# RediSearch/RediSearch

Hardware: NVIDIA H100
Metric: KNN QPS @k=10 on 10M x 768 fp32 (cosine, batch=256) (higher is better)
Workload: dtype f32

## Files before the change

### redisearch_b200/csrc/coarse_tc.cu

```cuda
#include "coarse_tc.h"
#include "distance_core.cuh"
#include "topk_common.cuh"

#include <cuda.h>
#include <cuda_fp16.h>
#include <algorithm>
#include <cstdio>
#include <cstdlib>
#include <type_traits>

namespace rsb200 {

constexpr int kTileM = 128;
constexpr int kMaxStages = 8;
constexpr int kCoarseThreads = 256;
constexpr int kListCap = 64;
constexpr uint32_t kStageBytes = kTileM * 128;
constexpr int kTF32StageStride = 33;

struct CfgTF32 {
    static constexpr int kTileN = 32;
    static constexpr int kBlockK = 32;
    static constexpr int kElem = 4;
};
// ... 320 lines not shown
        const int ew = warp - 4;
        const int et = threadIdx.x - 128;
        mbar_wait(qbar, 0);
        uint32_t s = 0, ph = 0;
        const uint64_t bdesc_first = make_smem_desc(smem_u32(sQ));
        constexpr uint64_t kQStep = kQBlockBytes >> 4, kHalfTile = (kStageBytes / 2) >> 4;
        for (uint32_t i = 0; i < my_tiles; i++) {
            const uint32_t tile = blockIdx.x + i * gridDim.x;
            float acc[2][16];
            uint32_t prev = 0;
            for (uint32_t kb = 0; kb < num_kb; kb++) {
                mbar_wait_spin(&full[s], ph);
                wg_fence();
                const uint64_t ad = make_smem_desc(smem_u32(sA + (size_t)s * kStageBytes));
                const uint64_t bd = bdesc_first + (uint64_t)kb * kQStep;
#pragma unroll
                for (int kk = 0; kk < 4; kk++) {
                    const uint32_t acc_on = (kb | (uint32_t)kk) != 0;
                    wgmma_tf32_n32(acc[0], ad + 2 * kk, bd + 2 * kk, acc_on);
                    wgmma_tf32_n32(acc[1], ad + kHalfTile + 2 * kk, bd + 2 * kk, acc_on);
                }
                wg_commit();
                wg_wait<1>();
                if (kb != 0 && et == 0) mbar_arrive(&empty[prev]);
                prev = s;
                if (++s == nstages) s = 0, ph ^= 1;
            }
            wg_wait<0>();
            if (et == 0) mbar_arrive(&empty[prev]);
            wg_fence_operands(acc[0]);
            wg_fence_operands(acc[1]);
            asm volatile("bar.sync 1, 128;" ::: "memory");
#pragma unroll
            for (int mb = 0; mb < 2; mb++)
#pragma unroll
                for (int j = 0; j < 4; j++)
#pragma unroll
                    for (int x = 0; x < 4; x++) {
                        const int r = 64 * mb + 16 * ew + (lane >> 2) + 8 * (x >> 1), c = 8 * j + 2 * (lane & 3) + (x & 1);
                        sacc[r * kTF32StageStride + c] = __float_as_uint(acc[mb][4 * j + x]);
                    }
            asm volatile("bar.sync 1, 128;" ::: "memory");
            uint32_t v[kHalves][32];
#pragma unroll
            for (int h = 0; h < kHalves; h++)
#pragma unroll
                for (int j = 0; j < 32; j++) v[h][j] = sacc[et * kTF32StageStride + h * 32 + j];
            const uint32_t row = tile * kTileM + et;
            uint32_t pend[kHalves];
#pragma unroll
            for (int h = 0; h < kHalves; h++) {
                pend[h] = 0;
                if (row < n_rows) {
#pragma unroll
                    for (int j = 0; j < 32; j++) {
                        const float d = 1.0f - __uint_as_float(v[h][j]);
                        v[h][j] = orderable_key(d);
                        if (v[h][j] < thresh[h * 32 + j]) pend[h] |= 1u << j;
                    }
                }
            }
            for (;;) {
                uint32_t any_left = 0;
#pragma unroll
                for (int h = 0; h < kHalves; h++) {
                    uint32_t still = 0;
                    uint32_t p = pend[h];
                    while (p) {
                        const int jj = __ffs(p) - 1;
                        p &= p - 1;
                        uint32_t key = 0;
#pragma unroll
                        for (int x = 0; x < 32; x++)
                            if (x == jj) key = v[h][x];
                        const int j = h * 32 + jj;
                        if (key >= thresh[j]) continue;
                        const uint32_t slot = atomicAdd(&counts[j], 1u);
                        if (slot < (uint32_t)kListCap)
                            lists[j * kListCap + slot] = ((uint64_t)key << 32) | row;
                        else
                            still |= 1u << jj;
                    }
                    pend[h] = still;
                    any_left |= still;
                }
                if (any_left) *pending_flag = 1;
                asm volatile("bar.sync 1, 128;" ::: "memory");
                const uint32_t any_pending = *pending_flag;
                for (int j = ew; j < kTileN; j += 4) {
                    const uint32_t c = min(counts[j], (uint32_t)kListCap);
                    if (c < (uint32_t)(kListCap / 2) && !any_pending) continue;
                    if (c <= keep) {
                        if (lane == 0) counts[j] = c;
                        continue;
                    }
                    uint64_t e0 = (lane < (int)c) ? lists[j * kListCap + lane] : kEmptySlot;
                    uint64_t e1 = (lane + 32 < (int)c) ? lists[j * kListCap + lane + 32] : kEmptySlot;
                    __syncwarp();
                    uint64_t last = 0;
                    for (uint32_t r = 0; r < keep; r++) {
                        uint64_t m = e0 < e1 ? e0 : e1;
#pragma unroll
                        for (int sft = 16; sft > 0; sft >>= 1) {
                            const uint64_t o = shfl_xor_u64(m, sft);
                            m = o < m ? o : m;
                        }
                        if (e0 == m) e0 = kEmptySlot; else if (e1 == m) e1 = kEmptySlot;
                        if (lane == 0) lists[j * kListCap + r] = m;
                        last = m;
                    }
                    if (lane == 0) {
                        counts[j] = keep;
                        thresh[j] = (uint32_t)(last >> 32);
                    }
                }
                asm volatile("bar.sync 1, 128;" ::: "memory");
                if (!any_pending) break;
                if (et == 0) *pending_flag = 0;
                asm volatile("bar.sync 1, 128;" ::: "memory");
            }
        }
        asm volatile("bar.sync 1, 128;" ::: "memory");
        for (int j = ew; j < kTileN; j += 4) {
            const uint32_t c = min(counts[j], (uint32_t)kListCap);
            uint64_t e0 = (lane < (int)c) ? lists[j * kListCap + lane] : kEmptySlot;
            uint64_t e1 = (lane + 32 < (int)c) ? lists[j * kListCap + lane + 32] : kEmptySlot;
            const uint32_t q = q_base + j;
            for (uint32_t r = 0; r < keep; r++) {
                uint64_t m = e0 < e1 ? e0 : e1;
#pragma unroll
                for (int sft = 16; sft > 0; sft >>= 1) {
                    const uint64_t o = shfl_xor_u64(m, sft);
                    m = o < m ? o : m;
                }
                if (e0 == m) e0 = kEmptySlot; else if (e1 == m) e1 = kEmptySlot;
                if (lane == 0 && q < nq) cand_out[((size_t)q * gridDim.x + blockIdx.x) * keep + r] = m;
            }
        }
    }
}

constexpr int kQM = 64;
constexpr int kQN = 128;
constexpr int kQMaxStages = 16;
constexpr int kQKbPerStage = 2;
constexpr int kQListStride = 129;
constexpr uint32_t kQBlockBytes = kQN * 128;
constexpr uint32_t kQStageBytes = kQKbPerStage * kQBlockBytes;
__host__ __device__ constexpr uint32_t coarse_kb(uint32_t bytes_per_row) {
    return ((bytes_per_row + 127) / 128 + kQKbPerStage - 1) / kQKbPerStage * kQKbPerStage;
}
constexpr int kQAccStride = kQN + 4;
constexpr uint32_t kQAccBytes = kQM * kQAccStride * 4;
__host__ __device__ constexpr int coarse_consumers(int mode) { return mode == 1 ? 2 : 1; }
__host__ __device__ constexpr int coarse_cta_queries(bool q8, int mode) { return q8 && mode == 1 ? 2 * kQM : kQM; }
__host__ __device__ constexpr int coarse_threads(int mode) { return 128 * (1 + coarse_consumers(mode)); }

template <int kId, int kCount>
__device__ __forceinline__ void named_sync() {
    asm volatile("bar.sync %0, %1;" ::"n"(kId), "n"(kCount) : "memory");
}
template <int kId, int kCount>
__device__ __forceinline__ void named_arrive() {
    asm volatile("bar.arrive %0, %1;" ::"n"(kId), "n"(kCount) : "memory");
}

enum : int { kCaPass, kCaWait, kCaIssue, kCaWait1, kCaEpilogue, kCaHandoff, kCaTiles, kCaSlots };
#ifdef COARSE_CYCLE_ACCOUNT
constexpr int kCaMaxCtas = 1024;
__device__ unsigned long long g_coarse_cycles[kCaMaxCtas][3][kCaSlots];
struct CycleAccount {
    unsigned long long v[kCaSlots] = {};
    __device__ __forceinline__ long long now() const { return clock64(); }
    __device__ __forceinline__ void add(int slot, long long t0) { v[slot] += (unsigned long long)(clock64() - t0); }
    __device__ __forceinline__ void count(int slot) { v[slot]++; }
    __device__ __forceinline__ void flush(uint32_t cta, int role) {
        if (cta < (uint32_t)kCaMaxCtas)
            for (int i = 0; i < kCaSlots; i++) g_coarse_cycles[cta][role][i] = v[i];
    }
};
#else
struct CycleAccount {
    __device__ __forceinline__ long long now() const { return 0; }
    __device__ __forceinline__ void add(int, long long) {}
    __device__ __forceinline__ void count(int) {}
    __device__ __forceinline__ void flush(uint32_t, int) {}
};
#endif

template <int kEpl>
__device__ __forceinline__ uint32_t select_keep(uint64_t *lists, int q, uint32_t c, uint32_t keep, int lane) {
    __syncwarp();
    uint64_t e[kEpl];
    uint32_t k[kEpl];
    bool v[kEpl];
#pragma unroll
    for (int t = 0; t < kEpl; t++) {
        const uint32_t idx = lane + 32 * t;
        v[t] = idx < c;
        e[t] = v[t] ? lists[idx * kQListStride + q] : kEmptySlot;
        k[t] = (uint32_t)(e[t] >> 32);
    }
    __syncwarp();
    uint32_t prefix = 0, remaining = keep;
#pragma unroll 1
    for (int bit = 31; bit >= 0; bit--) {
        const uint32_t hi_mask = bit == 31 ? 0u : ~((2u << bit) - 1u);
        uint32_t zeros = 0;
#pragma unroll
        for (int t = 0; t < kEpl; t++) {
            const bool z = v[t] && ((k[t] ^ prefix) & hi_mask) == 0 && !((k[t] >> bit) & 1u);
            zeros += __popc(__ballot_sync(0xFFFFFFFFu, z));
        }
        if (zeros < remaining) {
            remaining -= zeros;
            prefix |= 1u << bit;
        }
    }
    const uint32_t lt = (1u << lane) - 1u;
    uint32_t base = 0;
#pragma unroll
    for (int t = 0; t < kEpl; t++) {
        const bool less = v[t] && k[t] < prefix;
        const uint32_t m = __ballot_sync(0xFFFFFFFFu, less);
        if (less) lists[(base + __popc(m & lt)) * kQListStride + q] = e[t];
        base += __popc(m);
    }
    uint32_t n_eq = 0;
#pragma unroll
    for (int t = 0; t < kEpl; t++) n_eq += __popc(__ballot_sync(0xFFFFFFFFu, v[t] && k[t] == prefix));
    uint32_t row_cut = 0xFFFFFFFFu;
    if (n_eq > remaining) {
        uint32_t rp = 0, rem = remaining;
#pragma unroll 1
        for (int bit = 31; bit >= 0; bit--) {
            const uint32_t hi_mask = bit == 31 ? 0u : ~((2u << bit) - 1u);
            uint32_t zeros = 0;
#pragma unroll
            for (int t = 0; t < kEpl; t++) {
                const uint32_t row = (uint32_t)e[t];
                const bool z = v[t] && k[t] == prefix && ((row ^ rp) & hi_mask) == 0 && !((row >> bit) & 1u);
                zeros += __popc(__ballot_sync(0xFFFFFFFFu, z));
            }
            if (zeros < rem) {
                rem -= zeros;
                rp |= 1u << bit;
            }
        }
        row_cut = rp;
    }
#pragma unroll
    for (int t = 0; t < kEpl; t++) {
        const bool eq = v[t] && k[t] == prefix && (uint32_t)e[t] <= row_cut;
        const uint32_t m = __ballot_sync(0xFFFFFFFFu, eq);
        if (eq) lists[(base + __popc(m & lt)) * kQListStride + q] = e[t];
        base += __popc(m);
    }
    __syncwarp();
    return prefix;
}

__device__ __forceinline__ int range_int_bound(float r) {
    if (!(r == r) || r < -1073741824.0f) return INT_MIN;
    if (r >= 1073741824.0f) return INT_MAX;
    int x = (int)floorf(r);
    while (__int2float_rn(x + 1) <= r) x++;
    return x;
}

__device__ __forceinline__ int q8_dot_bound(float tdot, float rq, float rt) {
    const float r = __fmul_rn(rq, rt);
    const float f = __fmul_rn(tdot, r);
    if (!(f == f) || !(r >= 0x1p-125f && r <= 0x1p125f)) return INT_MIN;
    const float c = fminf(fmaxf(f, -33554432.0f), 33554432.0f);
    return (int)floorf(c - fabsf(c) * 1e-5f) - 1;
}

template <bool kDirect, int kEpl, int kOp, int kMode, int kVar = 0, bool kFilt = false, int kRegKb = 0>
__global__ void __launch_bounds__(coarse_threads(kMode), 1)
coarse_wgmma_kernel(const __grid_constant__ CUtensorMap map_rows, const uint8_t *__restrict__ shadow, size_t row_pitch,
                    const uint8_t *__restrict__ q16, size_t q16_pitch, const float *__restrict__ row_norm2,
                    const float *__restrict__ q_norm2, uint32_t n_rows, uint32_t nq, uint32_t dim, uint32_t row_bytes,
                    uint32_t num_kb, uint32_t tiles_total, uint32_t keep, uint32_t nstages, uint32_t csize,
                    uint64_t *__restrict__ list_scratch, uint64_t *__restrict__ cand_out, const uint32_t *__restrict__ nq_dev,
                    uint32_t tile_stride, const float *__restrict__ thr_fixed, uint32_t *__restrict__ overflow,
                    const uint32_t *__restrict__ filt, uint32_t filt_words, const uint32_t *__restrict__ filt_q) {
    constexpr bool kFixed = kMode == 1, kSample = kMode == 2;
    constexpr bool kQ8 = kOp == 5;
    constexpr bool kInt = kOp == 1 || kOp == 2 || kOp == 4 || kQ8;
    constexpr int kOpE = kQ8 ? 0 : kOp;
    constexpr int kCons = coarse_consumers(kMode), kConsThreads = 128 * kCons;
    constexpr int kCtaQ = coarse_cta_queries(kQ8, kMode);
    constexpr bool kWide = kCtaQ > kQM;
    static_assert(!kWide || (kCons == 2 && kCtaQ == kCons * kQM), "a wide CTA: one consumer warpgroup per 64 queries");
    constexpr uint32_t kQKbBytes = kCtaQ * 128;
    using Acc = typename std::conditional<kInt, uint32_t, float>::type;
    const uint32_t bx = blockIdx.x, by = blockIdx.y, gx = gridDim.x;
    static_assert(kMode == 0 || (!kDirect && (kOp == 0 || kOp == 3 || kQ8)) || (kDirect && kOp == 0) || (kDirect && kFixed && kInt && kEpl == 8),
                  "fixed bound / sample pass: the fp32 route and 16-bit corpora (inner product / cosine); fixed radius: 8-bit corpora");
    static_assert(!kQ8 || (!kDirect && !kFilt && kRegKb == 0 && kVar == 1), "int8 shadow: signed operands, no filters");
    static_assert(!kFilt || (!kDirect && (kOp == 0 || kOp == 3)) || (kDirect && kFixed && kInt && kEpl == 8),
                  "row filters: the fp32 route and the 8-bit fixed-radius pass");
    static_assert(kRegKb == 0 || (!kDirect && kFixed && kRegKb % kQKbPerStage == 0),
                  "register-held queries: the fixed-bound pass over the fp16 shadow, whole stages");
    auto filt_row = [&](uint32_t pos) { return filt + (size_t)filt_words * (filt_q ? filt_q[pos] : pos); };
    constexpr int kSliceSets = (int)kCoarseSampleSlices / (kQN / 32);
    constexpr int kQListCap = kEpl * 32;
    if (nq_dev) {
        nq = min(nq, *nq_dev);
        if (nq == 0) return;
    }
    constexpr uint32_t kQTrigger = kQListCap - 32;
    extern __shared__ uint8_t smem_raw[];
    uint8_t *smem = smem_raw + ((1024u - (smem_u32(smem_raw) & 1023u)) & 1023u);
    uint8_t *sB = smem;
    uint8_t *sQ = sB + (size_t)nstages * kQStageBytes;
    uint32_t *sacc = reinterpret_cast<uint32_t *>(sQ + (size_t)(num_kb - kRegKb) * kQKbBytes);
    uint64_t *bars = reinterpret_cast<uint64_t *>(sacc + (kFixed ? 0 : kQM * kQAccStride));
    uint64_t *full = bars, *empty = bars + kQMaxStages;
    uint32_t *qcount = reinterpret_cast<uint32_t *>(bars + 2 * kQMaxStages);
    uint64_t *lists = list_scratch + (size_t)(by * gx + bx) * (kQListCap * kQListStride);

    const int warp = threadIdx.x >> 5, lane = threadIdx.x & 31;
    const uint32_t q_base = by * kCtaQ;
    const uint32_t my_tiles = (tiles_total > bx) ? (tiles_total - bx + gx - 1) / gx : 0;

    if (threadIdx.x == 0) {
        for (uint32_t s = 0; s < nstages; s++) {
            mbar_init(&full[s], 1);
            mbar_init(&empty[s], kWide ? kCons * csize : csize);
        }
        asm volatile("fence.mbarrier_init.release.cluster;" ::: "memory");
        asm volatile("fence.proxy.async.shared::cta;" ::: "memory");
    }
    __syncthreads();
    const uint32_t crank = (csize > 1) ? cluster_ctarank() : 0;
    const uint16_t cmask = (uint16_t)((1u << csize) - 1u);
    if (csize > 1) cluster_sync_all();

    CycleAccount ca;
    const uint32_t cta = by * gx + bx;
    if (warp == 0) {
        uint32_t s = 0, ph = 0;
        const uint32_t slice = kQStageBytes / csize;
        const long long t_pass = ca.now();
        for (uint32_t i = 0; i < my_tiles; i++) {
            const uint32_t tile = (bx + i * gx) * tile_stride;
            ca.count(kCaTiles);
            for (uint32_t kb0 = 0; kb0 < num_kb; kb0 += kQKbPerStage) {
                const uint32_t kbn = min((uint32_t)kQKbPerStage, num_kb - kb0);
                const long long t_wait = ca.now();
                mbar_wait_spin(&empty[s], ph ^ 1);
                ca.add(kCaWait, t_wait);
                if (elect_one_sync()) {
                    const uint32_t bytes = kbn * kQBlockBytes;
                    mbar_expect_tx(&full[s], bytes);
                    if constexpr (kDirect) {
                        const uint32_t slice_rows = kQN / csize;
                        for (uint32_t j = 0; j < kbn; j++) {
                            uint8_t *dst = sB + (size_t)s * kQStageBytes + j * kQBlockBytes + crank * slice_rows * 128;
                            const int c0 = (int)((kb0 + j) * ((kOp == 0 || kOp == 3) ? 64 : 128)), c1 = (int)(tile * kQN + crank * slice_rows);
                            if (csize > 1)
                                tma_load_2d_mc(dst, &map_rows, &full[s], c0, c1, cmask);
                            else
                                tma_load_2d(dst, &map_rows, &full[s], c0, c1);
                        }
                    } else {
                        const uint8_t *src = shadow + ((size_t)tile * num_kb + kb0) * kQBlockBytes;
                        if constexpr (kFixed) {
                            if (i + 1 < my_tiles) bulk_prefetch_l2(src + (size_t)gx * num_kb * kQBlockBytes + crank * slice, slice);
                        }
                        if (csize > 1) {
                            bulk_load_1d_mc(sB + (size_t)s * kQStageBytes + crank * slice, src + crank * slice, slice, &full[s], cmask);
                        } else {
                            bulk_load_1d(sB + (size_t)s * kQStageBytes, src, bytes, &full[s]);
                        }
                    }
                }
                __syncwarp();
                if (++s == nstages) s = 0, ph ^= 1;
            }
        }
        ca.add(kCaPass, t_pass);
        if (kFixed && lane == 0) ca.flush(cta, 2);
    } else if (warp >= 4) {
        const int cw = kCons > 1 ? (warp - 4) >> 2 : 0;
        const int ew = kCons > 1 ? (warp - 4) & 3 : warp - 4;
        const int et = kCons > 1 ? (threadIdx.x - 128) & 127 : threadIdx.x - 128;
        const int wq = kWide ? kQM * cw : 0;
        const uint32_t qw = q_base + wq;
        const uint32_t q = qw + et;
        const bool live = et < kQM && q < nq;
        if ((kWide || cw == 0) && et < kQM) {
            const uint4 *src = reinterpret_cast<const uint4 *>(q16 + (size_t)q * q16_pitch);
            for (uint32_t kb = kRegKb; kb < num_kb; kb++) {
                uint8_t *row = sQ + (size_t)(kb - kRegKb) * kQKbBytes + wq * 128 + et * 128;
#pragma unroll
                for (int u = 0; u < 8; u++) {
                    uint4 x = make_uint4(0, 0, 0, 0);
                    if (live && kb * 128 + u * 16 < row_bytes) x = src[kb * 8 + u];
                    *reinterpret_cast<uint4 *>(row + ((u ^ (et & 7)) * 16)) = x;
                }
            }
            if constexpr (kFixed) qcount[wq + et] = 0;
        }
        uint32_t qa[kRegKb ? 4 * kRegKb : 1][4];
        if constexpr (kRegKb > 0) {
#pragma unroll
            for (int i2 = 0; i2 < 2; i2++) {
                const uint32_t fq = qw + 16 * ew + (lane >> 2) + 8 * i2;
                const uint8_t *src = q16 + (size_t)fq * q16_pitch;
#pragma unroll
                for (int t = 0; t < 4 * kRegKb; t++)
#pragma unroll
                    for (int h = 0; h < 2; h++) {
                        const uint32_t off = 32 * t + 4 * (lane & 3) + 16 * h;
                        qa[t][i2 + 2 * h] = (fq < nq && off < row_bytes) ? __ldg(reinterpret_cast<const uint32_t *>(src + off)) : 0u;
                    }
            }
        }
        asm volatile("fence.proxy.async.shared::cta;" ::: "memory");
        named_sync<1, kConsThreads>();
        auto release = [&](uint32_t st) {
            if (csize == 1) {
                if (et == 0) mbar_arrive(&empty[st]);
            } else if (et < (int)csize) {
                mbar_arrive_remote(mapa_u32(smem_u32(&empty[st]), (uint32_t)et));
            }
        };
        uint32_t thr = 0xFFFFFFFFu, cnt = 0;
        float thr_dot = -__int_as_float(0x7f800000);
        float nq_norm = 1.0f;
        if constexpr (kOp == 2) nq_norm = live ? *reinterpret_cast<const float *>(q16 + (size_t)q * q16_pitch + dim) : 1.0f;
        if constexpr (kOp == 3) nq_norm = live ? q_norm2[q] : 0.0f;
        const int *irn2 = reinterpret_cast<const int *>(row_norm2);
        int nq_int = 0, thr_e = live ? INT_MAX : INT_MIN;
        if constexpr (kOp == 4) nq_int = live ? reinterpret_cast<const int *>(q_norm2)[q] : 0;
        float smax[kSample ? kSliceSets : 1][kQN / 32];
#pragma unroll
        for (int x = 0; x < (kSample ? kSliceSets : 1); x++)
#pragma unroll
            for (int h = 0; h < kQN / 32; h++) smax[x][h] = -__int_as_float(0x7f800000);
        if (!live) thr_dot = __int_as_float(0x7f800000);
        uint32_t fthr[2];
        float fthr_dot[2], fnq[2];
        float frad[2];
        int fix[2], fnqi[2];
        float fsq[2] = {1.0f, 1.0f};
        float frq[2] = {1.0f, 1.0f};
        if constexpr (kQ8) {
#pragma unroll
            for (int i2 = 0; i2 < 2; i2++) {
                const uint32_t fq = qw + 16 * ew + (lane >> 2) + 8 * i2;
                if (fq < nq) fsq[i2] = *reinterpret_cast<const float *>(q16 + (size_t)fq * q16_pitch + row_bytes);
                if constexpr (kFixed) frq[i2] = __frcp_rn(fsq[i2]);
            }
        }
        if constexpr (kFixed && kInt && !kQ8) {
#pragma unroll
            for (int i2 = 0; i2 < 2; i2++) {
                const uint32_t fq = qw + 16 * ew + (lane >> 2) + 8 * i2;
                const bool flive = fq < nq;
                frad[i2] = flive ? thr_fixed[fq] : __int_as_float(0x7fffffff);
                fix[i2] = range_int_bound(frad[i2]);
                fnqi[i2] = (kOp == 4 && flive) ? reinterpret_cast<const int *>(q_norm2)[fq] : 0;
                fnq[i2] = (kOp == 2 && flive) ? *reinterpret_cast<const float *>(q16 + (size_t)fq * q16_pitch + dim) : 0.0f;
                fthr_dot[i2] = fnq[i2] * ((1.0f - frad[i2]) - 1e-6f * (1.0f + fabsf(frad[i2])));
            }
        }
        if constexpr (kFixed && (!kInt || kQ8)) {
#pragma unroll
            for (int i2 = 0; i2 < 2; i2++) {
                const uint32_t fq = qw + 16 * ew + (lane >> 2) + 8 * i2;
                const bool flive = fq < nq;
                fnq[i2] = (kOp == 3 && flive) ? q_norm2[fq] : 0.0f;
                const float T = flive ? thr_fixed[fq] : -__int_as_float(0x7f800000);
                fthr[i2] = orderable_key(T);
                if constexpr (kOpE == 0) {
                    const float t = 1.0f - T;
                    fthr_dot[i2] = t - (4e-7f + 2.4e-7f * fabsf(t));
                } else {
                    fthr_dot[i2] = 0.5f * (fnq[i2] - T) - 2e-6f * (fabsf(fnq[i2]) + fabsf(T));
                }
                if (!(T == T)) fthr_dot[i2] = -__int_as_float(0x7f800000), fthr[i2] = 0xFFFFFFFFu;
                if (!flive) fthr_dot[i2] = __int_as_float(0x7f800000);
            }
        }
        uint32_t s = 0, ph = 0;
        const uint64_t bdesc_first = make_smem_desc(smem_u32(sB)), adesc_first = make_smem_desc(smem_u32(sQ + wq * 128));
        constexpr uint64_t kStageStep = kQStageBytes >> 4, kBlockStep = kQBlockBytes >> 4, kAKbStep = kQKbBytes >> 4;
        const uint32_t stages_per_tile = num_kb / kQKbPerStage;
        auto skip = [&](uint32_t n) {
            for (s += n; s >= nstages; s -= nstages) ph ^= 1;
        };
        if (kCons > 1 && !kWide) skip(stages_per_tile * cw);
        const long long t_pass = ca.now();
        for (uint32_t i = kWide ? 0 : cw; i < my_tiles; i += kWide ? 1 : kCons) {
            const uint32_t tile = (bx + i * gx) * tile_stride;
            if (kCons > 1 && !kWide && i >= (uint32_t)kCons) skip(stages_per_tile * (kCons - 1));
            ca.count(kCaTiles);
            float nrm[kQN / 32];
            int inrm[kQN / 32];
            if constexpr (kOp == 4) {
#pragma unroll
                for (int h = 0; h < kQN / 32; h++) {
                    const uint32_t r = tile * kQN + h * 32 + lane;
                    inrm[h] = r < n_rows ? __ldg(irn2 + r) : 0;
                }
            }
            if constexpr (kOp == 3 && !kFixed) {
#pragma unroll
                for (int h = 0; h < kQN / 32; h++) {
                    const uint32_t r = tile * kQN + h * 32 + lane;
                    nrm[h] = r < n_rows ? __ldg(row_norm2 + r) : 0.0f;
                }
            }
            if constexpr (kOp == 2) {
#pragma unroll
                for (int h = 0; h < kQN / 32; h++) {
                    const uint32_t r = tile * kQN + h * 32 + lane;
                    nrm[h] = r < n_rows ? __ldg(reinterpret_cast<const float *>(shadow + (size_t)r * row_pitch + dim)) : 1.0f;
                }
            }
            const uint32_t rbase = tile * kQN + 2 * (lane & 3);
            float q8_st = 0.0f;
            if constexpr (kFixed && kQ8) q8_st = __ldg(row_norm2 + tile);
            float2 rn[(kFixed && kOp == 3) ? kQN / 8 : 1];
            if constexpr (kFixed && kOp == 3) {
#pragma unroll
                for (int j = 0; j < kQN / 8; j++) {
                    const uint32_t r = rbase + 8 * j;
                    if (r + 1 < n_rows)
                        rn[j] = __ldg(reinterpret_cast<const float2 *>(row_norm2 + r));
                    else
                        rn[j] = make_float2(r < n_rows ? __ldg(row_norm2 + r) : 0.0f, 0.0f);
                }
            }
            if constexpr (kCons > 1 && !kWide) {
                static_assert(kCons == 2, "the hand-off pairs two warpgroups");
                const long long t_handoff = ca.now();
                if (i != 0) {
                    if (cw == 0)
                        named_sync<2, 2 * 128>();
                    else
                        named_sync<3, 2 * 128>();
                }
                ca.add(kCaHandoff, t_handoff);
            }
            Acc acc[64];
            uint32_t prev = 0;
            auto stage = [&](uint32_t kb0, auto issue) {
                const long long t_wait = ca.now();
                mbar_wait_spin(&full[s], ph);
                const long long t_issue = ca.now();
                ca.add(kCaWait, t_wait);
                wg_fence();
                issue(bdesc_first + (uint64_t)s * kStageStep);
                wg_commit();
                if constexpr (kCons > 1 && !kWide) {
                    if (kb0 + kQKbPerStage >= num_kb && i + 1 < my_tiles) {
                        if (cw == 0)
                            named_arrive<3, 2 * 128>();
                        else
                            named_arrive<2, 2 * 128>();
                    }
                }
                ca.add(kCaIssue, t_issue);
                const long long t_wait1 = ca.now();
                wg_wait<1>();
                ca.add(kCaWait1, t_wait1);
                if (kb0 != 0) release(prev);
                prev = s;
                if (++s == nstages) s = 0, ph ^= 1;
            };
            if constexpr (kRegKb > 0) {
#pragma unroll
                for (int rs = 0; rs < kRegKb / kQKbPerStage; rs++)
                    stage(rs * kQKbPerStage, [&](uint64_t bd) {
#pragma unroll
                        for (int x = 0; x < 4 * kQKbPerStage; x++)
                            wgmma_f16_n128_ra(acc, qa[4 * kQKbPerStage * rs + x], bd + (x >> 2) * kBlockStep + 2 * (x & 3), (rs | x) != 0);
                    });
            }
            for (uint32_t kb0 = kRegKb; kb0 < num_kb; kb0 += kQKbPerStage)
                stage(kb0, [&](uint64_t bd) {
                    const uint64_t ad = adesc_first + (uint64_t)(kb0 - kRegKb) * kAKbStep;
#pragma unroll
                    for (int x = 0; x < 4 * kQKbPerStage; x++)
                        wgmma_n128<kInt, kVar>(acc, ad + (x >> 2) * kAKbStep + 2 * (x & 3), bd + (x >> 2) * kBlockStep + 2 * (x & 3),
                                               (kb0 | (uint32_t)x) != 0);
                });
            const long long t_epilogue = ca.now();
            wg_wait<0>();
            release(prev);
            wg_fence_operands(acc);
            if constexpr (kFixed && kQ8) {
                const float st = q8_st, rst = __frcp_rn(st);
#pragma unroll
                for (int i2 = 0; i2 < 2; i2++) {
                    const float sqt = __fmul_rn(fsq[i2], st);
                    const int ti = q8_dot_bound(fthr_dot[i2], frq[i2], rst);
                    int m3[11];
#pragma unroll
                    for (int g = 0; g < 10; g++)
                        m3[g] = __vimax3_s32((int)acc[4 * ((3 * g) >> 1) + 2 * i2 + ((3 * g) & 1)],
                                             (int)acc[4 * ((3 * g + 1) >> 1) + 2 * i2 + ((3 * g + 1) & 1)],
                                             (int)acc[4 * ((3 * g + 2) >> 1) + 2 * i2 + ((3 * g + 2) & 1)]);
                    m3[10] = max((int)acc[4 * 15 + 2 * i2], (int)acc[4 * 15 + 2 * i2 + 1]);
                    const int mx = __vimax3_s32(__vimax3_s32(m3[0], m3[1], m3[2]), __vimax3_s32(m3[3], m3[4], m3[5]),
                                                __vimax3_s32(__vimax3_s32(m3[6], m3[7], m3[8]), m3[9], m3[10]));
                    uint32_t pass = 0;
                    if (mx > ti) {
#pragma unroll
                        for (int j = 0; j < kQN / 8; j++)
#pragma unroll
                            for (int c = 0; c < 2; c++)
                                if ((int)acc[4 * j + 2 * i2 + c] > ti) pass |= 1u << (2 * j + c);
                    }
                    if (pass && tile * kQN + kQN > n_rows) {
#pragma unroll
                        for (int j = 0; j < kQN / 8; j++)
#pragma unroll
                            for (int c = 0; c < 2; c++)
                                if (rbase + 8 * j + c >= n_rows) pass &= ~(1u << (2 * j + c));
                    }
                    while (pass) {
                        const int b = __ffs(pass) - 1;
                        pass &= pass - 1;
                        uint32_t raw = 0;
#pragma unroll
                        for (int x = 0; x < 32; x++)
                            if (x == b) raw = acc[4 * (x >> 1) + 2 * i2 + (x & 1)];
                        const uint32_t row = rbase + 8 * (b >> 1) + (b & 1);
                        const uint32_t key = orderable_key(__fsub_rn(1.0f, __fmul_rn(sqt, __int2float_rn((int)raw))));
                        if (key < fthr[i2]) {
                            const int qs = wq + 16 * ew + (lane >> 2) + 8 * i2;
                            const uint32_t slot = atomicAdd(&qcount[qs], 1u);
                            if (slot < (uint32_t)kQListCap) lists[slot * kQListStride + qs] = ((uint64_t)key << 32) | row;
                        }
                    }
                }
                ca.add(kCaEpilogue, t_epilogue);
                continue;
            }
            if constexpr (kFixed && kInt) {
                uint32_t pass2[2] = {0u, 0u};
                if constexpr (kOp == 1) {
#pragma unroll
                    for (int i2 = 0; i2 < 2; i2++) {
                        int mx = (int)acc[2 * i2];
#pragma unroll
                        for (int x = 1; x < 32; x++) mx = max(mx, (int)acc[4 * (x >> 1) + 2 * i2 + (x & 1)]);
                        if (1 - mx <= fix[i2]) {
#pragma unroll
                            for (int x = 0; x < 32; x++)
                                if (1 - (int)acc[4 * (x >> 1) + 2 * i2 + (x & 1)] <= fix[i2]) pass2[i2] |= 1u << x;
                        }
                    }
                } else {
#pragma unroll
                    for (int j = 0; j < kQN / 8; j++)
#pragma unroll
                        for (int c = 0; c < 2; c++) {
                            const int src = 8 * (j & 3) + 2 * (lane & 3) + c;
                            if constexpr (kOp == 4) {
                                const int rn = __shfl_sync(0xFFFFFFFFu, inrm[j >> 2], src);
#pragma unroll
                                for (int i2 = 0; i2 < 2; i2++)
                                    if (rn + fnqi[i2] - 2 * (int)acc[4 * j + 2 * i2 + c] <= fix[i2]) pass2[i2] |= 1u << (2 * j + c);
                            } else {
                                const float nr = __shfl_sync(0xFFFFFFFFu, nrm[j >> 2], src);
#pragma unroll
                                for (int i2 = 0; i2 < 2; i2++)
                                    if (__int2float_rn((int)acc[4 * j + 2 * i2 + c]) >= nr * fthr_dot[i2]) pass2[i2] |= 1u << (2 * j + c);
                            }
                        }
                }
#pragma unroll
                for (int i2 = 0; i2 < 2; i2++) {
                    uint32_t pass = pass2[i2];
                    if (pass && tile * kQN + kQN > n_rows) {
#pragma unroll
                        for (int x = 0; x < 32; x++)
                            if (rbase + 8 * (x >> 1) + (x & 1) >= n_rows) pass &= ~(1u << x);
                    }
                    while (pass) {
                        const int b = __ffs(pass) - 1;
                        pass &= pass - 1;
                        uint32_t raw = 0;
#pragma unroll
                        for (int x = 0; x < 32; x++)
                            if (x == b) raw = acc[4 * (x >> 1) + 2 * i2 + (x & 1)];
                        const uint32_t row = rbase + 8 * (b >> 1) + (b & 1);
                        float d;
                        if constexpr (kOp == 1) {
                            d = (float)(1 - (int)raw);
                        } else if constexpr (kOp == 2) {
                            const float nr = __ldg(reinterpret_cast<const float *>(shadow + (size_t)row * row_pitch + dim));
                            d = __fsub_rn(1.0f, __fdiv_rn((float)(int)raw, __fmul_rn(nr, fnq[i2])));
                        } else {
                            d = __int2float_rn(__ldg(irn2 + row) + fnqi[i2] - 2 * (int)raw);
                        }
                        bool hit = d <= frad[i2];
                        if constexpr (kFilt) {
                            if (hit) hit = (__ldg(filt_row(q_base + 16 * ew + (lane >> 2) + 8 * i2) + (row >> 5)) >> (row & 31)) & 1u;
                        }
                        if (hit) {
                            const int qs = wq + 16 * ew + (lane >> 2) + 8 * i2;
                            const uint32_t slot = atomicAdd(&qcount[qs], 1u);
                            if (slot < (uint32_t)kQListCap) lists[slot * kQListStride + qs] = ((uint64_t)orderable_key(d) << 32) | row;
                        }
                    }
                }
                ca.add(kCaEpilogue, t_epilogue);
                continue;
            }
            if constexpr (kFixed && !kInt) {
#pragma unroll
                for (int i2 = 0; i2 < 2; i2++) {
                    uint32_t pass = 0;
                    if constexpr (kOp == 0) {
                        float m8[8];
#pragma unroll
                        for (int g = 0; g < 8; g++)
                            m8[g] = fmaxf(fmaxf(acc[8 * g + 2 * i2], acc[8 * g + 2 * i2 + 1]), fmaxf(acc[8 * g + 4 + 2 * i2], acc[8 * g + 5 + 2 * i2]));
                        const float mx = fmaxf(fmaxf(fmaxf(m8[0], m8[1]), fmaxf(m8[2], m8[3])), fmaxf(fmaxf(m8[4], m8[5]), fmaxf(m8[6], m8[7])));
                        if (mx > fthr_dot[i2]) {
#pragma unroll
                            for (int j = 0; j < kQN / 8; j++)
#pragma unroll
                                for (int c = 0; c < 2; c++)
                                    if (acc[4 * j + 2 * i2 + c] > fthr_dot[i2]) pass |= 1u << (2 * j + c);
                        }
                    } else {
#pragma unroll
                        for (int j = 0; j < kQN / 8; j++)
#pragma unroll
                            for (int c = 0; c < 2; c++)
                                if (acc[4 * j + 2 * i2 + c] > fmaf(c ? rn[j].y : rn[j].x, 0.499999f, fthr_dot[i2])) pass |= 1u << (2 * j + c);
                    }
                    if (pass && tile * kQN + kQN > n_rows) {
#pragma unroll
                        for (int j = 0; j < kQN / 8; j++)
#pragma unroll
                            for (int c = 0; c < 2; c++)
                                if (rbase + 8 * j + c >= n_rows) pass &= ~(1u << (2 * j + c));
                    }
                    while (pass) {
// ... 32 lines not shown
            }
#pragma unroll
            for (int j = 0; j < kQN / 8; j++) {
                const int m = 16 * ew + (lane >> 2), n = 8 * j + 2 * (lane & 3);
                uint32_t b[4];
#pragma unroll
                for (int x = 0; x < 4; x++) {
                    if constexpr (kQ8)
                        b[x] = __float_as_uint(__fmul_rn(tsqt[x >> 1], __int2float_rn((int)acc[4 * j + x])));
                    else if constexpr (kInt)
                        b[x] = acc[4 * j + x];
                    else
                        b[x] = __float_as_uint(acc[4 * j + x]);
                }
                *reinterpret_cast<uint2 *>(sacc + m * kQAccStride + n) = make_uint2(b[0], b[1]);
                *reinterpret_cast<uint2 *>(sacc + (m + 8) * kQAccStride + n) = make_uint2(b[2], b[3]);
            }
            asm volatile("bar.sync 1, 128;" ::: "memory");
            uint32_t v[kQN / 32][32];
            {
                const uint32_t *mine = sacc + (et & (kQM - 1)) * kQAccStride;
#pragma unroll
                for (int h = 0; h < kQN / 32; h++)
#pragma unroll
                    for (int u = 0; u < 8; u++) {
                        const uint4 w = *reinterpret_cast<const uint4 *>(mine + h * 32 + 4 * u);
                        v[h][4 * u] = w.x, v[h][4 * u + 1] = w.y, v[h][4 * u + 2] = w.z, v[h][4 * u + 3] = w.w;
                    }
            }
#pragma unroll
            for (int h = 0; h < kQN / 32; h++) {
                const uint32_t row0 = tile * kQN + h * 32;
                uint32_t fw = 0xFFFFFFFFu;
                if constexpr (kFilt) fw = (live && row0 < n_rows) ? __ldg(filt_row(q) + (row0 >> 5)) : 0u;
                if constexpr (kSample) {
                    float mx = -__int_as_float(0x7f800000);
                    const bool tail = row0 + 32 > n_rows;
                    if constexpr (kFilt) {
#pragma unroll
                        for (int j = 0; j < 32; j++) {
                            float u = __uint_as_float(v[h][j]);
                            if constexpr (kOpE != 0) u = fmaf(__shfl_sync(0xFFFFFFFFu, nrm[h], j), -0.5f, u);
                            if ((fw >> j) & 1u) mx = fmaxf(mx, u);
                        }
                    } else if constexpr (kOpE == 0) {
                        if (!tail) {
                            float m8[8];
#pragma unroll
                            for (int g = 0; g < 8; g++)
                                m8[g] = fmaxf(fmaxf(__uint_as_float(v[h][4 * g]), __uint_as_float(v[h][4 * g + 1])),
                                              fmaxf(__uint_as_float(v[h][4 * g + 2]), __uint_as_float(v[h][4 * g + 3])));
                            mx = fmaxf(fmaxf(fmaxf(m8[0], m8[1]), fmaxf(m8[2], m8[3])), fmaxf(fmaxf(m8[4], m8[5]), fmaxf(m8[6], m8[7])));
                        } else {
#pragma unroll
                            for (int j = 0; j < 32; j++)
                                if (row0 + j < n_rows) mx = fmaxf(mx, __uint_as_float(v[h][j]));
                        }
                    } else {
#pragma unroll
                        for (int j = 0; j < 32; j++) {
                            const float u = fmaf(__shfl_sync(0xFFFFFFFFu, nrm[h], j), -0.5f, __uint_as_float(v[h][j]));
                            if (!tail || row0 + j < n_rows) mx = fmaxf(mx, u);
                        }
                    }
#pragma unroll
                    for (int x = 0; x < kSliceSets; x++)
                        if ((int)(i % (uint32_t)kSliceSets) == x) smax[kSample ? x : 0][h] = fmaxf(smax[kSample ? x : 0][h], mx);
                    continue;
                }
                uint32_t pass = 0;
#pragma unroll
                for (int j = 0; j < 32; j++) {
                    bool p;
                    if constexpr (kOpE == 0)
                        p = __uint_as_float(v[h][j]) > thr_dot;
                    else if constexpr (kOp == 1)
                        p = (float)(int)v[h][j] > thr_dot;
                    else if constexpr (kOp == 2)
                        p = (float)(int)v[h][j] > __shfl_sync(0xFFFFFFFFu, nrm[h], j) * thr_dot - 0.01f;
                    else if constexpr (kOp == 4)
                        p = __shfl_sync(0xFFFFFFFFu, inrm[h], j) + nq_int - 2 * (int)v[h][j] < thr_e;
                    else
                        p = __uint_as_float(v[h][j]) > fmaf(__shfl_sync(0xFFFFFFFFu, nrm[h], j), 0.499999f, thr_dot);
                    if (p) pass |= 1u << j;
                }
                if (row0 + 32 > n_rows) pass &= (n_rows > row0) ? ((1u << (n_rows - row0)) - 1u) : 0u;
                if constexpr (kFilt) pass &= fw;
                while (pass) {
                    const int j = __ffs(pass) - 1;
                    pass &= pass - 1;
                    uint32_t raw = 0;
#pragma unroll
                    for (int x = 0; x < 32; x++)
                        if (x == j) raw = v[h][x];
                    float d;
                    if constexpr (kOpE == 0)
                        d = 1.0f - __uint_as_float(raw);
                    else if constexpr (kOp == 1)
                        d = (float)(1 - (int)raw);
                    else if constexpr (kOp == 2) {
                        const uint32_t r = row0 + j;
                        const float nr = __ldg(reinterpret_cast<const float *>(shadow + (size_t)r * row_pitch + dim));
                        d = __fsub_rn(1.0f, __fdiv_rn((float)(int)raw, __fmul_rn(nr, nq_norm)));
                    } else if constexpr (kOp == 4) {
                        d = __int2float_rn(__ldg(irn2 + row0 + j) + nq_int - 2 * (int)raw);
                    } else {
                        d = __fsub_rn(__fadd_rn(nq_norm, __ldg(row_norm2 + row0 + j)), __fmul_rn(2.0f, __uint_as_float(raw)));
                    }
                    const uint32_t key = orderable_key(d);
                    if (key < thr) {
                        lists[cnt * kQListStride + et] = ((uint64_t)key << 32) | (row0 + j);
                        cnt++;
                    }
                }
                uint32_t m = __ballot_sync(0xFFFFFFFFu, cnt > kQTrigger);
                while (m) {
                    const int src = __ffs(m) - 1;
                    m &= m - 1;
                    const uint32_t c = __shfl_sync(0xFFFFFFFFu, cnt, src);
                    const uint32_t worst = select_keep<kEpl>(lists, ew * 32 + src, c, keep, lane);
                    if (lane == src) {
                        cnt = keep;
                        thr = worst;
                        const float t = 1.0f - key_to_float(thr);
                        if constexpr (kOpE == 0)
                            thr_dot = t - 4e-7f;
                        else if constexpr (kOp == 1)
                            thr_dot = t - (fabsf(t) * 1e-6f + 2.0f);
                        else if constexpr (kOp == 2) {
                            const float tq = t * nq_norm;
                            thr_dot = tq - fabsf(tq) * 4e-6f;
                        } else if constexpr (kOp == 4) {
                            thr_e = __float2int_ru(key_to_float(thr));
                        } else {
                            const float dthr = key_to_float(thr);
                            thr_dot = 0.5f * (nq_norm - dthr) - 2e-6f * (fabsf(nq_norm) + fabsf(dthr));
                        }
                    }
                }
            }
        }
        ca.add(kCaPass, t_pass);
        if (kFixed && et == 0) ca.flush(cta, cw);
        __syncwarp();
        if constexpr (kFixed) {
            named_sync<1, kConsThreads>();
            constexpr int per = kCtaQ / (4 * kCons);
            const int pw = 4 * cw + ew;
            for (int qs = per * pw; qs < per * pw + per; qs++) {
                const uint32_t qq = q_base + qs;
                if (qq >= nq) break;
                const uint32_t n = qcount[qs], c = min(n, (uint32_t)kQListCap);
                uint64_t *dst = cand_out + ((size_t)qq * gx + bx) * keep;
                for (uint32_t r = lane; r < keep; r += 32) dst[r] = r < c ? lists[r * kQListStride + qs] : kEmptySlot;
                if (lane == 0 && n > (uint32_t)kQListCap) overflow[qq] = 1u;
            }
        }
        if constexpr (kSample) {
            if (live) {
                uint64_t *dst = cand_out + ((size_t)q * gx + bx) * keep;
#pragma unroll
                for (int x = 0; x < kSliceSets; x++)
#pragma unroll
                    for (int h = 0; h < kQN / 32; h++) {
                        const float m = smax[kSample ? x : 0][h];
                        uint64_t c = kEmptySlot;
                        if (m > -__int_as_float(0x7f800000)) {
                            const float d = kOpE == 0 ? 1.0f - m : __fsub_rn(nq_norm, __fmul_rn(2.0f, m));
                            c = (uint64_t)orderable_key(d) << 32;
                        }
                        if ((uint32_t)(x * (kQN / 32) + h) < keep) dst[x * (kQN / 32) + h] = c;
                    }
            }
        }
        for (int src = 0; src < ((kSample || kFixed) ? 0 : 32); src++) {
            uint32_t c = __shfl_sync(0xFFFFFFFFu, cnt, src);
            const uint32_t qq = q_base + ew * 32 + src;
            if (c > keep) {
                select_keep<kEpl>(lists, ew * 32 + src, c, keep, lane);
                c = keep;
            }
            if (ew * 32 + src < kQM && qq < nq) {
                uint64_t *dst = cand_out + ((size_t)qq * gx + bx) * keep;
                __syncwarp();
                for (uint32_t r = lane; r < keep; r += 32) dst[r] = r < c ? lists[r * kQListStride + ew * 32 + src] : kEmptySlot;
            }
        }
    }
    __syncthreads();
    if (csize > 1) cluster_sync_all();
}

__global__ void __launch_bounds__(256) to_f16_kernel(const uint8_t *__restrict__ src, size_t spitch, uint32_t dim, uint32_t first,
                                                     uint32_t n, uint8_t *__restrict__ dst, size_t dpitch) {
    const uint32_t per_row = dim / 8;
    const size_t total = (size_t)n * per_row;
    for (size_t i = (size_t)blockIdx.x * blockDim.x + threadIdx.x; i < total; i += (size_t)gridDim.x * blockDim.x) {
        const uint32_t r = first + (uint32_t)(i / per_row), c = (uint32_t)(i % per_row);
        const float4 *p = reinterpret_cast<const float4 *>(src + (size_t)r * spitch) + 2 * c;
        const float4 x = p[0], y = p[1];
        __half2 h0 = __floats2half2_rn(x.x, x.y), h1 = __floats2half2_rn(x.z, x.w);
        __half2 h2 = __floats2half2_rn(y.x, y.y), h3 = __floats2half2_rn(y.z, y.w);
        uint4 o;
        o.x = *reinterpret_cast<uint32_t *>(&h0);
        o.y = *reinterpret_cast<uint32_t *>(&h1);
        o.z = *reinterpret_cast<uint32_t *>(&h2);
        o.w = *reinterpret_cast<uint32_t *>(&h3);
        reinterpret_cast<uint4 *>(dst + (size_t)r * dpitch)[c] = o;
    }
}

constexpr uint32_t kRefineMaxSurv = 2048;
constexpr uint32_t kRefineMaxSurvWide = 4096;

__device__ __forceinline__ float query_eps(float eps, const float *q_norm2, uint32_t pos, float max_norm, uint32_t dim, bool l2,
                                           const float *q_eps = nullptr) {
    if (q_eps) return q_eps[pos];
    if (!q_norm2) return eps;
    const float qn2 = q_norm2[pos], qn = sqrtf(qn2);
    float e = eps * max_norm * qn + 5.97e-8f * sqrtf((float)dim) * (max_norm + qn);
    if (l2) e = 2.0f * e + (float)(dim + 4) * 1.2e-7f * (max_norm * max_norm + qn2);
    return e * 1.0001f;
}
__device__ __forceinline__ uint32_t block_kth_key(const uint64_t *mine, uint32_t total, uint32_t k, uint32_t *hist, uint32_t *ctl) {
    const int lane = threadIdx.x & 31;
    if (threadIdx.x == 0) ctl[0] = 0, ctl[1] = k, ctl[2] = 0;
    __syncthreads();
    uint32_t cnt = 0;
    for (uint32_t i = threadIdx.x; i < total; i += blockDim.x) cnt += mine[i] != kEmptySlot;
    cnt = __reduce_add_sync(0xFFFFFFFFu, cnt);
    if (lane == 0 && cnt) atomicAdd(&ctl[2], cnt);
    __syncthreads();
    if (ctl[2] < k) return 0xFFFFFFFFu;
    for (int shift = 24; shift >= 0; shift -= 8) {
        hist[threadIdx.x] = 0;
        __syncthreads();
        const uint32_t prefix = ctl[0];
        const uint32_t hi_mask = shift == 24 ? 0u : ~((1u << (shift + 8)) - 1u);
        for (uint32_t i = threadIdx.x; i < total; i += blockDim.x) {
            const uint64_t c = mine[i];
            if (c == kEmptySlot) continue;
            const uint32_t key = (uint32_t)(c >> 32);
            if (((key ^ prefix) & hi_mask) == 0) atomicAdd(&hist[(key >> shift) & 255u], 1u);
        }
        __syncthreads();
        if (threadIdx.x == 0) {
            uint32_t rem = ctl[1], b = 0;
            for (; b < 255; b++) {
                if (hist[b] >= rem) break;
                rem -= hist[b];
            }
            ctl[0] = prefix | (b << shift);
            ctl[1] = rem;
        }
        __syncthreads();
    }
    return ctl[0];
}

__global__ void __launch_bounds__(256) threshold_kernel(const uint64_t *__restrict__ cand, uint32_t nq, uint32_t lists_per_query,
                                                        uint32_t keep, uint32_t k, float eps, const float *__restrict__ q_norm2,
                                                        float max_norm, uint32_t dim, int l2, float *__restrict__ thr_out,
                                                        uint32_t *__restrict__ overflow, const float *__restrict__ q_eps) {
    __shared__ uint32_t hist[256];
    __shared__ uint32_t ctl[4];
    const uint32_t q = blockIdx.x;
    if (q >= nq) return;
    const uint32_t ak = block_kth_key(cand + (size_t)q * lists_per_query * keep, lists_per_query * keep, k, hist, ctl);
    if (threadIdx.x == 0) {
        const float e = query_eps(eps, q_norm2, q, max_norm, dim, l2 != 0, q_eps);
        float T;
        if (ak == 0xFFFFFFFFu)
            T = __int_as_float(0x7f800000);
        else if (e == 0.0f)
            T = key_to_float(ak + 1u);
        else
            T = key_to_float(ak) + (2.0f * e) * 1.001f + 1e-30f;
        thr_out[q] = T;
        overflow[q] = 0;
    }
}

template <int MT, uint32_t kSurv, bool kLab = false>
__global__ void __launch_bounds__(256) refine_kernel(const uint8_t *rows, size_t pitch, uint32_t dim, const uint8_t *queries,
                                                     size_t qpitch, uint32_t nq, uint32_t lists_per_query, uint32_t keep, uint32_t k,
                                                     const uint64_t *__restrict__ cand, float eps, const float *__restrict__ q_norm2,
                                                     float max_norm, uint32_t *__restrict__ ok, uint32_t ok_value, uint64_t *__restrict__ out,
                                                     const uint32_t *__restrict__ q_index, const uint32_t *__restrict__ nq_dev,
                                                     const float *__restrict__ thr_T, const uint32_t *__restrict__ overflow,
                                                     uint32_t smem_cap, const uint64_t *__restrict__ row_label, const float *__restrict__ q_eps) {
    using Tile = DistTile<DT_F32, MT, 1, 1>;
    __shared__ uint64_t surv[kSurv];
    __shared__ uint32_t hist[256];
    __shared__ uint32_t ctl[4];
    __shared__ uint32_t s_nsurv, s_bad, s_ncomp;
    if (nq_dev) nq = min(nq, *nq_dev);
    if (blockIdx.x >= nq) return;
    const uint32_t q = q_index ? q_index[blockIdx.x] : blockIdx.x;
    const int warp = threadIdx.x >> 5, lane = threadIdx.x & 31;
    const uint64_t *mine = cand + (size_t)blockIdx.x * lists_per_query * keep;
    uint32_t total = lists_per_query * keep;
    eps = query_eps(eps, q_norm2, blockIdx.x, max_norm, dim, MT == MT_L2, q_eps);
    if (threadIdx.x == 0) s_nsurv = 0, s_bad = 0, s_ncomp = 0;
    __syncthreads();
    extern __shared__ uint64_t s_cand[];
    for (uint32_t i0 = 0; i0 < total; i0 += blockDim.x) {
        const uint32_t i = i0 + threadIdx.x;
        const uint64_t c = i < total ? mine[i] : kEmptySlot;
        const uint32_t m = __ballot_sync(0xFFFFFFFFu, c != kEmptySlot);
        uint32_t base = 0;
        if (lane == 0 && m) base = atomicAdd(&s_ncomp, (uint32_t)__popc(m));
        base = __shfl_sync(0xFFFFFFFFu, base, 0);
        if (c != kEmptySlot) {
            const uint32_t pos = base + __popc(m & ((1u << lane) - 1u));
            if (pos < smem_cap) s_cand[pos] = c;
        }
    }
    __syncthreads();
    const bool packed = s_ncomp <= smem_cap;
    const uint64_t *mine_all = mine;
    const uint32_t total_all = total;
    if (packed) {
        mine = s_cand;
        total = s_ncomp;
    }
    const uint32_t ak_key = block_kth_key(mine, total, k, hist, ctl);
    const float cut = ak_key == 0xFFFFFFFFu ? __int_as_float(0x7f800000) : key_to_float(ak_key) + (2.0f * eps) * 1.001f + 1e-30f;
    for (uint32_t i0 = 0; i0 < total; i0 += blockDim.x) {
        const uint32_t i = i0 + threadIdx.x;
        const uint64_t c = i < total ? mine[i] : kEmptySlot;
        const bool take = c != kEmptySlot && (ak_key == 0xFFFFFFFFu || key_to_float((uint32_t)(c >> 32)) <= cut);
        const uint32_t m = __ballot_sync(0xFFFFFFFFu, take);
        uint32_t base = 0;
        if (lane == 0 && m) base = atomicAdd(&s_nsurv, (uint32_t)__popc(m));
        base = __shfl_sync(0xFFFFFFFFu, base, 0);
        if (take) {
            const uint32_t pos = base + __popc(m & ((1u << lane) - 1u));
            if (pos < kSurv) surv[pos] = c;
        }
    }
    __syncthreads();
    const uint32_t n_all = s_nsurv, n_surv = min(n_all, kSurv);
    const uint8_t *qb[1] = {queries + (size_t)q * qpitch};
    for (uint32_t i = warp; i < n_surv; i += 8) {
        const uint32_t row = (uint32_t)surv[i];
        const uint8_t *rowb[1] = {rows + (size_t)row * pitch};
        float d[1];
        Tile::run(rowb, qb, dim, lane, d);
        __syncwarp();
        if (lane == 0) surv[i] = make_composite(d[0], kLab ? (uint32_t)row_label[row] : row);
    }
    const uint32_t n_sort = max(32u, next_pow2(n_surv));
    __syncthreads();
    for (uint32_t i = n_surv + threadIdx.x; i < n_sort; i += blockDim.x) surv[i] = kEmptySlot;
    bitonic_sort_smem(surv, n_sort);
    for (uint32_t i = threadIdx.x; i < k; i += blockDim.x) out[(size_t)q * k + i] = i < n_surv ? surv[i] : kEmptySlot;
    bool bad = n_all > kSurv;
    if (q_norm2 && !(q_norm2[blockIdx.x] == q_norm2[blockIdx.x])) bad = true;
    if (!isfinite(cut) || (thr_T && !isfinite(thr_T[blockIdx.x]))) bad = true;
    const bool have_k = n_surv >= k;
    const float ek = have_k ? key_to_float((uint32_t)(surv[k - 1] >> 32)) : 0.0f;
    if (thr_T) {
        if (threadIdx.x == 0 && (overflow[blockIdx.x] != 0 || !have_k || !(thr_T[blockIdx.x] - eps > ek))) bad = true;
    } else {
        (void)total_all;
        for (uint32_t l = threadIdx.x; l < lists_per_query; l += blockDim.x) {
            const uint64_t *lst = mine_all + (size_t)l * keep;
            uint32_t worst = 0;
            bool full = true;
            for (uint32_t j = 0; j < keep; j++) {
                const uint64_t c = lst[j];
                if (c == kEmptySlot)
                    full = false;
                else
                    worst = max(worst, (uint32_t)(c >> 32));
            }
            if (!full) continue;
            if (!have_k)
                bad = true;
            else if (!(key_to_float(worst) - eps > ek))
                bad = true;
        }
    }
    if (bad) atomicOr(&s_bad, 1u);
    __syncthreads();
    if (threadIdx.x == 0) ok[q] = s_bad ? 0u : ok_value;
}

constexpr uint32_t kRangeWindow = 2048;

__global__ void range_bound_kernel(const float *__restrict__ radius, uint32_t nq, float eps, const float *__restrict__ q_norm2,
                                   float max_norm, uint32_t dim, int l2, float *__restrict__ thr, uint32_t *__restrict__ overflow,
                                   uint32_t *__restrict__ total) {
    const uint32_t q = blockIdx.x * blockDim.x + threadIdx.x;
    if (q == 0) *total = 0;
    if (q >= nq) return;
    const float e = query_eps(eps, q_norm2, q, max_norm, dim, l2 != 0);
    thr[q] = radius[q] + e * 1.001f + 1e-30f;
    overflow[q] = 0;
}

constexpr double kR16U = 0x1p-24;
constexpr double kR16TcStep = 0x1p-22;
constexpr double kR16Underflow = 0x1p-149;
constexpr double kR16Flush = 0x1p-126;
constexpr double kR16Margin = 2.0;
constexpr double kR16MaxMag = 0x1p120;

template <int DT>
__global__ void __launch_bounds__(256) range_bound16_kernel(const uint8_t *__restrict__ queries, size_t qpitch, uint32_t nq, uint32_t dim,
                                                            const float *__restrict__ radius, float max_norm, float *__restrict__ thr,
                                                            uint32_t *__restrict__ overflow) {
    const uint32_t q = blockIdx.x * 8 + (threadIdx.x >> 5);
    const int lane = threadIdx.x & 31;
    if (q >= nq) return;
    const uint8_t *qb = queries + (size_t)q * qpitch;
    double s = 0.0;
    for (uint32_t i = lane; i < dim; i += 32) {
        const double v = (double)load16<DT>(qb, i);
        s = __fma_ru(v, v, s);
    }
#pragma unroll
    for (int o = 16; o > 0; o >>= 1) s = __dadd_ru(s, __shfl_xor_sync(0xFFFFFFFFu, s, o));
    if (lane != 0) return;
    const double d = (double)dim;
    const double qn = __dsqrt_ru(s);
    const double x = __dadd_ru(__dmul_ru(__dmul_ru((double)max_norm, 1.0 + 0x1p-23), __dsqrt_ru(__fma_ru(d, 0x1p-20, 1.0))),
                               __dsqrt_ru(__dmul_ru(d, 0x1p-149)));
    const double mag = __dmul_ru(x, qn);
    const double chain = 8.0 * ((dim / 8 + 31) / 32) + (double)((dim % 8 + 31) / 32) + 7.0;
    const double gamma = __ddiv_ru(chain * kR16U, __dsub_rd(1.0, chain * kR16U));
    const double ue = __dmul_ru(kR16U, __dadd_ru(1.0, mag));
    const double b_tc = __dadd_ru(__dmul_ru(__dmul_ru(d, kR16TcStep), mag), ue);
    const double b_cc = __dadd_ru(__dadd_ru(__dmul_ru(gamma, mag), ue), __dmul_ru(d, kR16Underflow));
    const double eps = __dmul_ru(kR16Margin, __dadd_ru(__dadd_ru(b_tc, b_cc), __dmul_ru(d, kR16Flush)));
    const float t = __double2float_ru(__dadd_ru((double)radius[q], eps));
    const bool ok = isfinite(qn) && isfinite(x) && mag < kR16MaxMag && isfinite(t);
    thr[q] = ok ? t : -__int_as_float(0x7f800000);
    overflow[q] = 0;
}

template <int DT, int MT>
__global__ void __launch_bounds__(256) range_refine_kernel(const uint8_t *rows, size_t pitch, uint32_t dim, const uint8_t *queries,
                                                           size_t qpitch, uint32_t slots, uint64_t *cand, const float *__restrict__ radius,
                                                           const float *__restrict__ q_norm2, const float *__restrict__ thr,
                                                           const uint32_t *__restrict__ overflow, uint64_t *__restrict__ out,
                                                           uint32_t *__restrict__ total, uint32_t *__restrict__ ok, uint32_t *__restrict__ cnt,
                                                           uint32_t *__restrict__ off, uint32_t cap) {
    using Tile = DistTile<DT, MT, 1, 1>;
    __shared__ uint64_t s_cand[kRangeWindow];
    __shared__ uint32_t s_n, s_kept, s_base;
    const uint32_t q = blockIdx.x;
    const int warp = threadIdx.x >> 5, lane = threadIdx.x & 31;
    bool proven = overflow[q] == 0 && isfinite(thr[q]);
    if (q_norm2 && !(q_norm2[q] == q_norm2[q])) proven = false;
    if (!proven) {
        if (threadIdx.x == 0) ok[q] = 0, cnt[q] = 0;
        if (threadIdx.x == 0 && !cap) off[q] = 0;
        return;
    }
    const float r = radius[q];
    uint64_t *mine = cand + (size_t)q * slots;
    const uint8_t *qb[1] = {queries + (size_t)q * qpitch};
    if (threadIdx.x == 0) s_kept = 0;
    for (uint32_t w0 = 0; w0 < slots; w0 += kRangeWindow) {
        const uint32_t wend = min(slots, w0 + kRangeWindow);
        if (threadIdx.x == 0) s_n = 0;
        __syncthreads();
        for (uint32_t i0 = w0; i0 < wend; i0 += blockDim.x) {
            const uint32_t i = i0 + threadIdx.x;
            const uint64_t c = i < wend ? mine[i] : kEmptySlot;
            const uint32_t m = __ballot_sync(0xFFFFFFFFu, c != kEmptySlot);
            uint32_t base = 0;
            if (lane == 0 && m) base = atomicAdd(&s_n, (uint32_t)__popc(m));
            base = __shfl_sync(0xFFFFFFFFu, base, 0);
            if (c != kEmptySlot) s_cand[base + __popc(m & ((1u << lane) - 1u))] = c;
        }
        __syncthreads();
        const uint32_t n = s_n;
        for (uint32_t i = warp; i < n; i += blockDim.x / 32) {
            const uint32_t row = (uint32_t)s_cand[i];
            const uint8_t *rowb[1] = {rows + (size_t)row * pitch};
            float d[1];
            Tile::run(rowb, qb, dim, lane, d);
            if (lane == 0 && d[0] <= r) mine[atomicAdd(&s_kept, 1u)] = make_composite(d[0], row);
        }
        __syncthreads();
    }
    const uint32_t kept = s_kept;
    if (cap) {
        if (threadIdx.x == 0) ok[q] = 1, cnt[q] = kept;
        for (uint32_t i = threadIdx.x; i < min(kept, cap); i += blockDim.x) out[(size_t)q * cap + i] = mine[i];
        return;
    }
    if (threadIdx.x == 0) {
        s_base = atomicAdd(total, kept);
        ok[q] = 1;
        cnt[q] = kept;
        off[q] = s_base;
    }
    __syncthreads();
    for (uint32_t i = threadIdx.x; i < kept; i += blockDim.x) out[s_base + i] = mine[i];
}

__global__ void __launch_bounds__(256) range_pack_kernel(const uint64_t *__restrict__ cand, uint32_t slots, const uint32_t *__restrict__ overflow,
                                                         uint32_t cap, uint64_t *__restrict__ out, uint32_t *__restrict__ cnt,
                                                         uint32_t *__restrict__ ok) {
    __shared__ uint32_t s_n;
    const uint32_t q = blockIdx.x;
    if (overflow[q]) {
        if (threadIdx.x == 0) ok[q] = 0, cnt[q] = 0;
        return;
    }
    if (threadIdx.x == 0) s_n = 0;
    __syncthreads();
    const uint64_t *mine = cand + (size_t)q * slots;
    for (uint32_t i = threadIdx.x; i < slots; i += blockDim.x) {
        const uint64_t c = mine[i];
        if (c == kEmptySlot) continue;
        const uint32_t pos = atomicAdd(&s_n, 1u);
        if (pos < cap) out[(size_t)q * cap + pos] = c;
    }
    __syncthreads();
    if (threadIdx.x == 0) ok[q] = 1, cnt[q] = s_n;
}

__global__ void __launch_bounds__(512) range_label_fold_kernel(const uint64_t *__restrict__ cand, uint32_t slots, const uint32_t *__restrict__ front,
                                                               const uint32_t *__restrict__ overflow, const uint64_t *__restrict__ id_to_label,
                                                               uint32_t cap, uint64_t *__restrict__ out, uint32_t *__restrict__ cnt,
                                                               uint32_t *__restrict__ ok, uint32_t *__restrict__ flags) {
    extern __shared__ uint64_t s_hi[];
    uint32_t *s_row = reinterpret_cast<uint32_t *>(s_hi + kRangeFoldMaxHits);
    __shared__ uint32_t s_n, s_labels;
    const uint32_t q = blockIdx.x;
    const bool proven = front ? ok[q] != 0 : overflow[q] == 0;
    if (!proven) {
        if (threadIdx.x == 0) ok[q] = 0, flags[q] = 0;
        return;
    }
// ... 16 lines not shown
        if (threadIdx.x == 0) ok[q] = 0, flags[q] = 3;
        return;
    }
    uint32_t n2 = 1;
    while (n2 < n) n2 <<= 1;
    for (uint32_t i = n + threadIdx.x; i < n2; i += blockDim.x) s_hi[i] = ~0ull, s_row[i] = ~0u;
    __syncthreads();
    for (uint32_t k = 2; k <= n2; k <<= 1)
        for (uint32_t j = k >> 1; j > 0; j >>= 1) {
            for (uint32_t i = threadIdx.x; i < n2; i += blockDim.x) {
                const uint32_t p = i ^ j;
                if (p <= i) continue;
                const uint64_t ha = s_hi[i], hb = s_hi[p];
                const uint32_t ra = s_row[i], rb = s_row[p];
                const bool b_first = hb < ha || (hb == ha && rb < ra);
                if (b_first == ((i & k) == 0)) {
                    s_hi[i] = hb, s_hi[p] = ha;
                    s_row[i] = rb, s_row[p] = ra;
                }
            }
            __syncthreads();
        }
    for (uint32_t i = threadIdx.x; i < n; i += blockDim.x) {
        if (i > 0 && (s_hi[i] >> 32) == (s_hi[i - 1] >> 32)) continue;
        const uint32_t pos = atomicAdd(&s_labels, 1u);
        if (pos < cap) out[(size_t)q * cap + pos] = (s_hi[i] << 32) | s_row[i];
    }
    __syncthreads();
    if (threadIdx.x == 0) ok[q] = 1, flags[q] = 1, cnt[q] = s_labels;
}

__global__ void compact_unproven_kernel(const uint32_t *__restrict__ ok, uint32_t nq, uint32_t *__restrict__ idx,
                                        uint32_t *__restrict__ count) {
    __shared__ uint32_t n;
    if (threadIdx.x == 0) n = 0;
    __syncthreads();
    for (uint32_t q0 = 0; q0 < nq; q0 += blockDim.x) {
        const uint32_t q = q0 + threadIdx.x;
        const bool un = q < nq && ok[q] == 0;
        const uint32_t m = __ballot_sync(0xFFFFFFFFu, un);
        __shared__ uint32_t wbase[32];
        const int warp = threadIdx.x >> 5, lane = threadIdx.x & 31;
        if (lane == 0) wbase[warp] = __popc(m);
        __syncthreads();
        uint32_t before = 0;
        for (int w = 0; w < warp; w++) before += wbase[w];
        uint32_t all = 0;
        for (uint32_t w = 0; w < blockDim.x / 32; w++) all += wbase[w];
        if (un) idx[n + before + __popc(m & ((1u << lane) - 1u))] = q;
        __syncthreads();
        if (threadIdx.x == 0) n += all;
        __syncthreads();
    }
    if (threadIdx.x == 0) *count = n;
}
__global__ void gather_queries_kernel(const uint8_t *__restrict__ src, size_t pitch, const float *__restrict__ src_n2,
                                      const uint32_t *__restrict__ idx, const uint32_t *__restrict__ count,
                                      uint8_t *__restrict__ dst, float *__restrict__ dst_n2) {
    const uint32_t n = *count;
    for (uint32_t i = blockIdx.x; i < n; i += gridDim.x) {
        const uint4 *s4 = reinterpret_cast<const uint4 *>(src + (size_t)idx[i] * pitch);
        uint4 *d4 = reinterpret_cast<uint4 *>(dst + (size_t)i * pitch);
        for (uint32_t c = threadIdx.x; c < pitch / 16; c += blockDim.x) d4[c] = s4[c];
        if (src_n2 && threadIdx.x == 0) dst_n2[i] = src_n2[idx[i]];
    }
}

typedef CUresult (*EncodeTiledFn)(CUtensorMap *, CUtensorMapDataType, cuuint32_t, void *, const cuuint64_t *,
                                  const cuuint64_t *, const cuuint32_t *, const cuuint32_t *, CUtensorMapInterleave,
                                  CUtensorMapSwizzle, CUtensorMapL2promotion, CUtensorMapFloatOOBfill);

static EncodeTiledFn encode_fn() {
    static EncodeTiledFn fn = nullptr;
    static bool tried = false;
    if (!tried) {
        tried = true;
        void *p = nullptr;
        cudaDriverEntryPointQueryResult qres;
        if (cudaGetDriverEntryPoint("cuTensorMapEncodeTiled", &p, cudaEnableDefault, &qres) == cudaSuccess &&
            qres == cudaDriverEntryPointSuccess)
            fn = reinterpret_cast<EncodeTiledFn>(p);
    }
    return fn;
}

static bool make_map(CUtensorMap *m, CUtensorMapDataType dt, const void *base, uint64_t inner, uint64_t outer, uint64_t pitch_bytes,
                     uint32_t box_inner, uint32_t box_outer) {
    EncodeTiledFn fn = encode_fn();
    if (!fn) return false;
    cuuint64_t dims[2] = {inner, outer};
    cuuint64_t strides[1] = {pitch_bytes};
    cuuint32_t box[2] = {box_inner, box_outer};
    cuuint32_t estr[2] = {1, 1};
    return fn(m, dt, 2, const_cast<void *>(base), dims, strides, box, estr, CU_TENSOR_MAP_INTERLEAVE_NONE,
              CU_TENSOR_MAP_SWIZZLE_128B, CU_TENSOR_MAP_L2_PROMOTION_L2_256B, CU_TENSOR_MAP_FLOAT_OOB_FILL_NONE) == CUDA_SUCCESS;
}


static constexpr size_t kSmemLimit = 232448;

template <int V>
static const void *wgmma_kernel_fn_v(CoarseKind kind, uint32_t epl, int epi, int mode, bool filt) {
    if (filt) {
        if (kind != CoarseDirect8 || mode != 1) return nullptr;
        if (epi == 2) return (const void *)coarse_wgmma_kernel<true, 8, 4, 1, V, true>;
        return epi == 1 ? (const void *)coarse_wgmma_kernel<true, 8, 2, 1, V, true> : (const void *)coarse_wgmma_kernel<true, 8, 1, 1, V, true>;
    }
    if (kind == CoarseDirect16) {
        if (mode == 1) return (const void *)coarse_wgmma_kernel<true, 8, 0, 1, V>;
        if (mode == 2) return (const void *)coarse_wgmma_kernel<true, 3, 0, 2, V>;
        return epl == 3 ? (const void *)coarse_wgmma_kernel<true, 3, 0, 0, V> : (const void *)coarse_wgmma_kernel<true, 8, 0, 0, V>;
    }
    if (kind == CoarseDirect8) {
        if (mode == 1) {
            if (epi == 2) return (const void *)coarse_wgmma_kernel<true, 8, 4, 1, V>;
            return epi == 1 ? (const void *)coarse_wgmma_kernel<true, 8, 2, 1, V> : (const void *)coarse_wgmma_kernel<true, 8, 1, 1, V>;
        }
        if (epi == 2) return epl == 3 ? (const void *)coarse_wgmma_kernel<true, 3, 4, 0, V> : (const void *)coarse_wgmma_kernel<true, 8, 4, 0, V>;
        if (epi == 1) return epl == 3 ? (const void *)coarse_wgmma_kernel<true, 3, 2, 0, V> : (const void *)coarse_wgmma_kernel<true, 8, 2, 0, V>;
        return epl == 3 ? (const void *)coarse_wgmma_kernel<true, 3, 1, 0, V> : (const void *)coarse_wgmma_kernel<true, 8, 1, 0, V>;
    }
    return nullptr;
}
static constexpr uint32_t kFixedRegKb = 4;
static uint32_t fixed_reg_kb(uint32_t epl, bool l2, bool filt) { return (epl == 3 && !l2 && !filt) ? kFixedRegKb : 0u; }
static const void *wgmma_kernel_fn(CoarseKind kind, uint32_t epl, int epi, int mode = 0, uint32_t variant = 0, bool filt = false,
                                   uint32_t reg_kb = 0) {
    const bool l2 = epi != 0;
    if (kind == CoarseDirect16 || kind == CoarseDirect8)
        return variant ? wgmma_kernel_fn_v<1>(kind, epl, epi, mode, filt) : wgmma_kernel_fn_v<0>(kind, epl, epi, mode, filt);
    if (kind == CoarseQ8) {
        if (filt || reg_kb || epi) return nullptr;
        if (mode == 1) return (const void *)coarse_wgmma_kernel<false, 8, 5, 1, 1>;
        if (mode == 2) return (const void *)coarse_wgmma_kernel<false, 3, 5, 2, 1>;
        return epl == 8 ? (const void *)coarse_wgmma_kernel<false, 8, 5, 0, 1> : nullptr;
    }
    if (reg_kb) {
        if (mode != 1 || reg_kb != fixed_reg_kb(epl, l2, filt)) return nullptr;
        return (const void *)coarse_wgmma_kernel<false, 3, 0, 1, 0, false, kFixedRegKb>;
    }
    if (filt) {
        if (mode == 1 && epl == 8) return l2 ? (const void *)coarse_wgmma_kernel<false, 8, 3, 1, 0, true> : (const void *)coarse_wgmma_kernel<false, 8, 0, 1, 0, true>;
        if (mode == 1) return l2 ? (const void *)coarse_wgmma_kernel<false, 3, 3, 1, 0, true> : (const void *)coarse_wgmma_kernel<false, 3, 0, 1, 0, true>;
        if (mode == 2) return l2 ? (const void *)coarse_wgmma_kernel<false, 3, 3, 2, 0, true> : (const void *)coarse_wgmma_kernel<false, 3, 0, 2, 0, true>;
        if (epl != 8) return nullptr;
        return l2 ? (const void *)coarse_wgmma_kernel<false, 8, 3, 0, 0, true> : (const void *)coarse_wgmma_kernel<false, 8, 0, 0, 0, true>;
    }
    if (mode == 1 && epl == 8) return l2 ? (const void *)coarse_wgmma_kernel<false, 8, 3, 1> : (const void *)coarse_wgmma_kernel<false, 8, 0, 1>;
    if (mode == 1) return l2 ? (const void *)coarse_wgmma_kernel<false, 3, 3, 1> : (const void *)coarse_wgmma_kernel<false, 3, 0, 1>;
    if (mode == 2) return l2 ? (const void *)coarse_wgmma_kernel<false, 3, 3, 2> : (const void *)coarse_wgmma_kernel<false, 3, 0, 2>;
    if (l2) return epl == 3 ? (const void *)coarse_wgmma_kernel<false, 3, 3, 0> : (const void *)coarse_wgmma_kernel<false, 8, 3, 0>;
    return epl == 3 ? (const void *)coarse_wgmma_kernel<false, 3, 0, 0> : (const void *)coarse_wgmma_kernel<false, 8, 0, 0>;
}
static size_t wgmma_fixed_smem(uint32_t num_kb, int mode = 0, uint32_t reg_kb = 0, uint32_t cta_q = kQM) {
    return 1024 + (size_t)(num_kb - reg_kb) * cta_q * 128 + (mode == 1 ? cta_q * 4 : kQAccBytes) + 2 * kQMaxStages * 8 + 64;
}
static uint32_t wgmma_stages(uint32_t num_kb, int mode, uint32_t reg_kb, uint32_t cta_q = kQM) {
    return (uint32_t)std::min<size_t>(kQMaxStages, (kSmemLimit - wgmma_fixed_smem(num_kb, mode, reg_kb, cta_q)) / kQStageBytes);
}
static bool wgmma_fits_bytes(uint32_t row_bytes, uint32_t cta_q = kQM) {
    return wgmma_fixed_smem(coarse_kb(row_bytes), 0, 0, cta_q) + 2 * (size_t)kQStageBytes <= kSmemLimit;
}
static bool wgmma_fits(uint32_t dim) { return wgmma_fits_bytes(dim * 2); }

static size_t fixed_smem(uint32_t num_kb) {
    const uint32_t tn = CfgTF32::kTileN;
    return 1024 + (size_t)num_kb * tn * 128 + (size_t)kTileM * kTF32StageStride * 4 + (size_t)tn * kListCap * 8 + (2 * kMaxStages + 1) * 8 +
           tn * 8 + 64;
}

bool coarse_supported(const CorpusView &c, uint32_t nq, uint32_t k, CoarseKind kind) {
    if (kind == CoarseDirect16) {
        if ((c.dtype != DT_F16 && c.dtype != DT_BF16) || c.metric != MT_IP) return false;
        if (c.dim % 8 != 0 || c.dim < 32 || c.pitch % 16 != 0 || !wgmma_fits(c.dim)) return false;
        if (k > 128 || nq < 1 || c.n_rows < 65536) return false;
        return encode_fn() != nullptr;
    }
    if (kind == CoarseDirect8) {
        if (c.dtype != DT_I8 && c.dtype != DT_U8) return false;
        if (c.dim % 16 != 0 || c.dim < 32 || c.pitch % 16 != 0 || !wgmma_fits_bytes(c.dim)) return false;
        if (k > 128 || nq < 1 || c.n_rows < 65536) return false;
        return encode_fn() != nullptr;
    }
    if (kind == CoarseQ8) {
        if (c.dtype != DT_F32 || c.metric != MT_IP || c.dim % 8 != 0 || c.dim < 32 || c.dim > 1024 || c.pitch % 16 != 0) return false;
        if (k > kCoarseMaxK || nq < 1 || c.n_rows < 65536 || !wgmma_fits_bytes(c.dim, coarse_cta_queries(true, 1))) return false;
        if (coarse_kb(c.dim) >= coarse_kb(c.dim * 2)) return false;
        return encode_fn() != nullptr;
    }
    if (c.dtype != DT_F32 || (c.metric != MT_IP && c.metric != MT_L2)) return false;
    if (kind == CoarseTF32 && c.metric != MT_IP) return false;
    if (c.dim % 8 != 0 || c.dim < 32 || c.dim > 1024) return false;
    if (c.pitch % 16 != 0) return false;
    if (k > (kind == CoarseF16 ? kCoarseMaxKWide : kCoarseMaxK) || nq < 1) return false;
    if (c.n_rows < 65536) return false;
    if (kind == CoarseF16 && !wgmma_fits(c.dim)) return false;
    if (kind == CoarseTF32 && fixed_smem((c.dim + CfgTF32::kBlockK - 1) / CfgTF32::kBlockK) + 3 * kStageBytes > kSmemLimit) return false;
    return encode_fn() != nullptr;
}

CoarsePlan plan_coarse(const CorpusView &c, uint32_t nq, CoarseKind kind, uint32_t k, uint32_t keep_override, uint32_t tile_stride,
                       int mode, bool filt) {
    CoarsePlan p{};
    p.kind = kind;
    p.tile_stride = std::max(1u, tile_stride);
    p.mode = (kind == CoarseF16 || kind == CoarseQ8 || (kind == CoarseDirect16 && c.metric == MT_IP)) ? mode : (kind == CoarseDirect8 && mode == 1) ? 1 : 0;
    if (kind == CoarseF16 || kind == CoarseQ8 || kind == CoarseDirect16 || kind == CoarseDirect8) {
        p.num_kb = coarse_kb(kind == CoarseDirect8 || kind == CoarseQ8 ? c.dim : c.dim * 2);
        p.tiles = ((c.n_rows + kQN - 1) / kQN + p.tile_stride - 1) / p.tile_stride;
        const uint32_t cta_q = (uint32_t)coarse_cta_queries(kind == CoarseQ8, p.mode);
        p.grid_y = (nq + cta_q - 1) / cta_q;
        const uint32_t sms = (uint32_t)device_sm_count();
        p.grid_x = std::max(1u, std::min(p.tiles, sms / p.grid_y));
        p.keep = (kind == CoarseF16 || kind == CoarseQ8) ? (keep_override ? keep_override : (k <= kCoarseTier1MaxK ? kCoarseKeep : kCoarseKeepWide))
                                   : (k <= 32 ? 32u : 128u);
        p.epl = p.keep <= 32 ? 3 : 8;
        if (p.mode == 1 && kind == CoarseF16)
            p.keep = k > kCoarseMaxK ? kCoarseFixedCapWide : kCoarseFixedCap, p.epl = k > kCoarseMaxK ? 8 : 3;
        if (p.mode == 1 && (kind == CoarseDirect16 || kind == CoarseDirect8)) p.keep = kCoarseFixedCapDirect, p.epl = 8;
        if (p.mode == 1 && kind == CoarseQ8) p.keep = kCoarseFixedCapQ8, p.epl = 8;
        if (p.mode == 2) p.keep = kCoarseSampleSlices, p.epl = 3;
        p.threads = (uint32_t)coarse_threads(p.mode);
        const int epi = kind == CoarseQ8 ? 0 : kind == CoarseF16 ? (c.metric == MT_L2 ? 1 : 0) : c.metric == MT_COS ? 1 : (kind == CoarseDirect8 && c.metric == MT_L2) ? 2 : 0;
        static int rcap = -1;
        if (rcap < 0) {
            const char *e = getenv("VECSIM_B200_REGKB");
            rcap = e ? std::max(0, atoi(e)) : (int)kFixedRegKb;
        }
        p.reg_kb = 0;
        if (kind == CoarseF16 && p.mode == 1) {
            const uint32_t rk = fixed_reg_kb(p.epl, epi != 0, filt);
            if (rk && (int)rk <= rcap && p.num_kb >= rk + kQKbPerStage && wgmma_stages(p.num_kb, p.mode, rk) > wgmma_stages(p.num_kb, p.mode, 0))
                p.reg_kb = rk;
        }
        p.stages = wgmma_stages(p.num_kb, p.mode, p.reg_kb, cta_q);
        p.smem_bytes = wgmma_fixed_smem(p.num_kb, p.mode, p.reg_kb, cta_q) + (size_t)p.stages * kQStageBytes;
        p.csize = 1;
        static int ccap = -1;
        if (ccap < 0) {
            const char *e = getenv("VECSIM_B200_CLUSTER");
            ccap = e ? std::max(1, atoi(e)) : 4;
        }
        for (uint32_t cs = cta_q > kQM ? 2 : 4; cs > 1; cs >>= 1)
            if ((int)cs <= ccap && p.grid_y % cs == 0 && (kQStageBytes / kQKbPerStage) % (16 * cs) == 0) {
                p.csize = cs;
                break;
            }
        const void *kfn = wgmma_kernel_fn(kind, p.epl, epi, p.mode, (c.dtype == DT_BF16 || c.dtype == DT_I8 || kind == CoarseQ8) ? 1u : 0u, filt,
                                          p.reg_kb);
        if (p.csize > 1) {
            cudaFuncSetAttribute(kfn, cudaFuncAttributeMaxDynamicSharedMemorySize, (int)p.smem_bytes);
            cudaLaunchConfig_t cfg{};
            cudaLaunchAttribute at[1];
            cfg.gridDim = dim3(1, p.grid_y, 1);
            cfg.blockDim = dim3(p.threads);
            cfg.dynamicSmemBytes = p.smem_bytes;
            at[0].id = cudaLaunchAttributeClusterDimension;
            at[0].val.clusterDim.x = 1, at[0].val.clusterDim.y = p.csize, at[0].val.clusterDim.z = 1;
            cfg.attrs = at, cfg.numAttrs = 1;
            int nclusters = 0;
            if (cudaOccupancyMaxActiveClusters(&nclusters, kfn, &cfg) != cudaSuccess || nclusters < 1) {
                cudaGetLastError();
                p.csize = 1;
            } else {
                p.grid_x = std::max(1u, std::min(p.grid_x, (uint32_t)nclusters / (p.grid_y / p.csize)));
            }
        }
        p.cand_elems = (size_t)nq * p.grid_x * p.keep;
        p.scratch_elems = (size_t)p.grid_x * p.grid_y * (p.epl * 32) * kQListStride;
        return p;
    }
    const uint32_t bk = CfgTF32::kBlockK, tn = CfgTF32::kTileN;
    p.num_kb = (c.dim + bk - 1) / bk;
    p.tiles = (c.n_rows + kTileM - 1) / kTileM;
    p.grid_y = (nq + tn - 1) / tn;
    const uint32_t sms = (uint32_t)device_sm_count();
    p.grid_x = std::max(1u, std::min(p.tiles, sms / p.grid_y));
    p.keep = kCoarseKeep;
    const size_t fixed_bytes = fixed_smem(p.num_kb);
    p.threads = kCoarseThreads;
    p.stages = (uint32_t)std::min<size_t>(kMaxStages, (kSmemLimit - fixed_bytes) / kStageBytes);
    p.cand_elems = (size_t)nq * p.grid_x * p.keep;
    p.smem_bytes = fixed_bytes + (size_t)p.stages * kStageBytes;
    return p;
}

template <class Cfg>
static cudaError_t launch_coarse_t(const void *rows, size_t pitch, uint32_t n_rows, uint32_t dim, const void *d_queries, size_t qpitch,
                                   uint32_t nq, const CoarsePlan &p, uint64_t *d_cand, cudaStream_t s) {
    const CUtensorMapDataType dt = Cfg::kElem == 4 ? CU_TENSOR_MAP_DATA_TYPE_FLOAT32 : CU_TENSOR_MAP_DATA_TYPE_FLOAT16;
    CUtensorMap ma, mq;
    if (!make_map(&ma, dt, rows, dim, n_rows, pitch, Cfg::kBlockK, kTileM)) return cudaErrorInvalidValue;
    if (!make_map(&mq, dt, d_queries, dim, nq, qpitch, Cfg::kBlockK, Cfg::kTileN)) return cudaErrorInvalidValue;
    cudaError_t e = cudaFuncSetAttribute(coarse_kernel<Cfg>, cudaFuncAttributeMaxDynamicSharedMemorySize, (int)p.smem_bytes);
    if (e != cudaSuccess) return e;
    coarse_kernel<Cfg><<<dim3(p.grid_x, p.grid_y), p.threads, p.smem_bytes, s>>>(ma, mq, n_rows, nq, p.num_kb, p.tiles, p.keep, p.stages,
                                                                                d_cand);
    return cudaGetLastError();
}

cudaError_t launch_coarse(const CoarseOperands &o, uint32_t n_rows, uint32_t dim, uint32_t nq, const CoarsePlan &p, uint64_t *d_cand,
                          uint64_t *d_scratch, cudaStream_t s, const uint32_t *d_nq_dev, const float *d_thr_fixed, uint32_t *d_overflow,
                          const uint32_t *d_filt, uint32_t filt_words, const uint32_t *d_filt_q) {
    if (d_filt && p.kind != CoarseF16 && !(p.kind == CoarseDirect8 && p.mode == 1)) return cudaErrorInvalidValue;
    if (p.kind == CoarseF16 || p.kind == CoarseQ8 || p.kind == CoarseDirect16 || p.kind == CoarseDirect8) {
        if (p.mode == 1 && (!d_thr_fixed || !d_overflow)) return cudaErrorInvalidValue;
        const uint32_t ev = (p.kind == CoarseDirect16 || p.kind == CoarseDirect8) && o.elem_variant ? 1u : 0u;
        const void *kfn = wgmma_kernel_fn(p.kind, p.epl, o.epilogue, p.mode, ev, d_filt != nullptr, p.reg_kb);
        if (!kfn) return cudaErrorInvalidValue;
        cudaError_t e = cudaFuncSetAttribute(kfn, cudaFuncAttributeMaxDynamicSharedMemorySize, (int)p.smem_bytes);
        if (e != cudaSuccess) {
            fprintf(stderr, "vecsim_b200: coarse pass: %zu bytes of shared memory refused: %s\n", p.smem_bytes, cudaGetErrorString(e));
            return e;
        }
        CUtensorMap mr{};
        uint32_t row_bytes = dim * 2;
        if (p.kind == CoarseDirect16) {
            if (!make_map(&mr, ev ? CU_TENSOR_MAP_DATA_TYPE_BFLOAT16 : CU_TENSOR_MAP_DATA_TYPE_FLOAT16, o.rows, dim, n_rows, o.pitch, 64,
                          kQN / p.csize))
                return cudaErrorInvalidValue;
        } else if (p.kind == CoarseQ8) {
            row_bytes = (uint32_t)coarse_q8_payload(dim);
        } else if (p.kind == CoarseDirect8) {
            row_bytes = dim;
            if (!make_map(&mr, CU_TENSOR_MAP_DATA_TYPE_UINT8, o.rows, dim, n_rows, o.pitch, 128, kQN / p.csize)) return cudaErrorInvalidValue;
        }
        cudaLaunchConfig_t cfg{};
        cudaLaunchAttribute at[1];
        cfg.gridDim = dim3(p.grid_x, p.grid_y, 1);
        cfg.blockDim = dim3(p.threads);
        cfg.dynamicSmemBytes = p.smem_bytes;
        cfg.stream = s;
        at[0].id = cudaLaunchAttributeClusterDimension;
        at[0].val.clusterDim.x = 1, at[0].val.clusterDim.y = p.csize, at[0].val.clusterDim.z = 1;
        cfg.attrs = at, cfg.numAttrs = 1;
        const uint8_t *rows = static_cast<const uint8_t *>(o.rows), *qs = static_cast<const uint8_t *>(o.queries);
        size_t rp = o.pitch, qp = o.qpitch;
        const float *rn2 = o.row_norm2, *qn2 = o.q_norm2;
        uint32_t a_nrows = n_rows, a_nq = nq, a_dim = dim, a_rb = row_bytes, a_kb = p.num_kb, a_tiles = p.tiles, a_keep = p.keep,
                 a_st = p.stages, a_cs = p.csize, a_stride = p.tile_stride;
        void *args[] = {&mr,   &rows,    &rp,     &qs,   &qp,   &rn2,  &qn2,      &a_nrows, &a_nq,     &a_dim,       &a_rb, &a_kb,
                        &a_tiles, &a_keep, &a_st, &a_cs, &d_scratch, &d_cand, &d_nq_dev, &a_stride, &d_thr_fixed, &d_overflow,
                        &d_filt, &filt_words, &d_filt_q};
        const cudaError_t le = cudaLaunchKernelExC(&cfg, kfn, args);
        if (le != cudaSuccess)
            fprintf(stderr, "vecsim_b200: coarse pass launch failed (kind %d mode %d csize %u grid %u x %u smem %zu): %s\n", (int)p.kind,
                    p.mode, p.csize, p.grid_x, p.grid_y, p.smem_bytes, cudaGetErrorString(le));
        return le;
    }
    return launch_coarse_t<CfgTF32>(o.rows, o.pitch, n_rows, dim, o.queries, o.qpitch, nq, p, d_cand, s);
}

#ifdef COARSE_CYCLE_ACCOUNT
extern "C" int VecSimB200_CoarseCycles(unsigned long long *host, int max_ctas) {
    const size_t bytes = (size_t)std::min(max_ctas, kCaMaxCtas) * 3 * kCaSlots * sizeof(unsigned long long);
    if (cudaMemcpyFromSymbol(host, g_coarse_cycles, bytes) != cudaSuccess) return -1;
    return kCaSlots;
}
#endif

__global__ void __launch_bounds__(256) to_f16_tiled_kernel(const uint8_t *__restrict__ src, size_t spitch, uint32_t dim, uint32_t first,
                                                           uint32_t n, uint8_t *__restrict__ dst, uint32_t num_kb) {
    const uint32_t per_row = num_kb * 8;
    const size_t total = (size_t)n * per_row;
    for (size_t i = (size_t)blockIdx.x * blockDim.x + threadIdx.x; i < total; i += (size_t)gridDim.x * blockDim.x) {
        const uint32_t r = first + (uint32_t)(i / per_row), ci = (uint32_t)(i % per_row);
        uint4 o = make_uint4(0, 0, 0, 0);
        if (ci * 8 < dim) {
            const float4 *p = reinterpret_cast<const float4 *>(src + (size_t)r * spitch) + 2 * ci;
            const float4 x = p[0], y = p[1];
            __half2 h0 = __floats2half2_rn(x.x, x.y), h1 = __floats2half2_rn(x.z, x.w);
            __half2 h2 = __floats2half2_rn(y.x, y.y), h3 = __floats2half2_rn(y.z, y.w);
            o.x = *reinterpret_cast<uint32_t *>(&h0);
            o.y = *reinterpret_cast<uint32_t *>(&h1);
            o.z = *reinterpret_cast<uint32_t *>(&h2);
            o.w = *reinterpret_cast<uint32_t *>(&h3);
        }
        const uint32_t tile = r / kQN, rr = r % kQN, kb = ci / 8, c = ci % 8;
        uint8_t *blk = dst + ((size_t)tile * num_kb + kb) * kQBlockBytes;
        *reinterpret_cast<uint4 *>(blk + rr * 128 + ((c ^ (rr & 7)) * 16)) = o;
    }
}

size_t coarse_shadow_bytes(uint32_t rows, uint32_t dim) {
    return (size_t)((rows + kQN - 1) / kQN) * coarse_kb(dim * 2) * kQBlockBytes;
}

cudaError_t launch_to_f16_tiled(const void *src, size_t spitch, uint32_t dim, uint32_t first, uint32_t n, void *dst, cudaStream_t s) {
    if (n == 0) return cudaSuccess;
    const uint32_t num_kb = coarse_kb(dim * 2);
    const size_t total = (size_t)n * num_kb * 8;
    const uint32_t grid = (uint32_t)std::max<size_t>(1, std::min<size_t>((total + 255) / 256, (size_t)device_sm_count() * 16));
    to_f16_tiled_kernel<<<grid, 256, 0, s>>>(static_cast<const uint8_t *>(src), spitch, dim, first, n, static_cast<uint8_t *>(dst), num_kb);
    return cudaGetLastError();
}

__global__ void __launch_bounds__(256) to_i8_tiled_kernel(const uint8_t *__restrict__ src, size_t spitch, uint32_t dim, uint32_t n_rows,
                                                          uint32_t tile0, uint32_t ntiles, uint8_t *__restrict__ dst, uint32_t num_kb,
                                                          float *__restrict__ tscale, uint32_t *__restrict__ stats) {
    __shared__ float s_max[8];
    const int warp = threadIdx.x >> 5, lane = threadIdx.x & 31;
    float w_res = 0.0f, w_nrm = 0.0f;
    for (uint32_t t = tile0 + blockIdx.x; t < tile0 + ntiles; t += gridDim.x) {
        float m = 0.0f;
        for (uint32_t rr = warp; rr < (uint32_t)kQN; rr += 8) {
            const uint32_t r = t * kQN + rr;
            if (r >= n_rows) break;
            const float *x = reinterpret_cast<const float *>(src + (size_t)r * spitch);
            for (uint32_t e = lane * 4; e < dim; e += 128) {
                const float4 v = *reinterpret_cast<const float4 *>(x + e);
                m = fmaxf(m, fmaxf(fmaxf(fabsf(v.x), fabsf(v.y)), fmaxf(fabsf(v.z), fabsf(v.w))));
                if (!(v.x == v.x && v.y == v.y && v.z == v.z && v.w == v.w)) m = __int_as_float(0x7f800000);
            }
        }
#pragma unroll
        for (int o = 16; o > 0; o >>= 1) m = fmaxf(m, __shfl_xor_sync(0xFFFFFFFFu, m, o));
        if (lane == 0) s_max[warp] = m;
        __syncthreads();
        m = s_max[0];
        for (int w = 1; w < 8; w++) m = fmaxf(m, s_max[w]);
        __syncthreads();
        const float sc = m > 0.0f ? __fdiv_rn(m, 127.0f) : 1.0f;
        if (threadIdx.x == 0) tscale[t] = sc;
        for (uint32_t rr = warp; rr < (uint32_t)kQN; rr += 8) {
            const uint32_t r = t * kQN + rr;
            const bool real = r < n_rows;
            const float *x = reinterpret_cast<const float *>(src + (size_t)(real ? r : 0) * spitch);
            double res2 = 0.0, nrm2 = 0.0;
            for (uint32_t ci = lane; ci < num_kb * 8; ci += 32) {
                uint32_t w[4] = {0u, 0u, 0u, 0u};
#pragma unroll
                for (int g = 0; g < 4; g++) {
                    const uint32_t e = ci * 16 + g * 4;
                    if (!real || e >= dim) continue;
                    const float4 v = *reinterpret_cast<const float4 *>(x + e);
                    const float f[4] = {v.x, v.y, v.z, v.w};
#pragma unroll
                    for (int h = 0; h < 4; h++) {
                        const float qv = fminf(fmaxf(rintf(__fdiv_rn(f[h], sc)), -127.0f), 127.0f);
                        const double d = (double)f[h] - (double)sc * (double)qv;
                        res2 = fma(d, d, res2);
                        nrm2 = fma((double)f[h], (double)f[h], nrm2);
                        w[g] |= ((uint32_t)(int)qv & 0xFFu) << (8 * h);
                    }
                }
                const uint32_t kb = ci / 8, c = ci % 8;
                uint8_t *blk = dst + ((size_t)t * num_kb + kb) * kQBlockBytes;
                *reinterpret_cast<uint4 *>(blk + rr * 128 + ((c ^ (rr & 7)) * 16)) = make_uint4(w[0], w[1], w[2], w[3]);
            }
#pragma unroll
            for (int o = 16; o > 0; o >>= 1) {
                res2 += __shfl_xor_sync(0xFFFFFFFFu, res2, o);
                nrm2 += __shfl_xor_sync(0xFFFFFFFFu, nrm2, o);
            }
            const float rn = __double2float_ru(sqrt(res2));
            w_res = (rn == rn && w_res == w_res) ? fmaxf(w_res, rn) : __int_as_float(0x7fc00000);
            w_nrm = fmaxf(w_nrm, __double2float_ru(sqrt(nrm2)));
        }
    }
    if (lane == 0) {
        atomicMax(&stats[0], __float_as_uint(w_res));
        atomicMax(&stats[1], __float_as_uint(w_nrm));
    }
}

size_t coarse_shadow8_bytes(uint32_t rows, uint32_t dim) {
    return (size_t)((rows + kQN - 1) / kQN) * coarse_kb(dim) * kQBlockBytes;
}

cudaError_t launch_to_i8_tiled(const void *src, size_t spitch, uint32_t dim, uint32_t n_rows, uint32_t first, uint32_t n, void *dst,
                               float *d_tscale, uint32_t *d_stats, cudaStream_t s) {
    if (n == 0) return cudaSuccess;
    if (dim % 8 != 0 || spitch % 16 != 0) return cudaErrorInvalidValue;
    const uint32_t tile0 = first / kQN, ntiles = (first + n - 1) / kQN - tile0 + 1;
    const uint32_t grid = std::max(1u, std::min(ntiles, (uint32_t)device_sm_count() * 8));
    to_i8_tiled_kernel<<<grid, 256, 0, s>>>(static_cast<const uint8_t *>(src), spitch, dim, n_rows, tile0, ntiles, static_cast<uint8_t *>(dst),
                                            coarse_kb(dim), d_tscale, d_stats);
    return cudaGetLastError();
}

__global__ void __launch_bounds__(256) quantize_queries_kernel(const uint8_t *__restrict__ q, size_t qpitch, uint32_t dim, uint32_t nq,
                                                               uint8_t *__restrict__ q8, size_t pitch8, uint32_t payload,
                                                               float *__restrict__ eps, float delta_max, float x_max) {
    const int warp = threadIdx.x >> 5, lane = threadIdx.x & 31;
    const uint32_t i = blockIdx.x * 8 + warp;
    if (i >= nq) return;
    const float *x = reinterpret_cast<const float *>(q + (size_t)i * qpitch);
    float m = 0.0f;
    bool finite = true;
    for (uint32_t e = lane; e < dim; e += 32) {
        const float v = x[e];
        m = fmaxf(m, fabsf(v));
        finite = finite && fabsf(v) <= 3.4e38f;
    }
#pragma unroll
    for (int o = 16; o > 0; o >>= 1) m = fmaxf(m, __shfl_xor_sync(0xFFFFFFFFu, m, o));
    finite = __all_sync(0xFFFFFFFFu, finite);
    const float sc = (finite && m > 0.0f) ? __fdiv_rn(m, 127.0f) : 1.0f;
    double qn2 = 0.0, en2 = 0.0;
    uint8_t *dst = q8 + (size_t)i * pitch8;
    for (uint32_t e = lane; e < payload; e += 32) {
        int8_t b = 0;
        if (e < dim && finite) {
            const float v = x[e];
            const float qv = fminf(fmaxf(rintf(__fdiv_rn(v, sc)), -127.0f), 127.0f);
            const double d = (double)v - (double)sc * (double)qv;
            en2 = fma(d, d, en2);
            qn2 = fma((double)v, (double)v, qn2);
            b = (int8_t)(int)qv;
        }
        dst[e] = (uint8_t)b;
    }
#pragma unroll
    for (int o = 16; o > 0; o >>= 1) {
        qn2 += __shfl_xor_sync(0xFFFFFFFFu, qn2, o);
        en2 += __shfl_xor_sync(0xFFFFFFFFu, en2, o);
    }
    if (lane == 0) {
        *reinterpret_cast<float *>(dst + payload) = sc;
        const double qn = sqrt(qn2), en = sqrt(en2), X = (double)x_max, D = (double)delta_max;
        double e = qn * D + en * X + en * D + (double)(dim + 8) * 0x1p-23 * (qn + en) * (X + D) + 0x1p-21;
        e *= 1.0001;
        const float ef = __double2float_ru(e);
        eps[i] = (finite && isfinite(ef)) ? ef : __int_as_float(0x7fc00000);
    }
}

cudaError_t launch_quantize_queries(const void *d_q, size_t qpitch, uint32_t dim, uint32_t nq, void *d_q8, float *d_eps, float delta_max,
                                    float x_max, cudaStream_t s) {
    if (nq == 0) return cudaSuccess;
    quantize_queries_kernel<<<(nq + 7) / 8, 256, 0, s>>>(static_cast<const uint8_t *>(d_q), qpitch, dim, nq, static_cast<uint8_t *>(d_q8),
                                                         coarse_q8_pitch(dim), (uint32_t)coarse_q8_payload(dim), d_eps, delta_max, x_max);
    return cudaGetLastError();
}

template <int DT>
__global__ void __launch_bounds__(256) row_stats_kernel(const uint8_t *__restrict__ rows, size_t pitch, uint32_t dim, uint32_t first,
                                                        uint32_t n, float *__restrict__ norm2, uint32_t *__restrict__ stats) {
    const int warp = threadIdx.x >> 5, lane = threadIdx.x & 31;
    for (uint32_t r = blockIdx.x * 8 + warp; r < n; r += gridDim.x * 8) {
        const uint8_t *x = rows + (size_t)(first + r) * pitch;
        float s = 0.0f, m = 0.0f;
        for (uint32_t i = lane; i < dim; i += 32) {
            const float v = DT == DT_F32 ? reinterpret_cast<const float *>(x)[i] : load16<DT>(x, i);
            s = fmaf(v, v, s);
            m = fmaxf(m, fabsf(v));
            if (v != v) m = __int_as_float(0x7f800000);
        }
#pragma unroll
        for (int o = 16; o > 0; o >>= 1) {
            s += __shfl_xor_sync(0xFFFFFFFFu, s, o);
            m = fmaxf(m, __shfl_xor_sync(0xFFFFFFFFu, m, o));
        }
        if (lane == 0) {
            norm2[first + r] = m < 65520.0f ? s : __int_as_float(0x7fc00000);
            if (stats) {
                atomicMax(&stats[0], __float_as_uint(s));
                atomicMax(&stats[1], __float_as_uint(m));
            }
        }
    }
}
cudaError_t launch_row_stats(const void *rows, size_t pitch, uint32_t dim, uint32_t first, uint32_t n, float *d_norm2, uint32_t *d_stats,
                             cudaStream_t s, int dtype) {
    if (n == 0) return cudaSuccess;
    const uint32_t grid = std::max(1u, std::min((n + 7) / 8, (uint32_t)device_sm_count() * 8));
    const uint8_t *r = static_cast<const uint8_t *>(rows);
    if (dtype == DT_F32)
        row_stats_kernel<DT_F32><<<grid, 256, 0, s>>>(r, pitch, dim, first, n, d_norm2, d_stats);
    else if (dtype == DT_F16)
        row_stats_kernel<DT_F16><<<grid, 256, 0, s>>>(r, pitch, dim, first, n, d_norm2, d_stats);
    else if (dtype == DT_BF16)
        row_stats_kernel<DT_BF16><<<grid, 256, 0, s>>>(r, pitch, dim, first, n, d_norm2, d_stats);
    else
        return cudaErrorInvalidValue;
    return cudaGetLastError();
}

template <bool kSigned>
__global__ void __launch_bounds__(256) int_norm2_kernel(const uint8_t *__restrict__ rows, size_t pitch, uint32_t dim, uint32_t first,
                                                        uint32_t n, int32_t *__restrict__ norm2) {
    const int warp = threadIdx.x >> 5, lane = threadIdx.x & 31;
    for (uint32_t r = blockIdx.x * 8 + warp; r < n; r += gridDim.x * 8) {
        const uint8_t *x = rows + (size_t)(first + r) * pitch;
        int s = 0;
        for (uint32_t i = lane * 16; i < dim; i += 32 * 16) {
            const uint4 w = *reinterpret_cast<const uint4 *>(x + i);
            const uint32_t u[4] = {w.x, w.y, w.z, w.w};
#pragma unroll
            for (int t = 0; t < 4; t++) s = kSigned ? __dp4a((int)u[t], (int)u[t], s) : (int)__dp4a(u[t], u[t], (uint32_t)s);
        }
#pragma unroll
        for (int o = 16; o > 0; o >>= 1) s += __shfl_xor_sync(0xFFFFFFFFu, s, o);
        if (lane == 0) norm2[first + r] = s;
    }
}
cudaError_t launch_int_norm2(const void *rows, size_t pitch, uint32_t dim, uint32_t first, uint32_t n, bool is_signed, int32_t *d_norm2,
                             cudaStream_t s) {
    if (n == 0) return cudaSuccess;
    if (dim % 16 != 0 || pitch % 16 != 0 || dim > 2048) return cudaErrorInvalidValue;
    const uint32_t grid = std::max(1u, std::min((n + 7) / 8, (uint32_t)device_sm_count() * 8));
    const uint8_t *r = static_cast<const uint8_t *>(rows);
    if (is_signed)
        int_norm2_kernel<true><<<grid, 256, 0, s>>>(r, pitch, dim, first, n, d_norm2);
    else
        int_norm2_kernel<false><<<grid, 256, 0, s>>>(r, pitch, dim, first, n, d_norm2);
    return cudaGetLastError();
}

cudaError_t launch_to_f16(const void *src, size_t spitch, uint32_t dim, uint32_t first, uint32_t n, void *dst, size_t dpitch,
                          cudaStream_t s) {
    if (n == 0) return cudaSuccess;
    const size_t total = (size_t)n * (dim / 8);
    const uint32_t grid = (uint32_t)std::max<size_t>(1, std::min<size_t>((total + 255) / 256, (size_t)device_sm_count() * 16));
    to_f16_kernel<<<grid, 256, 0, s>>>(static_cast<const uint8_t *>(src), spitch, dim, first, n, static_cast<uint8_t *>(dst), dpitch);
    return cudaGetLastError();
}

cudaError_t launch_refine(const CorpusView &c, const void *d_queries, size_t qpitch, uint32_t nq, uint32_t lists_per_query, uint32_t keep,
                          uint32_t k, const uint64_t *d_cand, float eps, const float *d_q_norm2, float max_norm, uint32_t *d_ok,
                          uint64_t *d_out, const uint32_t *d_q_index, const uint32_t *d_nq_dev, cudaStream_t s, const float *d_thr_T,
                          const uint32_t *d_overflow, const uint64_t *d_row_label, const float *d_q_eps) {
    if (nq == 0) return cudaSuccess;
    const uint32_t okv = d_q_index ? 2u : 1u;
    const uint8_t *rows = static_cast<const uint8_t *>(c.rows), *qs = static_cast<const uint8_t *>(d_queries);
    const bool wide = k > kCoarseMaxK;
    if (k > kCoarseMaxKWide) return cudaErrorInvalidValue;
    const uint32_t max_cap = wide ? 8192 : 2560;
    const uint32_t smem_cap = std::min<uint32_t>(lists_per_query * keep, max_cap);
    const size_t smem = (size_t)smem_cap * 8;
    const auto kern = d_row_label ? (c.metric == MT_L2 ? (wide ? refine_kernel<MT_L2, kRefineMaxSurvWide, true> : refine_kernel<MT_L2, kRefineMaxSurv, true>)
                                                      : (wide ? refine_kernel<MT_IP, kRefineMaxSurvWide, true> : refine_kernel<MT_IP, kRefineMaxSurv, true>))
                    : c.metric == MT_L2 ? (wide ? refine_kernel<MT_L2, kRefineMaxSurvWide> : refine_kernel<MT_L2, kRefineMaxSurv>)
                                        : (wide ? refine_kernel<MT_IP, kRefineMaxSurvWide> : refine_kernel<MT_IP, kRefineMaxSurv>);
    cudaFuncAttributes fa{};
    cudaError_t e = cudaFuncGetAttributes(&fa, kern);
    if (e != cudaSuccess) return e;
    if (fa.sharedSizeBytes + (size_t)max_cap * 8 > 48 * 1024) {
        e = cudaFuncSetAttribute(kern, cudaFuncAttributeMaxDynamicSharedMemorySize, (int)(max_cap * 8));
        if (e != cudaSuccess) return e;
    }
    kern<<<nq, 256, smem, s>>>(rows, c.pitch, c.dim, qs, qpitch, nq, lists_per_query, keep, k, d_cand, eps, d_q_norm2, max_norm, d_ok, okv,
                               d_out, d_q_index, d_nq_dev, d_thr_T, d_overflow, smem_cap, d_row_label, d_q_eps);
    return cudaGetLastError();
}

cudaError_t launch_threshold(const uint64_t *d_cand, uint32_t nq, uint32_t lists_per_query, uint32_t keep, uint32_t k, float eps,
                             const float *d_q_norm2, float max_norm, uint32_t dim, int l2, float *d_thr, uint32_t *d_overflow, cudaStream_t s,
                             const float *d_q_eps) {
    if (nq == 0) return cudaSuccess;
    threshold_kernel<<<nq, 256, 0, s>>>(d_cand, nq, lists_per_query, keep, k, eps, d_q_norm2, max_norm, dim, l2, d_thr, d_overflow, d_q_eps);
    return cudaGetLastError();
}

__global__ void flags_from_overflow_kernel(const uint32_t *__restrict__ ovf, uint32_t nq, uint32_t *__restrict__ ok) {
    const uint32_t q = blockIdx.x * blockDim.x + threadIdx.x;
    if (q < nq) ok[q] = ovf[q] ? 0u : 1u;
}
cudaError_t launch_flags_from_overflow(const uint32_t *d_overflow, uint32_t nq, uint32_t *d_ok, cudaStream_t s) {
    if (nq == 0) return cudaSuccess;
    flags_from_overflow_kernel<<<(nq + 255) / 256, 256, 0, s>>>(d_overflow, nq, d_ok);
    return cudaGetLastError();
}
__global__ void scatter_rows_kernel(const uint64_t *__restrict__ src, const uint32_t *__restrict__ idx, const uint32_t *__restrict__ count,
                                    uint32_t k, uint64_t *__restrict__ dst, uint32_t *__restrict__ ok) {
    const uint32_t n = *count;
    for (uint32_t i = blockIdx.x; i < n; i += gridDim.x) {
        const uint32_t q = idx[i];
        for (uint32_t t = threadIdx.x; t < k; t += blockDim.x) dst[(size_t)q * k + t] = src[(size_t)i * k + t];
        if (threadIdx.x == 0) ok[q] = 2u;
    }
}
cudaError_t launch_scatter_rows(const uint64_t *d_src, const uint32_t *d_idx, const uint32_t *d_count, uint32_t max_n, uint32_t k,
                                uint64_t *d_dst, uint32_t *d_ok, cudaStream_t s) {
    if (max_n == 0) return cudaSuccess;
    scatter_rows_kernel<<<std::min(max_n, 256u), 128, 0, s>>>(d_src, d_idx, d_count, k, d_dst, d_ok);
    return cudaGetLastError();
}

cudaError_t launch_compact_unproven(const uint32_t *d_ok, uint32_t nq, uint32_t *d_idx, uint32_t *d_count, cudaStream_t s) {
    compact_unproven_kernel<<<1, 256, 0, s>>>(d_ok, nq, d_idx, d_count);
    return cudaGetLastError();
}
cudaError_t launch_range_bound(const float *d_radius, uint32_t nq, float eps, const float *d_q_norm2, float max_norm, uint32_t dim, int l2,
                               float *d_thr, uint32_t *d_overflow, uint32_t *d_total, cudaStream_t s) {
    if (nq == 0) return cudaSuccess;
    range_bound_kernel<<<(nq + 255) / 256, 256, 0, s>>>(d_radius, nq, eps, d_q_norm2, max_norm, dim, l2, d_thr, d_overflow, d_total);
    return cudaGetLastError();
}
cudaError_t launch_range_bound16(const void *d_queries, size_t qpitch, uint32_t nq, uint32_t dim, int dtype, const float *d_radius,
                                 float max_norm, float *d_thr, uint32_t *d_overflow, cudaStream_t s) {
    if (nq == 0) return cudaSuccess;
    const uint8_t *qs = static_cast<const uint8_t *>(d_queries);
    if (dtype == DT_F16)
        range_bound16_kernel<DT_F16><<<(nq + 7) / 8, 256, 0, s>>>(qs, qpitch, nq, dim, d_radius, max_norm, d_thr, d_overflow);
    else if (dtype == DT_BF16)
        range_bound16_kernel<DT_BF16><<<(nq + 7) / 8, 256, 0, s>>>(qs, qpitch, nq, dim, d_radius, max_norm, d_thr, d_overflow);
    else
        return cudaErrorInvalidValue;
    return cudaGetLastError();
}
cudaError_t launch_range_refine(const CorpusView &c, const void *d_queries, size_t qpitch, uint32_t nq, uint32_t slots, uint64_t *d_cand,
                                const float *d_radius, const float *d_q_norm2, const float *d_thr, const uint32_t *d_overflow, uint64_t *d_out,
                                uint32_t *d_total, uint32_t *d_ok, uint32_t *d_cnt, uint32_t *d_off, cudaStream_t s, uint32_t cap) {
    if (nq == 0) return cudaSuccess;
    const uint8_t *rows = static_cast<const uint8_t *>(c.rows), *qs = static_cast<const uint8_t *>(d_queries);
    if (c.dtype == DT_F32 && c.metric == MT_L2)
        range_refine_kernel<DT_F32, MT_L2><<<nq, 256, 0, s>>>(rows, c.pitch, c.dim, qs, qpitch, slots, d_cand, d_radius, d_q_norm2, d_thr,
                                                              d_overflow, d_out, d_total, d_ok, d_cnt, d_off, cap);
    else if (c.dtype == DT_F32 && c.metric == MT_IP)
        range_refine_kernel<DT_F32, MT_IP><<<nq, 256, 0, s>>>(rows, c.pitch, c.dim, qs, qpitch, slots, d_cand, d_radius, d_q_norm2, d_thr,
                                                              d_overflow, d_out, d_total, d_ok, d_cnt, d_off, cap);
    else if (c.dtype == DT_F16 && c.metric == MT_IP)
        range_refine_kernel<DT_F16, MT_IP><<<nq, 256, 0, s>>>(rows, c.pitch, c.dim, qs, qpitch, slots, d_cand, d_radius, d_q_norm2, d_thr,
                                                              d_overflow, d_out, d_total, d_ok, d_cnt, d_off, cap);
    else if (c.dtype == DT_BF16 && c.metric == MT_IP)
        range_refine_kernel<DT_BF16, MT_IP><<<nq, 256, 0, s>>>(rows, c.pitch, c.dim, qs, qpitch, slots, d_cand, d_radius, d_q_norm2, d_thr,
                                                               d_overflow, d_out, d_total, d_ok, d_cnt, d_off, cap);
    else
        return cudaErrorInvalidValue;
    return cudaGetLastError();
}
cudaError_t launch_range_pack(const uint64_t *d_cand, uint32_t nq, uint32_t slots, const uint32_t *d_overflow, uint32_t cap, uint64_t *d_out,
                              uint32_t *d_cnt, uint32_t *d_ok, cudaStream_t s) {
    if (nq == 0) return cudaSuccess;
    range_pack_kernel<<<nq, 256, 0, s>>>(d_cand, slots, d_overflow, cap, d_out, d_cnt, d_ok);
    return cudaGetLastError();
}
cudaError_t launch_range_label_fold(const uint64_t *d_cand, uint32_t nq, uint32_t slots, const uint32_t *d_front, const uint32_t *d_overflow,
                                    const uint64_t *d_id_to_label, uint32_t cap, uint64_t *d_out, uint32_t *d_cnt, uint32_t *d_ok,
                                    uint32_t *d_flags, cudaStream_t s) {
    if (nq == 0) return cudaSuccess;
    constexpr size_t smem = (size_t)kRangeFoldMaxHits * 12;
    cudaError_t e = cudaFuncSetAttribute(range_label_fold_kernel, cudaFuncAttributeMaxDynamicSharedMemorySize, (int)smem);
    if (e != cudaSuccess) return e;
    range_label_fold_kernel<<<nq, 512, smem, s>>>(d_cand, slots, d_front, d_overflow, d_id_to_label, cap, d_out, d_cnt, d_ok, d_flags);
    return cudaGetLastError();
}
cudaError_t launch_gather_queries(const void *d_src, size_t pitch, const float *d_src_n2, const uint32_t *d_idx, const uint32_t *d_count,
                                  uint32_t max_n, void *d_dst, float *d_dst_n2, cudaStream_t s) {
    if (max_n == 0) return cudaSuccess;
    gather_queries_kernel<<<std::min(max_n, 256u), 128, 0, s>>>(static_cast<const uint8_t *>(d_src), pitch, d_src_n2, d_idx, d_count,
                                                               static_cast<uint8_t *>(d_dst), d_dst_n2);
    return cudaGetLastError();
}

}
```

### redisearch_b200/csrc/coarse_tc.h

```cpp
#pragma once
#include "vecsim_kernels.h"

namespace rsb200 {

constexpr uint32_t kCoarseKeep = 24;
constexpr uint32_t kCoarseKeepWide = 128;
constexpr uint32_t kCoarseTier1MaxK = 16;
constexpr uint32_t kCoarseMaxK = 128;
constexpr uint32_t kCoarseMaxKWide = 1024;
constexpr uint32_t kCoarseFixedCapWide = 256;
constexpr uint32_t kCoarseSampleSlices = 32;
constexpr uint32_t kCoarseFixedCapDirect = 256;
constexpr uint32_t kCoarseFixedCapQ8 = 256;
constexpr uint32_t kCoarseFixedCap = 96;
constexpr uint32_t kRangeFoldMaxHits = 4096;
constexpr float kCoarseEpsTF32 = 2.5e-3f;
constexpr float kCoarseEpsF16 = 1.2e-3f;

enum CoarseKind : int { CoarseTF32 = 0, CoarseF16 = 1, CoarseDirect16 = 2, CoarseDirect8 = 3, CoarseQ8 = 4 };
inline float coarse_eps(CoarseKind k) { return k == CoarseF16 ? kCoarseEpsF16 : kCoarseEpsTF32; }

struct CoarsePlan {
    CoarseKind kind;
    uint32_t grid_x, grid_y, num_kb, tiles, keep;
    uint32_t stages;
    uint32_t threads;
    uint32_t epl;
    uint32_t tile_stride;
    int mode;
    uint32_t csize;
    uint32_t reg_kb;
    size_t cand_elems;
    size_t scratch_elems;
    size_t smem_bytes;
};

struct CoarseOperands {
    const void *rows;
    size_t pitch;
    const void *queries;
    size_t qpitch;
    int elem_variant;
    int epilogue;
    const float *row_norm2;
    const float *q_norm2;
};
bool coarse_supported(const CorpusView &c, uint32_t nq, uint32_t k, CoarseKind kind);
CoarsePlan plan_coarse(const CorpusView &c, uint32_t nq, CoarseKind kind, uint32_t k, uint32_t keep_override = 0, uint32_t tile_stride = 1,
                       int mode = 0, bool filt = false);
cudaError_t launch_coarse(const CoarseOperands &o, uint32_t n_rows, uint32_t dim, uint32_t nq, const CoarsePlan &p, uint64_t *d_cand,
                          uint64_t *d_scratch, cudaStream_t s, const uint32_t *d_nq_dev = nullptr, const float *d_thr_fixed = nullptr,
                          uint32_t *d_overflow = nullptr, const uint32_t *d_filt = nullptr, uint32_t filt_words = 0,
                          const uint32_t *d_filt_q = nullptr);
cudaError_t launch_threshold(const uint64_t *d_cand, uint32_t nq, uint32_t lists_per_query, uint32_t keep, uint32_t k, float eps,
                             const float *d_q_norm2, float max_norm, uint32_t dim, int l2, float *d_thr, uint32_t *d_overflow, cudaStream_t s,
                             const float *d_q_eps = nullptr);
size_t coarse_shadow_bytes(uint32_t rows, uint32_t dim);
cudaError_t launch_to_f16_tiled(const void *src, size_t spitch, uint32_t dim, uint32_t first, uint32_t n, void *dst, cudaStream_t s);
size_t coarse_shadow8_bytes(uint32_t rows, uint32_t dim);
cudaError_t launch_to_i8_tiled(const void *src, size_t spitch, uint32_t dim, uint32_t n_rows, uint32_t first, uint32_t n, void *dst,
                               float *d_tscale, uint32_t *d_stats, cudaStream_t s);
inline size_t coarse_q8_payload(uint32_t dim) { return (dim + 15) & ~(size_t)15; }
inline size_t coarse_q8_pitch(uint32_t dim) { return coarse_q8_payload(dim) + 16; }
cudaError_t launch_quantize_queries(const void *d_q, size_t qpitch, uint32_t dim, uint32_t nq, void *d_q8, float *d_eps, float delta_max,
                                    float x_max, cudaStream_t s);
cudaError_t launch_to_f16(const void *src, size_t spitch, uint32_t dim, uint32_t first, uint32_t n, void *dst, size_t dpitch,
                          cudaStream_t s);
cudaError_t launch_refine(const CorpusView &c, const void *d_queries, size_t qpitch, uint32_t nq, uint32_t lists_per_query, uint32_t keep,
                          uint32_t k, const uint64_t *d_cand, float eps, const float *d_q_norm2, float max_norm, uint32_t *d_ok,
                          uint64_t *d_out, const uint32_t *d_q_index, const uint32_t *d_nq_dev, cudaStream_t s,
                          const float *d_thr_T = nullptr, const uint32_t *d_overflow = nullptr, const uint64_t *d_row_label = nullptr,
                          const float *d_q_eps = nullptr);
cudaError_t launch_flags_from_overflow(const uint32_t *d_overflow, uint32_t nq, uint32_t *d_ok, cudaStream_t s);
cudaError_t launch_scatter_rows(const uint64_t *d_src, const uint32_t *d_idx, const uint32_t *d_count, uint32_t max_n, uint32_t k,
                                uint64_t *d_dst, uint32_t *d_ok, cudaStream_t s);
cudaError_t launch_compact_unproven(const uint32_t *d_ok, uint32_t nq, uint32_t *d_idx, uint32_t *d_count, cudaStream_t s);
cudaError_t launch_gather_queries(const void *d_src, size_t pitch, const float *d_src_n2, const uint32_t *d_idx, const uint32_t *d_count,
                                  uint32_t max_n, void *d_dst, float *d_dst_n2, cudaStream_t s);
cudaError_t launch_range_bound(const float *d_radius, uint32_t nq, float eps, const float *d_q_norm2, float max_norm, uint32_t dim, int l2,
                               float *d_thr, uint32_t *d_overflow, uint32_t *d_total, cudaStream_t s);
cudaError_t launch_range_bound16(const void *d_queries, size_t qpitch, uint32_t nq, uint32_t dim, int dtype, const float *d_radius,
                                 float max_norm, float *d_thr, uint32_t *d_overflow, cudaStream_t s);
cudaError_t launch_range_refine(const CorpusView &c, const void *d_queries, size_t qpitch, uint32_t nq, uint32_t slots, uint64_t *d_cand,
                                const float *d_radius, const float *d_q_norm2, const float *d_thr, const uint32_t *d_overflow, uint64_t *d_out,
                                uint32_t *d_total, uint32_t *d_ok, uint32_t *d_cnt, uint32_t *d_off, cudaStream_t s, uint32_t cap = 0);
cudaError_t launch_range_pack(const uint64_t *d_cand, uint32_t nq, uint32_t slots, const uint32_t *d_overflow, uint32_t cap, uint64_t *d_out,
                              uint32_t *d_cnt, uint32_t *d_ok, cudaStream_t s);
cudaError_t launch_range_label_fold(const uint64_t *d_cand, uint32_t nq, uint32_t slots, const uint32_t *d_front, const uint32_t *d_overflow,
                                    const uint64_t *d_id_to_label, uint32_t cap, uint64_t *d_out, uint32_t *d_cnt, uint32_t *d_ok,
                                    uint32_t *d_flags, cudaStream_t s);
cudaError_t launch_row_stats(const void *rows, size_t pitch, uint32_t dim, uint32_t first, uint32_t n, float *d_norm2, uint32_t *d_stats,
                             cudaStream_t s, int dtype = DT_F32);
cudaError_t launch_int_norm2(const void *rows, size_t pitch, uint32_t dim, uint32_t first, uint32_t n, bool is_signed, int32_t *d_norm2,
                             cudaStream_t s);

}
```

### redisearch_b200/csrc/vecsim_index.cpp

```cpp
#include "vecsim_index.h"
#include "batch_scratch.h"
#include "host_numeric.h"
#include "topk_common.cuh"
#include "coarse_tc.h"
#include "micro_batcher.h"

#include <algorithm>
#include <cmath>
#include <cstdarg>
#include <cstdio>
#include <cstdlib>
#include <cstring>
#include <chrono>
#include <limits>
#include <thread>

namespace rsb200 {

Globals &globals() {
    static Globals g;
    return g;
}

#define CU_OK(expr)                                                                                 \
// ... 793 lines not shown
        uint32_t h[2] = {0, 0}, h8[2] = {0, 0};
        if (stats && cudaMemcpyAsync(h, d_stats_, 8, cudaMemcpyDeviceToHost, st) != cudaSuccess) return false;
        if (d_shadow8_ && cudaMemcpyAsync(h8, d_stats8_, 8, cudaMemcpyDeviceToHost, st) != cudaSuccess) return false;
        if (cudaStreamSynchronize(st) != cudaSuccess) return false;
        if (d_shadow8_) {
            memcpy(&shadow8_delta_, &h8[0], 4);
            memcpy(&shadow8_xmax_, &h8[1], 4);
        }
        if (stats) {
            float n2, ma;
            memcpy(&n2, &h[0], 4);
            memcpy(&ma, &h[1], 4);
            shadow_max_norm_ = std::sqrt(n2);
            shadow_max_abs_ = ma;
        }
    }
    return true;
}

void FlatIndex::disable_coarse() {
    std::lock_guard<std::mutex> g(mu_);
    coarse_disabled_ = true;
    cudaFree(d_shadow_);
    cudaFree(d_shadow8_);
    cudaFree(d_tscale_);
    cudaFree(d_norm2_);
    d_shadow_ = nullptr;
    d_shadow8_ = nullptr;
    d_tscale_ = nullptr;
    d_norm2_ = nullptr;
    shadow_cap_ = shadow_rows_ = 0;
    shadow_dirty_.clear();
}

bool FlatIndex::shadow_values_in_range() {
    if (unit_rows() || shadow_max_abs_ <= 60000.0f) return true;
    disable_coarse();
    return false;
}

bool FlatIndex::shadow_operands(const void *d_q, size_t qpitch, uint32_t nq, uint8_t *q16, float *d_qn2, cudaStream_t st, LaunchCounters &lc,
                                CoarseOperands &ops) {
    const size_t q16_pitch = f16_query_pitch();
    ops = CoarseOperands{d_shadow_, 0, q16, q16_pitch, 0, mkind_ == MT_L2 ? 1 : 0, d_norm2_, d_qn2};
    bool ok = launch_to_f16(d_q, qpitch, (uint32_t)dim_, 0, nq, q16, q16_pitch, st) == cudaSuccess;
    if (d_qn2) ok = ok && launch_row_stats(d_q, qpitch, (uint32_t)dim_, 0, nq, d_qn2, nullptr, st) == cudaSuccess;
    lc.launches += d_qn2 ? 2 : 1;
    return ok;
}

bool FlatIndex::direct8_operands(const void *d_q, size_t qpitch, uint32_t nq, int32_t *d_qn, cudaStream_t st, LaunchCounters &lc,
                                 CoarseOperands &ops) {
    ops = CoarseOperands{d_rows_, pitch_, d_q, qpitch, dtype_ == DT_I8 ? 1 : 0, mkind_ == MT_COS ? 1 : int_l2() ? 2 : 0, nullptr, nullptr};
    if (!int_l2()) return true;
    ops.row_norm2 = reinterpret_cast<const float *>(d_norm2_);
    ops.q_norm2 = reinterpret_cast<const float *>(d_qn);
    lc.launches++;
    return launch_int_norm2(d_q, qpitch, (uint32_t)dim_, 0, nq, dtype_ == DT_I8, d_qn, st) == cudaSuccess;
}

void FlatIndex::RangeScratch::take(BatchScratch &s, const FlatIndex &ix, CoarseKind kind, const CoarsePlan &cp, uint32_t nq, bool fold) {
    const bool shadow = kind == CoarseF16, refine = kind != CoarseDirect8;
    cand = s.take<uint64_t>((size_t)nq * cp.grid_x * cp.keep);
    list_scratch = s.take<uint64_t>(cp.scratch_elems);
    q16 = s.take<uint8_t>(shadow ? nq * ix.f16_query_pitch() : 0);
    qn2 = s.take<float>((shadow && !ix.unit_rows()) || (kind == CoarseDirect8 && ix.int_l2()) ? nq : 0);
    thr = s.take<float>(refine ? nq : 0);
    ovf = s.take<uint32_t>(nq);
    front = s.take<uint32_t>(fold && refine ? nq : 0);
}

bool FlatIndex::enqueue_range_route(QueryCtx &c, const CorpusView &v, CoarseKind kind, const CoarsePlan &cp, const RangeScratch &r,
                                    const void *d_q, size_t qpitch, uint32_t nq, const float *d_radii, const uint32_t *bm, uint32_t words,
                                    const RangeOut &out, cudaStream_t st, LaunchCounters &lc) {
    const uint32_t slots = cp.grid_x * cp.keep;
    CoarseOperands ops{};
    bool ok;
    if (kind == CoarseDirect8) {
        ok = cudaMemsetAsync(r.ovf, 0, nq * 4, st) == cudaSuccess;
        ok = ok && direct8_operands(d_q, qpitch, nq, reinterpret_cast<int32_t *>(r.qn2), st, lc, ops);
    } else if (kind == CoarseDirect16) {
        ok = launch_range_bound16(d_q, qpitch, nq, (uint32_t)dim_, dtype_, d_radii, shadow_max_norm_, r.thr, r.ovf, st) == cudaSuccess;
        ops = CoarseOperands{v.rows, v.pitch, d_q, qpitch, dtype_ == DT_BF16 ? 1 : 0, 0, nullptr, nullptr};
        lc.launches++;
    } else {
        ok = shadow_operands(d_q, qpitch, nq, r.q16, r.qn2, st, lc, ops);
        ok = ok && launch_range_bound(d_radii, nq, kCoarseEpsF16, r.qn2, shadow_max_norm_, (uint32_t)dim_, mkind_ == MT_L2 ? 1 : 0, r.thr, r.ovf,
                                      out.total, st) == cudaSuccess;
        lc.launches++;
    }
    cudaEventRecord(c.ev_start, st);
    ok = ok && launch_coarse(ops, v.n_rows, v.dim, nq, cp, r.cand, r.list_scratch, st, nullptr, kind == CoarseDirect8 ? d_radii : r.thr, r.ovf, bm,
                             words) == cudaSuccess;
    cudaEventRecord(c.ev_stop, st);
    lc.launches += 2;
    if (kind == CoarseDirect8)
        return ok && (out.flags ? launch_range_label_fold(r.cand, nq, slots, nullptr, r.ovf, d_id_to_label_, out.cap, out.hits, out.cnt, out.ok,
                                                          out.flags, st)
                                : launch_range_pack(r.cand, nq, slots, r.ovf, out.cap, out.hits, out.cnt, out.ok, st)) == cudaSuccess;
    if (!out.flags)
        return ok && launch_range_refine(v, d_q, qpitch, nq, slots, r.cand, d_radii, r.qn2, r.thr, r.ovf, out.hits, out.total, out.ok, out.cnt,
                                         out.off, st, out.cap) == cudaSuccess;
    ok = ok && launch_range_refine(v, d_q, qpitch, nq, slots, r.cand, d_radii, r.qn2, r.thr, r.ovf, r.cand, out.total, out.ok, r.front, nullptr, st,
                                   slots) == cudaSuccess;
    lc.launches++;
    return ok && launch_range_label_fold(r.cand, nq, slots, r.front, nullptr, d_id_to_label_, out.cap, out.hits, out.cnt, out.ok, out.flags, st) ==
                     cudaSuccess;
}

bool FlatIndex::batch_scan(QueryCtx &c, const void *d_q, size_t qpitch, uint32_t nq, uint32_t ke, cudaStream_t st,
                           LaunchCounters &lc, uint64_t **d_result) {
    return multi_ ? batch_scan_labels(c, d_q, qpitch, nq, ke, st, lc, d_result) : batch_scan_rows(c, d_q, qpitch, nq, ke, st, lc, d_result);
}

static uint32_t sample_stride(const CoarsePlan &probe, uint32_t ke, double aim, double tiles_per_k) {
    const double f = std::min(0.25, std::max(0.01, (double)ke / (aim * probe.grid_x)));
    return (uint32_t)std::max(1.0, std::min(std::floor(1.0 / f), std::floor(probe.tiles / (tiles_per_k * ke))));
}

FlatIndex::KnnTiers FlatIndex::plan_knn_tiers(const CorpusView &v, uint32_t nq, CoarseKind kind, uint32_t ke, double aim, double tiles_per_k,
                                              bool filt) {
    KnnTiers t;
    const bool shadow = kind == CoarseF16 || kind == CoarseQ8;
    t.two_pass = shadow && coarse_fixed_enabled();
    t.tier2 = shadow && coarse_tier2_enabled();
    if (!t.two_pass) {
        t.main = plan_coarse(v, nq, kind, ke);
    } else {
        t.main = plan_coarse(v, nq, kind, ke, 0, 1, 1, filt);
        t.sample = ke > kCoarseMaxK ? plan_coarse(v, nq, kind, ke, kCoarseKeepWide, sample_stride(t.main, ke, aim, tiles_per_k), 0)
                                    : plan_coarse(v, nq, kind, ke, 0, sample_stride(t.main, ke, aim, tiles_per_k), 2);
    }
    if (t.tier2) t.second = plan_coarse(v, nq, kind, ke, kCoarseKeepWide);
    return t;
}

void FlatIndex::KnnScratch::take(BatchScratch &s, const KnnTiers &t, uint32_t nq, size_t q_pitch, bool norms, bool q8) {
    cand = s.take<uint64_t>((size_t)nq * t.main.grid_x * t.main.keep);
    cand_s = s.take<uint64_t>(t.two_pass ? (size_t)nq * t.sample.grid_x * t.sample.keep : 0);
    cand_t2 = s.take<uint64_t>(t.tier2 ? (size_t)nq * t.second.grid_x * t.second.keep : 0);
    list_scratch = s.take<uint64_t>(std::max(std::max(t.main.scratch_elems, t.two_pass ? t.sample.scratch_elems : 0),
                                             t.tier2 ? t.second.scratch_elems : 0));
    q = s.take<uint8_t>(nq * q_pitch);
    q_t2 = s.take<uint8_t>(t.tier2 ? nq * q_pitch : 0);
    qn2 = s.take<float>(norms ? nq : 0);
    qn2_t2 = s.take<float>(norms && t.tier2 ? nq : 0);
    qeps = s.take<float>(q8 ? nq : 0);
    qeps_t2 = s.take<float>(q8 && t.tier2 ? nq : 0);
    ok = s.take<uint32_t>(nq);
    idx = s.take<uint32_t>(nq);
    n2 = s.take<uint32_t>(nq ? 1 : 0);
    thr = s.take<float>(nq);
    ovf = s.take<uint32_t>(nq);
}

bool FlatIndex::enqueue_knn_tiers(QueryCtx &c, const CorpusView &v, CoarseKind kind, const KnnTiers &t, const KnnScratch &s,
                                  const CoarseOperands &ops, const void *d_q32, size_t qpitch, uint32_t nq, uint32_t ke, uint64_t *out,
                                  const uint32_t *bm, uint32_t words, const uint64_t *row_label, cudaStream_t st, LaunchCounters &lc) {
    const float eps = coarse_eps(kind);
    bool ok = true;
    if (t.two_pass) {
        ok = launch_coarse(ops, v.n_rows, v.dim, nq, t.sample, s.cand_s, s.list_scratch, st, nullptr, nullptr, nullptr, bm, words) == cudaSuccess;
        ok = ok && launch_threshold(s.cand_s, nq, t.sample.grid_x, t.sample.keep, ke, eps, s.qn2, shadow_max_norm_, (uint32_t)dim_,
                                    mkind_ == MT_L2 ? 1 : 0, s.thr, s.ovf, st, s.qeps) == cudaSuccess;
        lc.launches += 2;
    }
    const float *thr = t.two_pass ? s.thr : nullptr;
    uint32_t *ovf = t.two_pass ? s.ovf : nullptr;
    cudaEventRecord(c.ev_start, st);
    ok = ok && launch_coarse(ops, v.n_rows, v.dim, nq, t.main, s.cand, s.list_scratch, st, nullptr, thr, ovf, bm, words) == cudaSuccess;
    cudaEventRecord(c.ev_stop, st);
    ok = ok && launch_refine(v, d_q32, qpitch, nq, t.main.grid_x, t.main.keep, ke, s.cand, eps, s.qn2, shadow_max_norm_, s.ok, out, nullptr,
                             nullptr, st, thr, ovf, row_label, s.qeps) == cudaSuccess;
    lc.launches += 2;
    if (!t.tier2) return ok;
    ok = ok && launch_compact_unproven(s.ok, nq, s.idx, s.n2, st) == cudaSuccess;
    ok = ok && launch_gather_queries(ops.queries, ops.qpitch, s.qeps ? s.qeps : s.qn2, s.idx, s.n2, nq, s.q_t2, s.qeps ? s.qeps_t2 : s.qn2_t2,
                                     st) == cudaSuccess;
    CoarseOperands ops2 = ops;
    ops2.queries = s.q_t2;
    if (ops.q_norm2) ops2.q_norm2 = s.qn2_t2;
    ok = ok && launch_coarse(ops2, v.n_rows, v.dim, nq, t.second, s.cand_t2, s.list_scratch, st, s.n2, nullptr, nullptr, bm, words,
                             bm ? s.idx : nullptr) == cudaSuccess;
    ok = ok && launch_refine(v, d_q32, qpitch, nq, t.second.grid_x, t.second.keep, ke, s.cand_t2, eps, s.qn2_t2, shadow_max_norm_, s.ok, out,
                             s.idx, s.n2, st, nullptr, nullptr, row_label, s.qeps_t2) == cudaSuccess;
    lc.launches += 4;
    return ok;
}

bool FlatIndex::batch_scan_rows(QueryCtx &c, const void *d_q, size_t qpitch, uint32_t nq, uint32_t ke, cudaStream_t st,
                                LaunchCounters &lc, uint64_t **d_result, bool tc_only) {
    const CorpusView v = view();
    const ScanPlan sp = plan_scan_topk(v, nq, ke);
    const int cmode = coarse_mode();
    const bool is16 = dtype_ == DT_F16 || dtype_ == DT_BF16, is8 = dtype_ == DT_I8 || dtype_ == DT_U8;
    const CoarseKind dkind = is16 ? CoarseDirect16 : CoarseDirect8;
    if (cmode != 0 && nq >= 16 && (is16 || is8) && coarse_supported(v, nq, ke, dkind) && (!int_l2() || ensure_shadow(st))) {
        const CoarseOperands ops16{v.rows, v.pitch, d_q, qpitch, dtype_ == DT_BF16 ? 1 : 0, mkind_ == MT_COS ? 1 : 0, nullptr, nullptr};
        last_batch_coarse_ = true;
        last_batch_path_ = 2;
        c.d_last_ok = nullptr;
        c.last_ok_n = 0;
        const CoarsePlan cp = plan_coarse(v, nq, dkind, ke);
        const CoarsePlan probe = plan_coarse(v, nq, dkind, ke, 0, 1, 1);
        if (is16 && probe.mode == 1 && coarse_fixed_enabled()) {
            const CoarsePlan cps = plan_coarse(v, nq, dkind, ke, 0, sample_stride(probe, ke, 64.0, 2.0), 2);
            const bool tier2 = coarse_tier2_enabled();
            const size_t nO = (size_t)nq * ke;
            const size_t scratch = std::max(std::max(probe.scratch_elems, cps.scratch_elems), tier2 ? cp.scratch_elems : 0);
            uint64_t *cand_m, *cand_s, *cand_t2, *out2, *list_scratch;
            uint8_t *q_t2;
            uint32_t *d_ok, *d_idx, *d_n2, *d_ovf;
            float *d_thr;
            const auto layout = [&](void *base) {
                BatchScratch s(base);
                cand_m = s.take<uint64_t>((size_t)nq * probe.grid_x * probe.keep);
                cand_s = s.take<uint64_t>((size_t)nq * cps.grid_x * cps.keep);
                cand_t2 = s.take<uint64_t>(tier2 ? (size_t)nq * cp.grid_x * cp.keep : 0);
                out2 = s.take<uint64_t>(nO);
                list_scratch = s.take<uint64_t>(scratch);
                q_t2 = s.take<uint8_t>(tier2 ? (size_t)nq * qpitch : 0);
                d_ok = s.take<uint32_t>(nq);
                d_idx = s.take<uint32_t>(nq);
                d_n2 = s.take<uint32_t>(1);
                d_thr = s.take<float>(nq);
                d_ovf = s.take<uint32_t>(nq);
                return s.words();
            };
            if (!c.need_cand(layout(nullptr)) || !c.need_out(nO)) return false;
            layout(c.d_cand);
            c.d_last_ok = d_ok;
            c.last_ok_n = nq;
            bool ok = launch_coarse(ops16, v.n_rows, v.dim, nq, cps, cand_s, list_scratch, st) == cudaSuccess;
            ok = ok && launch_threshold(cand_s, nq, cps.grid_x, cps.keep, ke, 0.0f, nullptr, 0.0f, (uint32_t)dim_, 0, d_thr, d_ovf, st) == cudaSuccess;
            cudaEventRecord(c.ev_start, st);
            ok = ok && launch_coarse(ops16, v.n_rows, v.dim, nq, probe, cand_m, list_scratch, st, nullptr, d_thr, d_ovf) == cudaSuccess;
            cudaEventRecord(c.ev_stop, st);
            ok = ok && launch_final_select(cand_m, nq, (uint32_t)(probe.grid_x * probe.keep), ke, c.d_out, st, &lc) == cudaSuccess;
            ok = ok && launch_flags_from_overflow(d_ovf, nq, d_ok, st) == cudaSuccess;
            lc.launches += 4;
            if (tier2) {
                ok = ok && launch_compact_unproven(d_ok, nq, d_idx, d_n2, st) == cudaSuccess;
                ok = ok && launch_gather_queries(d_q, qpitch, nullptr, d_idx, d_n2, nq, q_t2, nullptr, st) == cudaSuccess;
                CoarseOperands ops2 = ops16;
                ops2.queries = q_t2;
                ok = ok && launch_coarse(ops2, v.n_rows, v.dim, nq, cp, cand_t2, list_scratch, st, d_n2) == cudaSuccess;
                ok = ok && launch_final_select(cand_t2, nq, (uint32_t)(cp.grid_x * cp.keep), ke, out2, st, &lc, d_n2) == cudaSuccess;
                ok = ok && launch_scatter_rows(out2, d_idx, d_n2, nq, ke, c.d_out, d_ok, st) == cudaSuccess;
                lc.launches += 4;
            }
            coarse_batches_++;
            *d_result = c.d_out;
            return ok;
        }
        uint64_t *cand, *list_scratch;
        int32_t *d_qn;
        const auto layout = [&](void *base) {
            BatchScratch s(base);
            cand = s.take<uint64_t>((size_t)nq * cp.grid_x * cp.keep);
            list_scratch = s.take<uint64_t>(cp.scratch_elems);
            d_qn = s.take<int32_t>(int_l2() ? nq : 0);
            return s.words();
        };
        if (!c.need_cand(layout(nullptr)) || !c.need_out((size_t)nq * ke)) return false;
        layout(c.d_cand);
        CoarseOperands ops = ops16;
        bool ok = !is8 || direct8_operands(d_q, qpitch, nq, d_qn, st, lc, ops);
        cudaEventRecord(c.ev_start, st);
        ok = ok && launch_coarse(ops, v.n_rows, v.dim, nq, cp, cand, list_scratch, st) == cudaSuccess;
        cudaEventRecord(c.ev_stop, st);
        ok = ok && launch_final_select(cand, nq, (uint32_t)(cp.grid_x * cp.keep), ke, c.d_out, st, &lc) == cudaSuccess;
        lc.launches++;
        coarse_batches_++;
        *d_result = c.d_out;
        return ok;
    }
    CoarseKind kind = cmode == 2 ? CoarseTF32 : CoarseF16;
    const bool unit = unit_rows();
    const bool wide = ke > kCoarseMaxK;
    const bool eligible = cmode != 0 && !coarse_disabled_ && dtype_ == DT_F32 && (unit || cmode == 1) &&
                          (nq >= 16 || (!wide && single_query_takes_coarse(ke, nullptr, q8_route(nq, ke)))) && (!wide || coarse_fixed_enabled());
    if (eligible && kind == CoarseF16 && q8_route(nq, ke) && ensure_shadow(st, true) && std::isfinite(shadow8_delta_) &&
        std::isfinite(shadow8_xmax_))
        kind = CoarseQ8;
    bool coarse = eligible && coarse_supported(v, nq, ke, kind);
    if (eligible && kind == CoarseF16 && (!coarse || !ensure_shadow(st))) {
        kind = CoarseTF32;
        coarse = unit && coarse_supported(v, nq, ke, kind);
    }
    if (coarse && !shadow_values_in_range()) coarse = false;
    last_batch_coarse_ = coarse;
    last_batch_path_ = coarse ? 1 : 0;
    last_shadow_bits_ = !coarse ? 0 : kind == CoarseQ8 ? 8 : kind == CoarseF16 ? 16 : 0;
    if (!coarse && tc_only) {
        *d_result = nullptr;
        return true;
    }
    const WidePlan wp = wide ? plan_topk_wide(v.n_rows, nq) : WidePlan{};
    if (!coarse && wide) {
        if (!c.need_scores(wp.score_elems) || !c.need_cand(wp.cand_elems) || !c.need_out((size_t)nq * ke)) return false;
        cudaEventRecord(c.ev_start, st);
        const bool ok = launch_topk_wide(v, d_q, qpitch, nq, ke, nullptr, nullptr, wp, c.d_scores, c.d_cand, c.d_out, c.d_abort, st, &lc) ==
                        cudaSuccess;
        cudaEventRecord(c.ev_stop, st);
        *d_result = c.d_out;
        return ok;
    }
    if (!coarse) {
        if (!c.need_cand(sp.cand_elems) || !c.need_out((size_t)nq * ke)) return false;
        cudaEventRecord(c.ev_start, st);
        bool ok = launch_scan_topk(v, d_q, qpitch, nq, ke, sp, c.d_cand, st, &lc, nullptr, c.d_abort) == cudaSuccess;
        cudaEventRecord(c.ev_stop, st);
        ok = ok && launch_final_select(c.d_cand, nq, sp.lists_per_query * ke, ke, c.d_out, st, &lc) == cudaSuccess;
        *d_result = c.d_out;
        return ok;
    }
    const bool q8 = kind == CoarseQ8, shadow = kind == CoarseF16 || q8;
    const KnnTiers t = plan_knn_tiers(v, nq, kind, ke, wide ? 128.0 : q8 ? 8.0 : 24.0, wide ? 1 / 32.0 : 2.0, false);
    const size_t nO = (size_t)nq * ke;
    const size_t q_pitch = !shadow ? 0 : q8 ? coarse_q8_pitch((uint32_t)dim_) : f16_query_pitch();
    const size_t nO12 = wide ? 0 : nO;
    KnnScratch ks;
    uint64_t *out1, *out2, *cand2;
    const auto layout = [&](void *base) {
        BatchScratch s(base);
        ks.take(s, t, nq, q_pitch, !unit, q8);
// ... 1374 lines not shown
```

### redisearch_b200/csrc/vecsim_index.h

```cpp
#pragma once
#include "../../include/vecsim_b200.h"
#include "coarse_tc.h"
#include "vecsim_kernels.h"

#include <atomic>
#include <map>
#include <memory>
#include <limits>
#include <memory>
#include <mutex>
#include <string>
#include <unordered_map>
#include <unordered_set>
#include <vector>

struct VecSimQueryResult {
    size_t id;
    double score;
};
struct VecSimQueryReply {
    std::vector<VecSimQueryResult> results;
    VecSimQueryReply_Code code = VecSim_QueryReply_OK;
};
struct VecSimQueryReply_Iterator {
// ... 58 lines not shown
class FlatIndex;

struct BatchIter {
    FlatIndex *index;
    std::vector<uint8_t> query;
    void *timeout_ctx;
    std::unique_ptr<QueryCtx> ctx;
    bool scored = false;
    uint32_t n_rows = 0;
    size_t label_count = 0;
    size_t returned = 0;
    bool has_cursor = false;
    uint64_t cursor = 0;
    std::unordered_set<size_t> seen;
    std::vector<size_t> id_to_label_snap;
};

struct AdhocCtx {
    FlatIndex *index;
    std::vector<uint8_t> query;
    std::unique_ptr<QueryCtx> ctx;
    bool query_on_device = false;
};

class FlatIndex {
  public:
    static FlatIndex *create(const BFParams &p, void *log_ctx);
    ~FlatIndex();

    int add(const void *blob, size_t label);
    int add_bulk(const void *blobs, size_t stride, size_t n, const size_t *labels, size_t label0);
    int add_bulk_device(const void *d_rows, size_t n, size_t label0);
    int remove(size_t label);
    size_t size() const { return count_; }
    size_t label_count() const { return multi_ ? label_to_ids_.size() : label_to_id_.size(); }
    bool reserve(size_t rows);
    bool flush();

    VecSimQueryReply *topk(const void *q, size_t k, VecSimQueryParams *qp, VecSimQueryReply_Order order);
    VecSimQueryReply *topk_combined(const void *q, size_t k, VecSimQueryParams *qp, VecSimQueryReply_Order order);
    static int microbatch_window_us();
    int topk_batch(const void *qs, size_t qstride, size_t nq, size_t k, VecSimQueryParams *qp, size_t *out_labels,
                   double *out_scores);
    int topk_batch_device(const void *d_q, size_t nq, size_t k, int64_t *d_labels, float *d_scores, cudaStream_t s);
    VecSimQueryReply *range(const void *q, double radius, VecSimQueryParams *qp, VecSimQueryReply_Order order);
    int range_batch(const void *qs, size_t qstride, size_t nq, const double *radii, VecSimQueryParams *qp, VecSimQueryReply_Order order,
                    VecSimQueryReply **replies, uint32_t *out_flags);
    int range_batch_device(const void *d_q, size_t nq, const float *d_radii, size_t cap, VecSimQueryReply_Order order, int64_t *d_labels,
                           float *d_scores, uint32_t *d_counts, cudaStream_t s);
    int label_range_batch_device(const void *d_q, size_t nq, const float *d_radii, size_t cap, VecSimQueryReply_Order order, int64_t *d_labels,
                                 float *d_scores, uint32_t *d_counts, cudaStream_t s);
    int hybrid_range_batch_device(const void *d_q, size_t nq, const float *d_radii, size_t cap, VecSimQueryReply_Order order,
                                  const uint32_t *const *d_doc_ids, const uint32_t *const *d_counts, const size_t *caps, VecSimQueryParams *qp,
                                  int64_t *d_labels, float *d_scores, uint32_t *d_counts_out, int *out_modes, cudaStream_t s);
    double distance_from(size_t label, const void *stored_form_blob);
    bool prefer_adhoc(size_t subset, size_t k, bool initial);

    BatchIter *batch_new(const void *q, VecSimQueryParams *qp);
    VecSimQueryReply *batch_next(BatchIter *it, size_t n, VecSimQueryReply_Order order);

    AdhocCtx *adhoc_new(const void *q);
    void adhoc_distances(AdhocCtx *c, const size_t *labels, double *out, size_t n);
    int topk_filtered(const void *q, size_t k, const uint32_t *doc_ids, size_t n, bool ids_on_device, size_t *out_labels,
                      double *out_scores, size_t *out_count);
    int topk_filtered_batch(const void *const *queries, size_t nq, size_t k, const uint32_t *const *d_doc_ids, const size_t *counts,
                            size_t *out_labels, double *out_scores, size_t *out_counts);
    int topk_filtered_batch_device(const void *d_q, size_t nq, size_t k, const uint32_t *const *d_doc_ids, const uint32_t *const *d_counts,
                                   const size_t *caps, int64_t *d_labels, float *d_scores, uint32_t *d_counts_out, cudaStream_t s);
    int hybrid_topk_batch_device(const void *d_q, size_t nq, size_t k, const uint32_t *const *d_doc_ids, const uint32_t *const *d_counts,
                                 const size_t *caps, VecSimQueryParams *qp, int64_t *d_labels, float *d_scores, uint32_t *d_counts_out,
                                 int *out_modes, cudaStream_t s);

    VecSimIndexBasicInfo basic_info() const;
    VecSimIndexStatsInfo stats_info() const;
    VecSimIndexDebugInfo debug_info() const;
    VecSimDebugInfoIterator *debug_iterator() const;
    void set_last_mode(VecSearchMode m) { last_mode_ = m; }
    VecSimB200_Stats get_stats(bool reset);
    int last_coarse_flags(uint32_t *out, size_t n);
    const void *device_rows(size_t *pitch, size_t *rows) {
        flush();
        *pitch = pitch_;
        *rows = count_;
        return d_rows_;
    }

    bool read_rows(size_t first, size_t n, void *host_dst);
    size_t query_blob_bytes() const { return stored_bytes_; }
    void preprocess_query(const void *blob, uint8_t *dst) const;
    void preprocess_storage(const void *blob, uint8_t *dst) const;

    VecSimType type_;
    VecSimMetric metric_;
    size_t dim_;
    bool multi_;
    size_t block_size_;
    void *log_ctx_;

    void log(const char *level, const char *fmt, ...) const;

  private:
    FlatIndex() = default;
    CorpusView view() const;
    std::unique_ptr<QueryCtx> checkout();
    void checkin(std::unique_ptr<QueryCtx> c);
    bool grow_to(size_t rows);
    bool sync_labels_to_device();
    bool timed_out(void *ctx) const;
    int wait_polling(cudaStream_t s, void *timeout_ctx) const;
    int wait_or_abandon(QueryCtx &c, void *timeout_ctx) const;
    void record_scan(const QueryCtx *c, uint64_t bytes);
    long select_from_scores(QueryCtx &c, uint32_t n, bool has_cursor, uint64_t cursor, size_t want);
    size_t query_pitch() const { return (stored_bytes_ + 15) & ~(size_t)15; }
    size_t f16_query_pitch() const { return (dim_ * 2 + 15) & ~(size_t)15; }
    bool stage_queries(QueryCtx &c, const void *blobs, size_t stride, size_t nq, bool raw, const void *tail = nullptr, size_t tail_bytes = 0);
    bool batch_scan(QueryCtx &c, const void *d_q, size_t qpitch, uint32_t nq, uint32_t ke, cudaStream_t st, LaunchCounters &lc,
                    uint64_t **d_result);
    bool batch_scan_rows(QueryCtx &c, const void *d_q, size_t qpitch, uint32_t nq, uint32_t ke, cudaStream_t st, LaunchCounters &lc,
                         uint64_t **d_result, bool tc_only = false);
    bool batch_scan_labels(QueryCtx &c, const void *d_q, size_t qpitch, uint32_t nq, uint32_t kl, cudaStream_t st, LaunchCounters &lc,
                           uint64_t **d_result, bool host_fallback = false);

    bool shadow_operands(const void *d_q, size_t qpitch, uint32_t nq, uint8_t *q16, float *d_qn2, cudaStream_t st, LaunchCounters &lc,
                         CoarseOperands &ops);
    bool direct8_operands(const void *d_q, size_t qpitch, uint32_t nq, int32_t *d_qn, cudaStream_t st, LaunchCounters &lc, CoarseOperands &ops);
    bool shadow_values_in_range();

    struct RangeScratch {
        uint64_t *cand = nullptr, *list_scratch = nullptr;
        uint8_t *q16 = nullptr;
        float *qn2 = nullptr, *thr = nullptr;
        uint32_t *ovf = nullptr, *front = nullptr;
        void take(BatchScratch &s, const FlatIndex &ix, CoarseKind kind, const CoarsePlan &cp, uint32_t nq, bool fold);
    };
    struct RangeOut {
        uint64_t *hits;
        uint32_t cap;
        uint32_t *ok, *cnt, *off, *total, *flags;
    };
    bool enqueue_range_route(QueryCtx &c, const CorpusView &v, CoarseKind kind, const CoarsePlan &cp, const RangeScratch &r, const void *d_q,
                             size_t qpitch, uint32_t nq, const float *d_radii, const uint32_t *bm, uint32_t words, const RangeOut &out,
                             cudaStream_t st, LaunchCounters &lc);

    struct KnnTiers {
        CoarsePlan main{}, sample{}, second{};
        bool two_pass = false, tier2 = false;
    };
    static KnnTiers plan_knn_tiers(const CorpusView &v, uint32_t nq, CoarseKind kind, uint32_t ke, double aim, double tiles_per_k, bool filt);
    struct KnnScratch {
        uint64_t *cand = nullptr, *cand_s = nullptr, *cand_t2 = nullptr, *list_scratch = nullptr;
        uint8_t *q = nullptr, *q_t2 = nullptr;
        float *qn2 = nullptr, *qn2_t2 = nullptr, *qeps = nullptr, *qeps_t2 = nullptr, *thr = nullptr;
        uint32_t *ok = nullptr, *idx = nullptr, *n2 = nullptr, *ovf = nullptr;
        void take(BatchScratch &s, const KnnTiers &t, uint32_t nq, size_t q_pitch, bool norms, bool q8);
    };
    bool enqueue_knn_tiers(QueryCtx &c, const CorpusView &v, CoarseKind kind, const KnnTiers &t, const KnnScratch &s, const CoarseOperands &ops,
                           const void *d_q32, size_t qpitch, uint32_t nq, uint32_t ke, uint64_t *out, const uint32_t *bm, uint32_t words,
                           const uint64_t *row_label, cudaStream_t st, LaunchCounters &lc);

    static size_t ragged_table_elems(size_t nq, size_t tail_words) { return 4 * nq + 2 + (tail_words + 1) / 2; }
    bool upload_ragged_table(uint64_t *d_tab, const uint32_t *const *d_doc_ids, const uint32_t *const *d_counts, const size_t *caps, uint32_t nq,
                             const std::vector<uint32_t> &tail, cudaStream_t st, RaggedBatch &b, bool &ok);
    void finish_reply(VecSimQueryReply *rep, VecSimQueryReply_Order order) const;

    DType dtype_;
    MetricKind mkind_;
    size_t elem_bytes_ = 0;
    size_t stored_bytes_ = 0;
    size_t pitch_ = 0;

    uint8_t *d_rows_ = nullptr;
    uint8_t *d_shadow_ = nullptr;
    size_t shadow_cap_ = 0, shadow_rows_ = 0;
    uint8_t *d_shadow8_ = nullptr;
    float *d_tscale_ = nullptr;
    uint32_t *d_stats8_ = nullptr;
    float shadow8_delta_ = 0.0f, shadow8_xmax_ = 0.0f;
    float *d_norm2_ = nullptr;
    uint32_t *d_stats_ = nullptr;
    float shadow_max_norm_ = 0.0f, shadow_max_abs_ = std::numeric_limits<float>::infinity();
    std::atomic<bool> coarse_disabled_{false};
    std::atomic<bool> raw_rows_{false};
    bool unit_rows() const { return metric_ == VecSimMetric_Cosine && !raw_rows_; }
    std::vector<idType> shadow_dirty_;
    bool keeps_row_copies() const { return d_shadow_ || d_shadow8_ || d_norm2_; }
    bool int_l2() const { return (dtype_ == DT_I8 || dtype_ == DT_U8) && mkind_ == MT_L2; }
    bool ensure_shadow(cudaStream_t st, bool q8 = false);
    bool q8_route(uint32_t nq, uint32_t ke) const;
    void disable_coarse();
    bool single_query_takes_coarse(uint32_t ke, const float *host_query = nullptr, bool q8 = false);
    size_t capacity_ = 0;
    size_t count_ = 0;
    size_t resident_ = 0;
    uint8_t *h_stage_ = nullptr;
    size_t stage_cap_rows_ = 0;
    cudaStream_t copy_stream_ = nullptr;

    std::vector<size_t> id_to_label_;
    std::unordered_map<size_t, idType> label_to_id_;
    std::unordered_map<size_t, std::vector<idType>> label_to_ids_;
    std::map<size_t, size_t> rows_per_label_;
    void label_rows_changed(size_t from, size_t to);
    size_t max_rows_per_label() const;
    uint64_t *d_id_to_label_ = nullptr;
    size_t d_labels_cap_ = 0;
    bool labels_dirty_ = true;
    uint32_t *d_label_to_id_ = nullptr;
    size_t l2i_size_ = 0, l2i_cap_ = 0;
    uint32_t *d_label_rows_ = nullptr;
    size_t label_rows_cap_ = 0;
    bool l2i_dirty_ = true;
    bool sync_label_table();
    int range_device(const void *d_q, size_t nq, const float *d_radii, size_t cap, VecSimQueryReply_Order order, int64_t *d_labels,
                     float *d_scores, uint32_t *d_counts, cudaStream_t s);

    mutable std::mutex mu_;
    std::mutex pool_mu_;
    std::vector<std::unique_ptr<QueryCtx>> pool_;
    mutable VecSearchMode last_mode_ = EMPTY_MODE;

    std::atomic<uint64_t> launches_total_{0};
    std::atomic<uint64_t> coarse_batches_{0};
    bool last_batch_coarse_ = false;
    int last_batch_path_ = 0;
  public:
    int last_batch_path() const { return last_batch_path_; }
    int last_shadow_bits_ = 0;
    int last_shadow_bits() const { return last_shadow_bits_; }
  private:
    std::unique_ptr<QueryCtx> dev_ctx_;
    std::mutex dev_mu_;
    struct TableSlot {
        uint64_t *h = nullptr;
        size_t cap = 0;
        cudaEvent_t ev = nullptr;
    };
    std::vector<TableSlot> table_ring_;
    TableSlot *table_slot(size_t elems);
    bool dev_timing_pending_ = false;
    uint64_t dev_timing_bytes_ = 0;
    void collect_dev_timing_locked();
    std::atomic<uint64_t> scan_launches_{0};
    std::atomic<uint64_t> scan_bytes_{0};
    double scan_us_ = 0;
    std::mutex stats_mu_;
    struct TopkReq;
    std::mutex mb_mu_;
    std::map<size_t, std::shared_ptr<void>> batchers_;
    friend struct BatchIter;
};

}
```

Baseline: 73940.

## Use fragment-register epilogue for int8 sample pass and count-compacted refine

Extends the register-fragment epilogue (two consumer warpgroups, 128-query CTAs) to the int8 sample pass, reducing per-slice maxima straight from accumulator fragments instead of staging through shared memory, and adds L2 prefetch for that pass. The int8 fixed pass now writes only live list entries plus a per-list count, so refine can prefix-scan the counts and copy exactly the live candidates rather than scanning padded slots. Refine also moves to 512 threads with a larger counted smem capacity, and the kth-key radix select uses a parallel block scan instead of a serial thread-0 loop. The cost is more register pressure, more shared memory, and extra count-buffer plumbing.

```diff
diff --git a/redisearch_b200/csrc/coarse_tc.cu b/redisearch_b200/csrc/coarse_tc.cu
--- a/redisearch_b200/csrc/coarse_tc.cu
+++ b/redisearch_b200/csrc/coarse_tc.cu
@@ -496,9 +496,10 @@
 }
 constexpr int kQAccStride = kQN + 4;
 constexpr uint32_t kQAccBytes = kQM * kQAccStride * 4;
-__host__ __device__ constexpr int coarse_consumers(int mode) { return mode == 1 ? 2 : 1; }
-__host__ __device__ constexpr int coarse_cta_queries(bool q8, int mode) { return q8 && mode == 1 ? 2 * kQM : kQM; }
-__host__ __device__ constexpr int coarse_threads(int mode) { return 128 * (1 + coarse_consumers(mode)); }
+__host__ __device__ constexpr bool coarse_frag_epilogue(bool q8, int mode) { return mode == 1 || (q8 && mode == 2); }
+__host__ __device__ constexpr int coarse_consumers(bool q8, int mode) { return coarse_frag_epilogue(q8, mode) ? 2 : 1; }
+__host__ __device__ constexpr int coarse_cta_queries(bool q8, int mode) { return q8 && (mode == 1 || mode == 2) ? 2 * kQM : kQM; }
+__host__ __device__ constexpr int coarse_threads(bool q8, int mode) { return 128 * (1 + coarse_consumers(q8, mode)); }
 
 template <int kId, int kCount>
 __device__ __forceinline__ void named_sync() {
@@ -621,19 +622,21 @@
 }
 
 template <bool kDirect, int kEpl, int kOp, int kMode, int kVar = 0, bool kFilt = false, int kRegKb = 0>
-__global__ void __launch_bounds__(coarse_threads(kMode), 1)
+__global__ void __launch_bounds__(coarse_threads(kOp == 5, kMode), 1)
 coarse_wgmma_kernel(const __grid_constant__ CUtensorMap map_rows, const uint8_t *__restrict__ shadow, size_t row_pitch,
                     const uint8_t *__restrict__ q16, size_t q16_pitch, const float *__restrict__ row_norm2,
                     const float *__restrict__ q_norm2, uint32_t n_rows, uint32_t nq, uint32_t dim, uint32_t row_bytes,
                     uint32_t num_kb, uint32_t tiles_total, uint32_t keep, uint32_t nstages, uint32_t csize,
                     uint64_t *__restrict__ list_scratch, uint64_t *__restrict__ cand_out, const uint32_t *__restrict__ nq_dev,
                     uint32_t tile_stride, const float *__restrict__ thr_fixed, uint32_t *__restrict__ overflow,
-                    const uint32_t *__restrict__ filt, uint32_t filt_words, const uint32_t *__restrict__ filt_q) {
+                    const uint32_t *__restrict__ filt, uint32_t filt_words, const uint32_t *__restrict__ filt_q,
+                    uint32_t *__restrict__ list_count) {
     constexpr bool kFixed = kMode == 1, kSample = kMode == 2;
     constexpr bool kQ8 = kOp == 5;
     constexpr bool kInt = kOp == 1 || kOp == 2 || kOp == 4 || kQ8;
     constexpr int kOpE = kQ8 ? 0 : kOp;
-    constexpr int kCons = coarse_consumers(kMode), kConsThreads = 128 * kCons;
+    constexpr bool kFrag = coarse_frag_epilogue(kQ8, kMode);
+    constexpr int kCons = coarse_consumers(kQ8, kMode), kConsThreads = 128 * kCons;
     constexpr int kCtaQ = coarse_cta_queries(kQ8, kMode);
     constexpr bool kWide = kCtaQ > kQM;
     static_assert(!kWide || (kCons == 2 && kCtaQ == kCons * kQM), "a wide CTA: one consumer warpgroup per 64 queries");
@@ -648,7 +651,9 @@
     static_assert(kRegKb == 0 || (!kDirect && kFixed && kRegKb % kQKbPerStage == 0),
                   "register-held queries: the fixed-bound pass over the fp16 shadow, whole stages");
     auto filt_row = [&](uint32_t pos) { return filt + (size_t)filt_words * (filt_q ? filt_q[pos] : pos); };
-    constexpr int kSliceSets = (int)kCoarseSampleSlices / (kQN / 32);
+    constexpr int kSliceSets = (int)kCoarseSampleSlices / (kFrag ? 8 : kQN / 32);
+    static_assert(!kSample || kSliceSets * (kFrag ? 8 : kQN / 32) == (int)kCoarseSampleSlices, "whole slice sets");
+    static_assert(!(kSample && kFrag) || kSliceSets == kQN / 32, "kFrag: a slice per 32-row chunk and (lane % 4, c)");
     constexpr int kQListCap = kEpl * 32;
     if (nq_dev) {
         nq = min(nq, *nq_dev);
@@ -660,7 +665,7 @@
     uint8_t *sB = smem;
     uint8_t *sQ = sB + (size_t)nstages * kQStageBytes;
     uint32_t *sacc = reinterpret_cast<uint32_t *>(sQ + (size_t)(num_kb - kRegKb) * kQKbBytes);
-    uint64_t *bars = reinterpret_cast<uint64_t *>(sacc + (kFixed ? 0 : kQM * kQAccStride));
+    uint64_t *bars = reinterpret_cast<uint64_t *>(sacc + (kFrag ? 0 : kQM * kQAccStride));
     uint64_t *full = bars, *empty = bars + kQMaxStages;
     uint32_t *qcount = reinterpret_cast<uint32_t *>(bars + 2 * kQMaxStages);
     uint64_t *lists = list_scratch + (size_t)(by * gx + bx) * (kQListCap * kQListStride);
@@ -711,8 +716,9 @@
                         }
                     } else {
                         const uint8_t *src = shadow + ((size_t)tile * num_kb + kb0) * kQBlockBytes;
-                        if constexpr (kFixed) {
-                            if (i + 1 < my_tiles) bulk_prefetch_l2(src + (size_t)gx * num_kb * kQBlockBytes + crank * slice, slice);
+                        if constexpr (kFixed || (kSample && kFrag)) {
+                            const size_t ahead = (size_t)gx * (kFixed ? 1u : tile_stride) * num_kb * kQBlockBytes;
+                            if (i + 1 < my_tiles) bulk_prefetch_l2(src + ahead + crank * slice, slice);
                         }
                         if (csize > 1) {
                             bulk_load_1d_mc(sB + (size_t)s * kQStageBytes + crank * slice, src + crank * slice, slice, &full[s], cmask);
@@ -868,7 +874,7 @@
             }
             const uint32_t rbase = tile * kQN + 2 * (lane & 3);
             float q8_st = 0.0f;
-            if constexpr (kFixed && kQ8) q8_st = __ldg(row_norm2 + tile);
+            if constexpr (kFrag && kQ8) q8_st = __ldg(row_norm2 + tile);
             float2 rn[(kFixed && kOp == 3) ? kQN / 8 : 1];
             if constexpr (kFixed && kOp == 3) {
 #pragma unroll
@@ -938,6 +944,27 @@
             wg_wait<0>();
             release(prev);
             wg_fence_operands(acc);
+            if constexpr (kSample && kQ8) {
+                const bool tail = tile * kQN + kQN > n_rows;
+#pragma unroll
+                for (int i2 = 0; i2 < 2; i2++) {
+                    const float sqt = __fmul_rn(fsq[i2], q8_st);
+#pragma unroll
+                    for (int c = 0; c < 2; c++)
+#pragma unroll
+                        for (int h = 0; h < kQN / 32; h++) {
+                            int v[4];
+#pragma unroll
+                            for (int u = 0; u < 4; u++) {
+                                const int j = 4 * h + u;
+                                v[u] = (!tail || rbase + 8 * j + c < n_rows) ? (int)acc[4 * j + 2 * i2 + c] : INT_MIN;
+                            }
+                            const int mx = max(__vimax3_s32(v[0], v[1], v[2]), v[3]);
+                            if (mx != INT_MIN) smax[h][2 * i2 + c] = fmaxf(smax[h][2 * i2 + c], __fmul_rn(sqt, __int2float_rn(mx)));
+                        }
+                }
+                continue;
+            }
             if constexpr (kFixed && kQ8) {
                 const float st = q8_st, rst = __frcp_rn(st);
 #pragma unroll
@@ -1276,11 +1303,31 @@
                 if (qq >= nq) break;
                 const uint32_t n = qcount[qs], c = min(n, (uint32_t)kQListCap);
                 uint64_t *dst = cand_out + ((size_t)qq * gx + bx) * keep;
-                for (uint32_t r = lane; r < keep; r += 32) dst[r] = r < c ? lists[r * kQListStride + qs] : kEmptySlot;
+                if constexpr (kQ8) {
+                    for (uint32_t r = lane; r < c; r += 32) dst[r] = lists[r * kQListStride + qs];
+                } else {
+                    for (uint32_t r = lane; r < keep; r += 32) dst[r] = r < c ? lists[r * kQListStride + qs] : kEmptySlot;
+                }
+                if (lane == 0 && list_count) list_count[(size_t)qq * gx + bx] = c;
                 if (lane == 0 && n > (uint32_t)kQListCap) overflow[qq] = 1u;
             }
         }
-        if constexpr (kSample) {
+        if constexpr (kSample && kFrag) {
+#pragma unroll
+            for (int i2 = 0; i2 < 2; i2++) {
+                const uint32_t fq = qw + 16 * ew + (lane >> 2) + 8 * i2;
+                if (fq >= nq) continue;
+                uint64_t *dst = cand_out + ((size_t)fq * gx + bx) * keep + 8 * (lane & 3);
+#pragma unroll
+                for (int c = 0; c < 2; c++)
+#pragma unroll
+                    for (int h = 0; h < kQN / 32; h++) {
+                        const float m = smax[h][2 * i2 + c];
+                        dst[4 * c + h] = m > -__int_as_float(0x7f800000) ? (uint64_t)orderable_key(1.0f - m) << 32 : kEmptySlot;
+                    }
+            }
+        }
+        if constexpr (kSample && !kFrag) {
             if (live) {
                 uint64_t *dst = cand_out + ((size_t)q * gx + bx) * keep;
 #pragma unroll
@@ -1336,6 +1383,9 @@
 
 constexpr uint32_t kRefineMaxSurv = 2048;
 constexpr uint32_t kRefineMaxSurvWide = 4096;
+constexpr uint32_t kRefineMaxLists = 256;
+constexpr uint32_t kRefineThreads = 512;
+constexpr uint32_t kRefineCapPadded = 2560, kRefineCapWide = 8192, kRefineCapCounted = 8192;
 
 __device__ __forceinline__ float query_eps(float eps, const float *q_norm2, uint32_t pos, float max_norm, uint32_t dim, bool l2,
                                            const float *q_eps = nullptr) {
@@ -1346,36 +1396,54 @@
     if (l2) e = 2.0f * e + (float)(dim + 4) * 1.2e-7f * (max_norm * max_norm + qn2);
     return e * 1.0001f;
 }
-__device__ __forceinline__ uint32_t block_kth_key(const uint64_t *mine, uint32_t total, uint32_t k, uint32_t *hist, uint32_t *ctl) {
+__device__ __forceinline__ uint32_t block_incl_scan(uint32_t v, uint32_t *wsum, uint32_t *total) {
+    const int lane = threadIdx.x & 31, warp = threadIdx.x >> 5, nw = blockDim.x >> 5;
+#pragma unroll
+    for (int o = 1; o < 32; o <<= 1) {
+        const uint32_t y = __shfl_up_sync(0xFFFFFFFFu, v, o);
+        if (lane >= o) v += y;
+    }
+    if (lane == 31) wsum[warp] = v;
+    __syncthreads();
+    uint32_t base = 0, all = 0;
+    for (int w = 0; w < nw; w++) {
+        const uint32_t x = wsum[w];
+        if (w < warp) base += x;
+        all += x;
+    }
+    *total = all;
+    return v + base;
+}
+
+template <class At>
+__device__ __forceinline__ uint32_t block_kth_key(At at, uint32_t total, uint32_t k, uint32_t *hist, uint32_t *ctl) {
     const int lane = threadIdx.x & 31;
     if (threadIdx.x == 0) ctl[0] = 0, ctl[1] = k, ctl[2] = 0;
     __syncthreads();
     uint32_t cnt = 0;
-    for (uint32_t i = threadIdx.x; i < total; i += blockDim.x) cnt += mine[i] != kEmptySlot;
+    for (uint32_t i = threadIdx.x; i < total; i += blockDim.x) cnt += at(i) != kEmptySlot;
     cnt = __reduce_add_sync(0xFFFFFFFFu, cnt);
     if (lane == 0 && cnt) atomicAdd(&ctl[2], cnt);
     __syncthreads();
     if (ctl[2] < k) return 0xFFFFFFFFu;
     for (int shift = 24; shift >= 0; shift -= 8) {
-        hist[threadIdx.x] = 0;
+        if (threadIdx.x < 256) hist[threadIdx.x] = 0;
         __syncthreads();
-        const uint32_t prefix = ctl[0];
+        const uint32_t prefix = ctl[0], rem = ctl[1];
         const uint32_t hi_mask = shift == 24 ? 0u : ~((1u << (shift + 8)) - 1u);
         for (uint32_t i = threadIdx.x; i < total; i += blockDim.x) {
-            const uint64_t c = mine[i];
+            const uint64_t c = at(i);
             if (c == kEmptySlot) continue;
             const uint32_t key = (uint32_t)(c >> 32);
             if (((key ^ prefix) & hi_mask) == 0) atomicAdd(&hist[(key >> shift) & 255u], 1u);
         }
         __syncthreads();
-        if (threadIdx.x == 0) {
-            uint32_t rem = ctl[1], b = 0;
-            for (; b < 255; b++) {
-                if (hist[b] >= rem) break;
-                rem -= hist[b];
-            }
-            ctl[0] = prefix | (b << shift);
-            ctl[1] = rem;
+        const uint32_t h = threadIdx.x < 256 ? hist[threadIdx.x] : 0u;
+        uint32_t all;
+        const uint32_t incl = block_incl_scan(h, hist + 256, &all), excl = incl - h;
+        if (excl < rem && (incl >= rem || threadIdx.x == 255)) {
+            ctl[0] = prefix | (threadIdx.x << shift);
+            ctl[1] = rem - excl;
         }
         __syncthreads();
     }
@@ -1386,11 +1454,12 @@
                                                         uint32_t keep, uint32_t k, float eps, const float *__restrict__ q_norm2,
                                                         float max_norm, uint32_t dim, int l2, float *__restrict__ thr_out,
                                                         uint32_t *__restrict__ overflow, const float *__restrict__ q_eps) {
-    __shared__ uint32_t hist[256];
+    __shared__ uint32_t hist[256 + 16];
     __shared__ uint32_t ctl[4];
     const uint32_t q = blockIdx.x;
     if (q >= nq) return;
-    const uint32_t ak = block_kth_key(cand + (size_t)q * lists_per_query * keep, lists_per_query * keep, k, hist, ctl);
+    const uint64_t *mine = cand + (size_t)q * lists_per_query * keep;
+    const uint32_t ak = block_kth_key([&](uint32_t i) { return mine[i]; }, lists_per_query * keep, k, hist, ctl);
     if (threadIdx.x == 0) {
         const float e = query_eps(eps, q_norm2, q, max_norm, dim, l2 != 0, q_eps);
         float T;
@@ -1406,53 +1475,73 @@
 }
 
 template <int MT, uint32_t kSurv, bool kLab = false>
-__global__ void __launch_bounds__(256) refine_kernel(const uint8_t *rows, size_t pitch, uint32_t dim, const uint8_t *queries,
+__global__ void __launch_bounds__(kRefineThreads) refine_kernel(const uint8_t *rows, size_t pitch, uint32_t dim, const uint8_t *queries,
                                                      size_t qpitch, uint32_t nq, uint32_t lists_per_query, uint32_t keep, uint32_t k,
                                                      const uint64_t *__restrict__ cand, float eps, const float *__restrict__ q_norm2,
                                                      float max_norm, uint32_t *__restrict__ ok, uint32_t ok_value, uint64_t *__restrict__ out,
                                                      const uint32_t *__restrict__ q_index, const uint32_t *__restrict__ nq_dev,
                                                      const float *__restrict__ thr_T, const uint32_t *__restrict__ overflow,
-                                                     uint32_t smem_cap, const uint64_t *__restrict__ row_label, const float *__restrict__ q_eps) {
+                                                     uint32_t smem_cap, const uint64_t *__restrict__ row_label, const float *__restrict__ q_eps,
+                                                     const uint32_t *__restrict__ list_count) {
     using Tile = DistTile<DT_F32, MT, 1, 1>;
     __shared__ uint64_t surv[kSurv];
-    __shared__ uint32_t hist[256];
+    __shared__ uint32_t hist[256 + 16];
     __shared__ uint32_t ctl[4];
     __shared__ uint32_t s_nsurv, s_bad, s_ncomp;
+    __shared__ uint32_t s_off[kRefineMaxLists], s_cnt[kRefineMaxLists];
     if (nq_dev) nq = min(nq, *nq_dev);
     if (blockIdx.x >= nq) return;
     const uint32_t q = q_index ? q_index[blockIdx.x] : blockIdx.x;
     const int warp = threadIdx.x >> 5, lane = threadIdx.x & 31;
+    constexpr uint32_t kWarps = kRefineThreads / 32;
     const uint64_t *mine = cand + (size_t)blockIdx.x * lists_per_query * keep;
     uint32_t total = lists_per_query * keep;
     eps = query_eps(eps, q_norm2, blockIdx.x, max_norm, dim, MT == MT_L2, q_eps);
     if (threadIdx.x == 0) s_nsurv = 0, s_bad = 0, s_ncomp = 0;
     __syncthreads();
     extern __shared__ uint64_t s_cand[];
-    for (uint32_t i0 = 0; i0 < total; i0 += blockDim.x) {
-        const uint32_t i = i0 + threadIdx.x;
-        const uint64_t c = i < total ? mine[i] : kEmptySlot;
-        const uint32_t m = __ballot_sync(0xFFFFFFFFu, c != kEmptySlot);
-        uint32_t base = 0;
-        if (lane == 0 && m) base = atomicAdd(&s_ncomp, (uint32_t)__popc(m));
-        base = __shfl_sync(0xFFFFFFFFu, base, 0);
-        if (c != kEmptySlot) {
-            const uint32_t pos = base + __popc(m & ((1u << lane) - 1u));
-            if (pos < smem_cap) s_cand[pos] = c;
+    if (list_count) {
+        const uint32_t cl = threadIdx.x < lists_per_query ? min(list_count[(size_t)blockIdx.x * lists_per_query + threadIdx.x], keep) : 0u;
+        uint32_t n_live;
+        const uint32_t incl = block_incl_scan(cl, hist + 256, &n_live);
+        if (threadIdx.x < lists_per_query) s_off[threadIdx.x] = incl - cl, s_cnt[threadIdx.x] = cl;
+        if (threadIdx.x == 0) s_ncomp = n_live;
+        __syncthreads();
+        if (n_live <= smem_cap) {
+            for (uint32_t l = warp; l < lists_per_query; l += kWarps) {
+                const uint64_t *src = mine + (size_t)l * keep;
+                uint64_t *dst = s_cand + s_off[l];
+                for (uint32_t j = lane; j < s_cnt[l]; j += 32) dst[j] = src[j];
+            }
+        }
+    } else {
+        for (uint32_t i0 = 0; i0 < total; i0 += blockDim.x) {
+            const uint32_t i = i0 + threadIdx.x;
+            const uint64_t c = i < total ? mine[i] : kEmptySlot;
+            const uint32_t m = __ballot_sync(0xFFFFFFFFu, c != kEmptySlot);
+            uint32_t base = 0;
+            if (lane == 0 && m) base = atomicAdd(&s_ncomp, (uint32_t)__popc(m));
+            base = __shfl_sync(0xFFFFFFFFu, base, 0);
+            if (c != kEmptySlot) {
+                const uint32_t pos = base + __popc(m & ((1u << lane) - 1u));
+                if (pos < smem_cap) s_cand[pos] = c;
+            }
         }
     }
     __syncthreads();
     const bool packed = s_ncomp <= smem_cap;
     const uint64_t *mine_all = mine;
-    const uint32_t total_all = total;
-    if (packed) {
-        mine = s_cand;
-        total = s_ncomp;
-    }
-    const uint32_t ak_key = block_kth_key(mine, total, k, hist, ctl);
+    if (packed) total = s_ncomp;
+    auto at = [&](uint32_t i) -> uint64_t {
+        if (packed) return s_cand[i];
+        if (list_count) return i % keep < s_cnt[i / keep] ? mine[i] : kEmptySlot;
+        return mine[i];
+    };
+    const uint32_t ak_key = block_kth_key(at, total, k, hist, ctl);
     const float cut = ak_key == 0xFFFFFFFFu ? __int_as_float(0x7f800000) : key_to_float(ak_key) + (2.0f * eps) * 1.001f + 1e-30f;
     for (uint32_t i0 = 0; i0 < total; i0 += blockDim.x) {
         const uint32_t i = i0 + threadIdx.x;
-        const uint64_t c = i < total ? mine[i] : kEmptySlot;
+        const uint64_t c = i < total ? at(i) : kEmptySlot;
         const bool take = c != kEmptySlot && (ak_key == 0xFFFFFFFFu || key_to_float((uint32_t)(c >> 32)) <= cut);
         const uint32_t m = __ballot_sync(0xFFFFFFFFu, take);
         uint32_t base = 0;
@@ -1465,8 +1554,16 @@
     }
     __syncthreads();
     const uint32_t n_all = s_nsurv, n_surv = min(n_all, kSurv);
+    uint32_t touch = 0;
+    {
+        const uint32_t row_bytes = dim * (uint32_t)sizeof(float), lines = (row_bytes + 127) / 128;
+        for (uint32_t t = threadIdx.x; t < n_surv * lines; t += blockDim.x) {
+            const uint8_t *r = rows + (size_t)(uint32_t)surv[t / lines] * pitch;
+            touch ^= __ldcg(reinterpret_cast<const uint32_t *>(r + (t % lines) * 128));
+        }
+    }
     const uint8_t *qb[1] = {queries + (size_t)q * qpitch};
-    for (uint32_t i = warp; i < n_surv; i += 8) {
+    for (uint32_t i = warp; i < n_surv; i += kWarps) {
         const uint32_t row = (uint32_t)surv[i];
         const uint8_t *rowb[1] = {rows + (size_t)row * pitch};
         float d[1];
@@ -1487,7 +1584,6 @@
     if (thr_T) {
         if (threadIdx.x == 0 && (overflow[blockIdx.x] != 0 || !have_k || !(thr_T[blockIdx.x] - eps > ek))) bad = true;
     } else {
-        (void)total_all;
         for (uint32_t l = threadIdx.x; l < lists_per_query; l += blockDim.x) {
             const uint64_t *lst = mine_all + (size_t)l * keep;
             uint32_t worst = 0;
@@ -1509,6 +1605,7 @@
     if (bad) atomicOr(&s_bad, 1u);
     __syncthreads();
     if (threadIdx.x == 0) ok[q] = s_bad ? 0u : ok_value;
+    asm volatile("" ::"r"(touch));
 }
 
 constexpr uint32_t kRangeWindow = 2048;
@@ -1831,14 +1928,14 @@
     if (l2) return epl == 3 ? (const void *)coarse_wgmma_kernel<false, 3, 3, 0> : (const void *)coarse_wgmma_kernel<false, 8, 3, 0>;
     return epl == 3 ? (const void *)coarse_wgmma_kernel<false, 3, 0, 0> : (const void *)coarse_wgmma_kernel<false, 8, 0, 0>;
 }
-static size_t wgmma_fixed_smem(uint32_t num_kb, int mode = 0, uint32_t reg_kb = 0, uint32_t cta_q = kQM) {
-    return 1024 + (size_t)(num_kb - reg_kb) * cta_q * 128 + (mode == 1 ? cta_q * 4 : kQAccBytes) + 2 * kQMaxStages * 8 + 64;
-}
-static uint32_t wgmma_stages(uint32_t num_kb, int mode, uint32_t reg_kb, uint32_t cta_q = kQM) {
-    return (uint32_t)std::min<size_t>(kQMaxStages, (kSmemLimit - wgmma_fixed_smem(num_kb, mode, reg_kb, cta_q)) / kQStageBytes);
+static size_t wgmma_fixed_smem(uint32_t num_kb, bool frag = false, uint32_t reg_kb = 0, uint32_t cta_q = kQM) {
+    return 1024 + (size_t)(num_kb - reg_kb) * cta_q * 128 + (frag ? cta_q * 4 : kQAccBytes) + 2 * kQMaxStages * 8 + 64;
+}
+static uint32_t wgmma_stages(uint32_t num_kb, bool frag, uint32_t reg_kb, uint32_t cta_q = kQM) {
+    return (uint32_t)std::min<size_t>(kQMaxStages, (kSmemLimit - wgmma_fixed_smem(num_kb, frag, reg_kb, cta_q)) / kQStageBytes);
 }
 static bool wgmma_fits_bytes(uint32_t row_bytes, uint32_t cta_q = kQM) {
-    return wgmma_fixed_smem(coarse_kb(row_bytes), 0, 0, cta_q) + 2 * (size_t)kQStageBytes <= kSmemLimit;
+    return wgmma_fixed_smem(coarse_kb(row_bytes), false, 0, cta_q) + 2 * (size_t)kQStageBytes <= kSmemLimit;
 }
 static bool wgmma_fits(uint32_t dim) { return wgmma_fits_bytes(dim * 2); }
 
@@ -1899,7 +1996,8 @@
         if (p.mode == 1 && (kind == CoarseDirect16 || kind == CoarseDirect8)) p.keep = kCoarseFixedCapDirect, p.epl = 8;
         if (p.mode == 1 && kind == CoarseQ8) p.keep = kCoarseFixedCapQ8, p.epl = 8;
         if (p.mode == 2) p.keep = kCoarseSampleSlices, p.epl = 3;
-        p.threads = (uint32_t)coarse_threads(p.mode);
+        p.threads = (uint32_t)coarse_threads(kind == CoarseQ8, p.mode);
+        const bool frag = coarse_frag_epilogue(kind == CoarseQ8, p.mode);
         const int epi = kind == CoarseQ8 ? 0 : kind == CoarseF16 ? (c.metric == MT_L2 ? 1 : 0) : c.metric == MT_COS ? 1 : (kind == CoarseDirect8 && c.metric == MT_L2) ? 2 : 0;
         static int rcap = -1;
         if (rcap < 0) {
@@ -1909,11 +2007,11 @@
         p.reg_kb = 0;
         if (kind == CoarseF16 && p.mode == 1) {
             const uint32_t rk = fixed_reg_kb(p.epl, epi != 0, filt);
-            if (rk && (int)rk <= rcap && p.num_kb >= rk + kQKbPerStage && wgmma_stages(p.num_kb, p.mode, rk) > wgmma_stages(p.num_kb, p.mode, 0))
+            if (rk && (int)rk <= rcap && p.num_kb >= rk + kQKbPerStage && wgmma_stages(p.num_kb, frag, rk) > wgmma_stages(p.num_kb, frag, 0))
                 p.reg_kb = rk;
         }
-        p.stages = wgmma_stages(p.num_kb, p.mode, p.reg_kb, cta_q);
-        p.smem_bytes = wgmma_fixed_smem(p.num_kb, p.mode, p.reg_kb, cta_q) + (size_t)p.stages * kQStageBytes;
+        p.stages = wgmma_stages(p.num_kb, frag, p.reg_kb, cta_q);
+        p.smem_bytes = wgmma_fixed_smem(p.num_kb, frag, p.reg_kb, cta_q) + (size_t)p.stages * kQStageBytes;
         p.csize = 1;
         static int ccap = -1;
         if (ccap < 0) {
@@ -1980,10 +2078,11 @@
 
 cudaError_t launch_coarse(const CoarseOperands &o, uint32_t n_rows, uint32_t dim, uint32_t nq, const CoarsePlan &p, uint64_t *d_cand,
                           uint64_t *d_scratch, cudaStream_t s, const uint32_t *d_nq_dev, const float *d_thr_fixed, uint32_t *d_overflow,
-                          const uint32_t *d_filt, uint32_t filt_words, const uint32_t *d_filt_q) {
+                          const uint32_t *d_filt, uint32_t filt_words, const uint32_t *d_filt_q, uint32_t *d_list_count) {
     if (d_filt && p.kind != CoarseF16 && !(p.kind == CoarseDirect8 && p.mode == 1)) return cudaErrorInvalidValue;
     if (p.kind == CoarseF16 || p.kind == CoarseQ8 || p.kind == CoarseDirect16 || p.kind == CoarseDirect8) {
         if (p.mode == 1 && (!d_thr_fixed || !d_overflow)) return cudaErrorInvalidValue;
+        if (p.mode == 1 && p.kind == CoarseQ8 && !d_list_count) return cudaErrorInvalidValue;
         const uint32_t ev = (p.kind == CoarseDirect16 || p.kind == CoarseDirect8) && o.elem_variant ? 1u : 0u;
         const void *kfn = wgmma_kernel_fn(p.kind, p.epl, o.epilogue, p.mode, ev, d_filt != nullptr, p.reg_kb);
         if (!kfn) return cudaErrorInvalidValue;
@@ -2020,7 +2119,7 @@
                  a_st = p.stages, a_cs = p.csize, a_stride = p.tile_stride;
         void *args[] = {&mr,   &rows,    &rp,     &qs,   &qp,   &rn2,  &qn2,      &a_nrows, &a_nq,     &a_dim,       &a_rb, &a_kb,
                         &a_tiles, &a_keep, &a_st, &a_cs, &d_scratch, &d_cand, &d_nq_dev, &a_stride, &d_thr_fixed, &d_overflow,
-                        &d_filt, &filt_words, &d_filt_q};
+                        &d_filt, &filt_words, &d_filt_q, &d_list_count};
         const cudaError_t le = cudaLaunchKernelExC(&cfg, kfn, args);
         if (le != cudaSuccess)
             fprintf(stderr, "vecsim_b200: coarse pass launch failed (kind %d mode %d csize %u grid %u x %u smem %zu): %s\n", (int)p.kind,
@@ -2299,28 +2398,30 @@
 cudaError_t launch_refine(const CorpusView &c, const void *d_queries, size_t qpitch, uint32_t nq, uint32_t lists_per_query, uint32_t keep,
                           uint32_t k, const uint64_t *d_cand, float eps, const float *d_q_norm2, float max_norm, uint32_t *d_ok,
                           uint64_t *d_out, const uint32_t *d_q_index, const uint32_t *d_nq_dev, cudaStream_t s, const float *d_thr_T,
-                          const uint32_t *d_overflow, const uint64_t *d_row_label, const float *d_q_eps) {
+                          const uint32_t *d_overflow, const uint64_t *d_row_label, const float *d_q_eps, const uint32_t *d_list_count) {
     if (nq == 0) return cudaSuccess;
     const uint32_t okv = d_q_index ? 2u : 1u;
     const uint8_t *rows = static_cast<const uint8_t *>(c.rows), *qs = static_cast<const uint8_t *>(d_queries);
     const bool wide = k > kCoarseMaxK;
     if (k > kCoarseMaxKWide) return cudaErrorInvalidValue;
-    const uint32_t max_cap = wide ? 8192 : 2560;
+    if (d_list_count && (!d_thr_T || lists_per_query > kRefineMaxLists)) return cudaErrorInvalidValue;
+    const uint32_t max_cap = wide ? kRefineCapWide : d_list_count ? kRefineCapCounted : kRefineCapPadded;
     const uint32_t smem_cap = std::min<uint32_t>(lists_per_query * keep, max_cap);
     const size_t smem = (size_t)smem_cap * 8;
     const auto kern = d_row_label ? (c.metric == MT_L2 ? (wide ? refine_kernel<MT_L2, kRefineMaxSurvWide, true> : refine_kernel<MT_L2, kRefineMaxSurv, true>)
                                                       : (wide ? refine_kernel<MT_IP, kRefineMaxSurvWide, true> : refine_kernel<MT_IP, kRefineMaxSurv, true>))
                     : c.metric == MT_L2 ? (wide ? refine_kernel<MT_L2, kRefineMaxSurvWide> : refine_kernel<MT_L2, kRefineMaxSurv>)
                                         : (wide ? refine_kernel<MT_IP, kRefineMaxSurvWide> : refine_kernel<MT_IP, kRefineMaxSurv>);
+    constexpr uint32_t kOptIn = std::max(kRefineCapWide, kRefineCapCounted) * 8;
     cudaFuncAttributes fa{};
     cudaError_t e = cudaFuncGetAttributes(&fa, kern);
     if (e != cudaSuccess) return e;
-    if (fa.sharedSizeBytes + (size_t)max_cap * 8 > 48 * 1024) {
-        e = cudaFuncSetAttribute(kern, cudaFuncAttributeMaxDynamicSharedMemorySize, (int)(max_cap * 8));
+    if (fa.sharedSizeBytes + smem > 48 * 1024 && fa.maxDynamicSharedSizeBytes < (int)kOptIn) {
+        e = cudaFuncSetAttribute(kern, cudaFuncAttributeMaxDynamicSharedMemorySize, (int)kOptIn);
         if (e != cudaSuccess) return e;
     }
-    kern<<<nq, 256, smem, s>>>(rows, c.pitch, c.dim, qs, qpitch, nq, lists_per_query, keep, k, d_cand, eps, d_q_norm2, max_norm, d_ok, okv,
-                               d_out, d_q_index, d_nq_dev, d_thr_T, d_overflow, smem_cap, d_row_label, d_q_eps);
+    kern<<<nq, kRefineThreads, smem, s>>>(rows, c.pitch, c.dim, qs, qpitch, nq, lists_per_query, keep, k, d_cand, eps, d_q_norm2, max_norm, d_ok, okv,
+                               d_out, d_q_index, d_nq_dev, d_thr_T, d_overflow, smem_cap, d_row_label, d_q_eps, d_list_count);
     return cudaGetLastError();
 }
 
diff --git a/redisearch_b200/csrc/coarse_tc.h b/redisearch_b200/csrc/coarse_tc.h
--- a/redisearch_b200/csrc/coarse_tc.h
+++ b/redisearch_b200/csrc/coarse_tc.h
@@ -51,7 +51,7 @@
 cudaError_t launch_coarse(const CoarseOperands &o, uint32_t n_rows, uint32_t dim, uint32_t nq, const CoarsePlan &p, uint64_t *d_cand,
                           uint64_t *d_scratch, cudaStream_t s, const uint32_t *d_nq_dev = nullptr, const float *d_thr_fixed = nullptr,
                           uint32_t *d_overflow = nullptr, const uint32_t *d_filt = nullptr, uint32_t filt_words = 0,
-                          const uint32_t *d_filt_q = nullptr);
+                          const uint32_t *d_filt_q = nullptr, uint32_t *d_list_count = nullptr);
 cudaError_t launch_threshold(const uint64_t *d_cand, uint32_t nq, uint32_t lists_per_query, uint32_t keep, uint32_t k, float eps,
                              const float *d_q_norm2, float max_norm, uint32_t dim, int l2, float *d_thr, uint32_t *d_overflow, cudaStream_t s,
                              const float *d_q_eps = nullptr);
@@ -70,7 +70,7 @@
                           uint32_t k, const uint64_t *d_cand, float eps, const float *d_q_norm2, float max_norm, uint32_t *d_ok,
                           uint64_t *d_out, const uint32_t *d_q_index, const uint32_t *d_nq_dev, cudaStream_t s,
                           const float *d_thr_T = nullptr, const uint32_t *d_overflow = nullptr, const uint64_t *d_row_label = nullptr,
-                          const float *d_q_eps = nullptr);
+                          const float *d_q_eps = nullptr, const uint32_t *d_list_count = nullptr);
 cudaError_t launch_flags_from_overflow(const uint32_t *d_overflow, uint32_t nq, uint32_t *d_ok, cudaStream_t s);
 cudaError_t launch_scatter_rows(const uint64_t *d_src, const uint32_t *d_idx, const uint32_t *d_count, uint32_t max_n, uint32_t k,
                                 uint64_t *d_dst, uint32_t *d_ok, cudaStream_t s);
diff --git a/redisearch_b200/csrc/vecsim_index.cpp b/redisearch_b200/csrc/vecsim_index.cpp
--- a/redisearch_b200/csrc/vecsim_index.cpp
+++ b/redisearch_b200/csrc/vecsim_index.cpp
@@ -969,6 +969,7 @@
     n2 = s.take<uint32_t>(nq ? 1 : 0);
     thr = s.take<float>(nq);
     ovf = s.take<uint32_t>(nq);
+    cnt = s.take<uint32_t>(q8 && t.two_pass ? (size_t)nq * t.main.grid_x : 0);
 }
 
 bool FlatIndex::enqueue_knn_tiers(QueryCtx &c, const CorpusView &v, CoarseKind kind, const KnnTiers &t, const KnnScratch &s,
@@ -985,10 +986,11 @@
     const float *thr = t.two_pass ? s.thr : nullptr;
     uint32_t *ovf = t.two_pass ? s.ovf : nullptr;
     cudaEventRecord(c.ev_start, st);
-    ok = ok && launch_coarse(ops, v.n_rows, v.dim, nq, t.main, s.cand, s.list_scratch, st, nullptr, thr, ovf, bm, words) == cudaSuccess;
+    ok = ok && launch_coarse(ops, v.n_rows, v.dim, nq, t.main, s.cand, s.list_scratch, st, nullptr, thr, ovf, bm, words, nullptr, s.cnt) ==
+                   cudaSuccess;
     cudaEventRecord(c.ev_stop, st);
     ok = ok && launch_refine(v, d_q32, qpitch, nq, t.main.grid_x, t.main.keep, ke, s.cand, eps, s.qn2, shadow_max_norm_, s.ok, out, nullptr,
-                             nullptr, st, thr, ovf, row_label, s.qeps) == cudaSuccess;
+                             nullptr, st, thr, ovf, row_label, s.qeps, s.cnt) == cudaSuccess;
     lc.launches += 2;
     if (!t.tier2) return ok;
     ok = ok && launch_compact_unproven(s.ok, nq, s.idx, s.n2, st) == cudaSuccess;
diff --git a/redisearch_b200/csrc/vecsim_index.h b/redisearch_b200/csrc/vecsim_index.h
--- a/redisearch_b200/csrc/vecsim_index.h
+++ b/redisearch_b200/csrc/vecsim_index.h
@@ -234,6 +234,7 @@
         uint8_t *q = nullptr, *q_t2 = nullptr;
         float *qn2 = nullptr, *qn2_t2 = nullptr, *qeps = nullptr, *qeps_t2 = nullptr, *thr = nullptr;
         uint32_t *ok = nullptr, *idx = nullptr, *n2 = nullptr, *ovf = nullptr;
+        uint32_t *cnt = nullptr;
         void take(BatchScratch &s, const KnnTiers &t, uint32_t nq, size_t q_pitch, bool norms, bool q8);
     };
     bool enqueue_knn_tiers(QueryCtx &c, const CorpusView &v, CoarseKind kind, const KnnTiers &t, const KnnScratch &s, const CoarseOperands &ops,
```

Measured after the change: 78970, median of 6. +6.8%, better.
